# pyamg/pyamg

Measured on AMD Instinct MI355X. Metric: vcycle_iterations_per_sec, higher is better.
Workload: dtype f64; 1 GPU; 3D 7-pt Poisson 256^3 (16.7M dof) SA V-cycle, symmetric Gauss-Seidel, fp64; key=c3, n=16777216, nnz=117047296, levels=5, cycle=V(1,1), graph=True, parallelism=1 GPU, gs_order=fast, full=False

## Files before the change

include/pyamg_amd.h:

```cpp
#ifndef PYAMG_AMD_H
#define PYAMG_AMD_H

#include <stddef.h>
#include <stdint.h>

#ifdef __cplusplus
extern "C" {
#endif

#define PAMG_OK              0
#define PAMG_E_ARG          -1
#define PAMG_E_UNSUPPORTED  -2
#define PAMG_E_NODEVICE     -3
#define PAMG_E_STATE        -4
#define PAMG_E_ALLOC        -5
#define PAMG_E_TIMEOUT      -6

#define PAMG_F64 0
#define PAMG_F32 1

typedef void *pamg_stream_t;
typedef void *pamg_event_t;
typedef struct pamg_matrix_s *pamg_matrix_t;
typedef struct pamg_solver_s *pamg_solver_t;
// ... 159 lines not shown
                                int32_t row_step, int32_t blocksize);
int pamg_block_gauss_seidel_f32(const int32_t *Ap, int Ap_size, const int32_t *Aj,
                                int Aj_size, const float *Ax, int Ax_size, float *x,
                                int x_size, const float *b, int b_size, const float *Tx,
                                int Tx_size, int32_t row_start, int32_t row_stop,
                                int32_t row_step, int32_t blocksize);

int pamg_pinv_array_f64(double *AA, int AA_size, int32_t m, int32_t n, char TransA);
int pamg_pinv_array_f32(float *AA, int AA_size, int32_t m, int32_t n, char TransA);

int pamg_standard_aggregation(int32_t n_row, const int32_t *Ap, int Ap_size, const int32_t *Aj, int Aj_size,
                              int32_t *x, int x_size, int32_t *y, int y_size, int32_t *naggs);
int pamg_fit_candidates_f64(int32_t n_row, int32_t n_col, int32_t K1, int32_t K2, const int32_t *Ap, int Ap_size,
                            const int32_t *Ai, int Ai_size, double *Ax, int Ax_size, const double *B, int B_size,
                            double *R, int R_size, double tol);
int pamg_fit_candidates_f32(int32_t n_row, int32_t n_col, int32_t K1, int32_t K2, const int32_t *Ap, int Ap_size,
                            const int32_t *Ai, int Ai_size, float *Ax, int Ax_size, const float *B, int B_size,
                            float *R, int R_size, float tol);
int pamg_fit_tentative_f64(int32_t n_fine, int32_t n_coarse, int32_t K1, int32_t K2, const int32_t *Tp, const int32_t *Tj,
                           const double *B, double *Qx, double *R, double tol);
int pamg_fit_tentative_f32(int32_t n_fine, int32_t n_coarse, int32_t K1, int32_t K2, const int32_t *Tp, const int32_t *Tj,
                           const float *B, float *Qx, float *R, float tol);

int pamg_bsr_transpose_f64(int32_t n_brow, int32_t n_bcol, int32_t R, int32_t C, const int32_t *Ap, const int32_t *Aj,
                           const double *Ax, int32_t *Bp, int32_t *Bi, double *Bx);
int pamg_bsr_transpose_f32(int32_t n_brow, int32_t n_bcol, int32_t R, int32_t C, const int32_t *Ap, const int32_t *Aj,
                           const float *Ax, int32_t *Bp, int32_t *Bi, float *Bx);

#define PAMG_CSR 0
#define PAMG_BSR 1
int pamg_matrix_create(pamg_matrix_t *A, int dtype, int flavour, int n_brow, int n_bcol,
                       int R, int C, const int32_t *Ap, const int32_t *Aj, const void *Ax);
int pamg_matrix_destroy(pamg_matrix_t A);
int pamg_matrix_info(pamg_matrix_t A, int64_t info[8]);
int pamg_matrix_tune(pamg_matrix_t A, int key, int value);
int pamg_matrix_value_codes(pamg_matrix_t A, int *n_values);
int pamg_matrix_row_patterns(pamg_matrix_t A, int *n_patterns);
int pamg_matrix_row_masks(pamg_matrix_t A, long long info[8]);
int pamg_matrix_autotune(pamg_matrix_t A, int allow_cap);
int pamg_matrix_gs_profile(pamg_matrix_t A, int which, long long *out, int64_t capacity, int64_t *count);
int pamg_matrix_tile_info(pamg_matrix_t A, int which, int64_t info[8]);
int pamg_matrix_lane_info(pamg_matrix_t A, int which, int64_t info[8]);
int pamg_matrix_lanem_info(pamg_matrix_t A, int which, int64_t info[20], double *growth);
int pamg_matrix_point_twin(pamg_matrix_t A, int *state);
int pamg_matrix_lanem_levels(pamg_matrix_t A, int which, int64_t *out, int64_t capacity, int64_t *count);
int pamg_matrix_kz_info(pamg_matrix_t A, int which, int64_t info[8]);
int pamg_matrix_line_info(pamg_matrix_t A, int which, int64_t info[8]);
int pamg_matrix_lane_profile(pamg_matrix_t A, int which, long long *out, int64_t capacity, int64_t *count);
int pamg_matrix_subset_rows(pamg_matrix_t A, const int32_t *rows, int nrows, pamg_matrix_t *sub);
int pamg_matrix_kaczmarz(pamg_matrix_t L, int nr, void *v, const void *b, const void *Dinv, double omega,
                         int sweep, int iterations, void *xout, pamg_stream_t s);
int pamg_matrix_jacobi_indexed(pamg_matrix_t sub, void *x, const void *b, double omega, void *work,
                               pamg_stream_t s);
int pamg_matrix_flow_error(pamg_matrix_t A, int *error);

#define PAMG_SPMV_SET      0
#define PAMG_SPMV_ACC      1
#define PAMG_SPMV_RESID    2
#define PAMG_SPMV_AXPBY    3
#define PAMG_SPMV_ACC_AXPBY 4
int pamg_matrix_spmv(pamg_matrix_t A, int mode, const void *x, const void *b_or_v, double c,
                     void *y, pamg_stream_t s);
int pamg_matrix_split_ranges(pamg_matrix_t A, int64_t n_owned_cols);
int pamg_matrix_spmv_part(pamg_matrix_t A, int part, int mode, const void *x, const void *b_or_v, double c, void *y,
                          pamg_stream_t stream);
int pamg_matrix_resid_sumsq(pamg_matrix_t A, const void *x, const void *b, double *out_sumsq,
                            pamg_stream_t s);

#define PAMG_FORWARD   0
#define PAMG_BACKWARD  1
#define PAMG_SYMMETRIC 2
int pamg_matrix_jacobi(pamg_matrix_t A, void *x, const void *b, void *work, double omega,
                       int iterations, pamg_stream_t s);
int pamg_matrix_jacobi_step(pamg_matrix_t A, const void *x_in, const void *b, void *x_out,
                            double omega, pamg_stream_t s);
int pamg_matrix_block_jacobi_step(pamg_matrix_t A, const void *Dinv, const void *x_in, const void *b, void *x_out,
                                  double omega, pamg_stream_t s);
int pamg_matrix_block_jacobi_indexed(pamg_matrix_t A, const void *Dinv, void *x, const void *b, const int32_t *idx,
                                     int64_t nidx, double omega, void *work, pamg_stream_t s);
int pamg_matrix_gauss_seidel(pamg_matrix_t A, void *x, const void *b, int sweep, double omega,
                             int iterations, pamg_stream_t s);
int pamg_matrix_gauss_seidel_x0(pamg_matrix_t A, void *x, const void *b, int sweep, double omega,
                                int iterations, int x_is_zero, pamg_stream_t s);
int pamg_matrix_sym_info(pamg_matrix_t A, int64_t info[8]);
int pamg_matrix_polynomial(pamg_matrix_t A, void *x, const void *b, void *work,
                           const double *coeffs, int ncoeffs, int iterations, int x_is_zero,
                           pamg_stream_t s);
int pamg_matrix_block_jacobi(pamg_matrix_t A, void *x, const void *b, void *work,
                             const void *Dinv, double omega, int iterations, pamg_stream_t s);
int pamg_matrix_block_gauss_seidel(pamg_matrix_t A, void *x, const void *b, const void *Dinv,
                                   int sweep, int iterations, pamg_stream_t s);

int pamg_dev_pinv_array(int dtype, void *AA, int64_t m, int n, int transA, pamg_stream_t s);

int pamg_vec_sumsq(int dtype, int64_t n, const void *x, double *out_sumsq, pamg_stream_t s);
int pamg_vec_axpy(int dtype, int64_t n, double a, const void *x, void *y, pamg_stream_t s);
int pamg_vec_scale(int dtype, int64_t n, double a, const void *x, void *y, pamg_stream_t s);
int pamg_vec_mul(int dtype, int64_t n, const void *a, const void *b, void *y, pamg_stream_t s);
int pamg_vec_gather(int dtype, int64_t n, const int32_t *idx, const void *src, void *dst,
                    pamg_stream_t s);

int pamg_csr_renumber(int dtype, int64_t nrows, int64_t ncols, const int32_t *Ap, const int32_t *Aj, const void *Ax,
                      const int32_t *row_old_of_new, const int32_t *col_new_of_old, int32_t *Bp, int32_t *Bj, void *Bx);
int pamg_csr_row_argmax_abs(int dtype, int64_t nrows, const int32_t *Ap, const int32_t *Aj, const void *Ax, int32_t *out);
int pamg_csr_sort_rows(int dtype, int64_t nrows, const int32_t *Ap, int32_t *Aj, void *Ax, int block);
int pamg_host_cpus(int fresh);

#define PAMG_SMOOTH_NONE        0
#define PAMG_SMOOTH_JACOBI      1
#define PAMG_SMOOTH_GS          2
#define PAMG_SMOOTH_SOR         3
#define PAMG_SMOOTH_POLY        4
#define PAMG_SMOOTH_BLOCK_JACOBI 5
#define PAMG_SMOOTH_BLOCK_GS    6
#define PAMG_SMOOTH_CF_JACOBI   7
#define PAMG_SMOOTH_FC_JACOBI   8
#define PAMG_SMOOTH_GS_NE       9
#define PAMG_SMOOTH_GS_NR      10
#define PAMG_SMOOTH_JACOBI_NE  11
#define PAMG_SMOOTH_CF_BLOCK_JACOBI 12
#define PAMG_SMOOTH_FC_BLOCK_JACOBI 13
#define PAMG_SMOOTH_SCHWARZ    14
#define PAMG_SMOOTH_KRYLOV     15
#define PAMG_KRYLOV_CG    0
#define PAMG_KRYLOV_GMRES 1
#define PAMG_KRYLOV_CGNE  2
#define PAMG_KRYLOV_CGNR  3
#define PAMG_CYCLE_V 0
#define PAMG_CYCLE_W 1
#define PAMG_CYCLE_F 2
#define PAMG_CYCLE_AMLI 3
int pamg_solver_create(pamg_solver_t *S, int dtype);
int pamg_solver_destroy(pamg_solver_t S);
int pamg_solver_add_level(pamg_solver_t S, pamg_matrix_t A, pamg_matrix_t P, pamg_matrix_t R);
int pamg_solver_set_smoother(pamg_solver_t S, int level, int which, int kind, int iterations,
                             double omega, int sweep, const double *coeffs, int ncoeffs,
                             const void *Dinv, int blocksize);
int pamg_solver_set_cf_smoother(pamg_solver_t S, int level, int which, int kind, int iterations,
                                int f_iterations, int c_iterations, double omega, const int32_t *Fpts,
                                int nF, const int32_t *Cpts, int nC);
int pamg_solver_set_cf_block_smoother(pamg_solver_t S, int level, int which, int kind, int iterations,
                                      int f_iterations, int c_iterations, double omega, const void *Dinv,
                                      int blocksize, const int32_t *Fpts, int nF, const int32_t *Cpts, int nC);
typedef struct pamg_schwarz_s *pamg_schwarz_t;
int pamg_schwarz_create(pamg_schwarz_t *out, pamg_matrix_t A, int nsub, const int32_t *Sp, const int32_t *Sj,
                        const int32_t *Tp, const void *Tx);
int pamg_schwarz_destroy(pamg_schwarz_t h);
int pamg_schwarz_sweep(pamg_schwarz_t h, void *x, const void *b, int row_start, int row_stop, int row_step,
                       pamg_stream_t s);
int pamg_schwarz_info(pamg_schwarz_t h, int64_t info[4]);
int pamg_schwarz_set_mode(pamg_schwarz_t h, int mode);
int pamg_schwarz_error(pamg_schwarz_t h, int *error);
int pamg_solver_set_schwarz_smoother(pamg_solver_t S, int level, int which, int iterations, int sweep, pamg_matrix_t Ar,
                                     int nsub, const int32_t *Sp, const int32_t *Sj, const int32_t *Tp, const void *Tx);
int pamg_solver_set_ne_smoother(pamg_solver_t S, int level, int which, int kind, int iterations, double omega,
                                int sweep, const void *Dinv, pamg_matrix_t At, pamg_matrix_t Ar);
int pamg_solver_set_krylov_smoother(pamg_solver_t S, int level, int which, int method, double tol, int maxiter, int restart,
                                    pamg_matrix_t At);
int pamg_solver_set_coarse_dense(pamg_solver_t S, const void *M, int n_c);
int pamg_solver_set_coarse_relax(pamg_solver_t S);
typedef int (*pamg_coarse_host_fn)(void *user, const void *b_host, void *x_host, int64_t n_c);
int pamg_solver_set_coarse_host(pamg_solver_t S, pamg_coarse_host_fn fn, void *user, int n_c);
int pamg_solver_finalize(pamg_solver_t S);
int pamg_solver_cycle(pamg_solver_t S, void *x, const void *b, int cycle, int cycles_per_level,
                      pamg_stream_t s);
int pamg_solver_solve(pamg_solver_t S, void *x, const void *b, double tol, int maxiter,
                      int cycle, int cycles_per_level, int check_every, double *residuals,
// ... 86 lines not shown
```

pyamg_amd/_capi.py:

```python
from __future__ import annotations

import ctypes as C
import os
from pathlib import Path

import numpy as np

PKG = Path(__file__).resolve().parent
LIB_PATH = Path(os.environ.get("PAMG_LIB", PKG / "libpyamg_amd.so"))

OK = 0
E_ARG, E_UNSUPPORTED, E_NODEVICE, E_STATE, E_ALLOC = -1, -2, -3, -4, -5
E_TIMEOUT, E_COMM = -6, -7
F64, F32 = 0, 1
CSR, BSR = 0, 1
SPMV_SET, SPMV_ACC, SPMV_RESID, SPMV_AXPBY, SPMV_ACC_AXPBY = 0, 1, 2, 3, 4
FORWARD, BACKWARD, SYMMETRIC = 0, 1, 2
SMOOTH = {"schwarz": 14, "cf_block_jacobi": 12, "fc_block_jacobi": 13, "gauss_seidel_ne": 9, "gauss_seidel_nr": 10, "jacobi_ne": 11, "cf_jacobi": 7, "fc_jacobi": 8, "none": 0, "jacobi": 1, "gauss_seidel": 2, "sor": 3, "polynomial": 4,
          "block_jacobi": 5, "block_gauss_seidel": 6}
KRYLOV = {"cg": 0, "gmres": 1, "cgne": 2, "cgnr": 3}
ACCEL = {"bicgstab": 0, "cr": 1, "steepest_descent": 2, "minimal_residual": 3}
SWEEP = {"forward": FORWARD, "backward": BACKWARD, "symmetric": SYMMETRIC}
CYCLE = {"V": 0, "W": 1, "F": 2, "AMLI": 3}

# ... 44 lines not shown
    for n in ("h2d", "d2h", "d2d"):
        f(f"pamg_memcpy_{n}", _vp, _vp, _sz, _vp)
    f("pamg_memset", _vp, _i, _sz, _vp)
    f("pamg_stream_create", P(_vp))
    f("pamg_stream_destroy", _vp)
    f("pamg_stream_synchronize", _vp)
    f("pamg_device_synchronize")
    f("pamg_event_create", P(_vp))
    f("pamg_event_destroy", _vp)
    f("pamg_event_record", _vp, _vp)
    f("pamg_event_synchronize", _vp)
    f("pamg_event_elapsed_ms", _vp, _vp, P(C.c_float))
    for sfx, ct in (("f64", C.c_double), ("f32", C.c_float)):
        f(f"pamg_csr_matvec_{sfx}", _i, _i, _vp, _vp, _vp, _vp, _vp)
        f(f"pamg_bsr_matvec_{sfx}", _i, _i, _i, _i, _vp, _vp, _vp, _vp, _vp)
        csr5 = (_vp, _i, _vp, _i, _vp, _i, _vp, _i, _vp, _i)
        f(f"pamg_gauss_seidel_{sfx}", *csr5, _i, _i, _i)
        f(f"pamg_sor_gauss_seidel_{sfx}", *csr5, _i, _i, _i, ct)
        f(f"pamg_overlapping_schwarz_csr_{sfx}", *csr5, _vp, _i, _vp, _i, _vp, _i, _vp, _i, _i, _i, _i, _i, _i)
        f(f"pamg_gauss_seidel_indexed_{sfx}", *csr5, _vp, _i, _i, _i, _i)
        f(f"pamg_bsr_gauss_seidel_{sfx}", *csr5, _i, _i, _i, _i)
        f(f"pamg_jacobi_{sfx}", *csr5, _vp, _i, _i, _i, _i, _vp, _i)
        f(f"pamg_bsr_jacobi_{sfx}", *csr5, _vp, _i, _i, _i, _i, _i, _vp, _i)
        f(f"pamg_jacobi_indexed_{sfx}", *csr5, _vp, _i, _vp, _i)
        f(f"pamg_gauss_seidel_ne_{sfx}", *csr5, _i, _i, _i, _vp, _i, ct)
        f(f"pamg_gauss_seidel_nr_{sfx}", *csr5, _i, _i, _i, _vp, _i, ct)
        f(f"pamg_jacobi_ne_{sfx}", *csr5, _vp, _i, _vp, _i, _i, _i, _i, _vp, _i)
        f(f"pamg_block_jacobi_{sfx}", *csr5, _vp, _i, _vp, _i, _i, _i, _i, _vp, _i, _i)
        f(f"pamg_block_gauss_seidel_{sfx}", *csr5, _vp, _i, _i, _i, _i, _i)
        f(f"pamg_block_jacobi_indexed_{sfx}", *csr5, _vp, _i, _vp, _i, _vp, _i, _i)
    f("pamg_pinv_array_f64", _vp, _i, _i, _i, C.c_char)
    f("pamg_pinv_array_f32", _vp, _i, _i, _i, C.c_char)
    f("pamg_dev_pinv_array", _i, _vp, C.c_int64, _i, _i, _vp)
    f("pamg_bsr_transpose_f64", _i, _i, _i, _i, _vp, _vp, _vp, _vp, _vp, _vp)
    f("pamg_bsr_transpose_f32", _i, _i, _i, _i, _vp, _vp, _vp, _vp, _vp, _vp)
    f("pamg_standard_aggregation", _i, _vp, _i, _vp, _i, _vp, _i, _vp, _i, P(_i))
    f("pamg_csr_standard_aggregation", _vp, _vp, _vp, P(_i))
    f("pamg_fit_candidates_f64", _i, _i, _i, _i, _vp, _i, _vp, _i, _vp, _i, _vp, _i, _vp, _i, _d)
    f("pamg_fit_candidates_f32", _i, _i, _i, _i, _vp, _i, _vp, _i, _vp, _i, _vp, _i, _vp, _i, C.c_float)
    f("pamg_fit_tentative_f64", _i, _i, _i, _i, _vp, _vp, _vp, _vp, _vp, _d)
    f("pamg_fit_tentative_f32", _i, _i, _i, _i, _vp, _vp, _vp, _vp, _vp, C.c_float)
    f("pamg_matrix_create", P(_vp), _i, _i, _i, _i, _i, _i, _vp, _vp, _vp)
    f("pamg_matrix_destroy", _vp)
    f("pamg_matrix_info", _vp, P(C.c_int64))
    f("pamg_matrix_tune", _vp, _i, _i)
    f("pamg_matrix_value_codes", _vp, P(C.c_int))
    f("pamg_matrix_row_patterns", _vp, P(C.c_int))
    f("pamg_matrix_row_masks", _vp, P(C.c_longlong))
    f("pamg_matrix_flow_error", _vp, P(_i))
    f("pamg_matrix_subset_rows", _vp, _vp, _i, P(_vp))
    f("pamg_matrix_kaczmarz", _vp, _i, _vp, _vp, _vp, _d, _i, _i, _vp, _vp)
    f("pamg_vec_mul", _i, C.c_int64, _vp, _vp, _vp, _vp)
    f("pamg_matrix_jacobi_indexed", _vp, _vp, _vp, _d, _vp, _vp)
    f("pamg_matrix_gs_profile", _vp, _i, _vp, C.c_int64, P(C.c_int64))
    f("pamg_matrix_tile_info", _vp, _i, P(C.c_int64))
    f("pamg_matrix_lane_info", _vp, _i, P(C.c_int64))
    f("pamg_matrix_lanem_info", _vp, _i, P(C.c_int64), P(C.c_double))
    f("pamg_matrix_point_twin", _vp, P(_i))
    f("pamg_matrix_lanem_levels", _vp, _i, _vp, C.c_int64, P(C.c_int64))
    f("pamg_matrix_kz_info", _vp, _i, P(C.c_int64))
    f("pamg_matrix_line_info", _vp, _i, P(C.c_int64))
    f("pamg_matrix_lane_profile", _vp, _i, _vp, C.c_int64, P(C.c_int64))
    f("pamg_matrix_autotune", _vp, _i)
    f("pamg_matrix_spmv", _vp, _i, _vp, _vp, _d, _vp, _vp)
    f("pamg_matrix_split_ranges", _vp, C.c_int64)
    f("pamg_matrix_spmv_part", _vp, _i, _i, _vp, _vp, _d, _vp, _vp)
    f("pamg_matrix_resid_sumsq", _vp, _vp, _vp, _vp, _vp)
    f("pamg_matrix_jacobi", _vp, _vp, _vp, _vp, _d, _i, _vp)
    f("pamg_l1_cache_clear")
    f("pamg_l1_cache_size", P(C.c_int))
    f("pamg_matrix_jacobi_step", _vp, _vp, _vp, _vp, _d, _vp)
    f("pamg_matrix_block_jacobi_step", _vp, _vp, _vp, _vp, _vp, _d, _vp)
    f("pamg_matrix_block_jacobi_indexed", _vp, _vp, _vp, _vp, _vp, C.c_int64, _d, _vp, _vp)
    f("pamg_schwarz_create", P(_vp), _vp, _i, _vp, _vp, _vp, _vp)
    f("pamg_schwarz_destroy", _vp)
    f("pamg_schwarz_sweep", _vp, _vp, _vp, _i, _i, _i, _vp)
    f("pamg_schwarz_info", _vp, P(C.c_int64))
    f("pamg_schwarz_set_mode", _vp, _i)
    f("pamg_schwarz_error", _vp, P(_i))
    f("pamg_solver_set_schwarz_smoother", _vp, _i, _i, _i, _i, _vp, _i, _vp, _vp, _vp, _vp)
    f("pamg_solver_set_cf_block_smoother", _vp, _i, _i, _i, _i, _i, _i, _d, _vp, _i, _vp, _i, _vp, _i)
    f("pamg_matrix_gauss_seidel", _vp, _vp, _vp, _i, _d, _i, _vp)
    f("pamg_matrix_gauss_seidel_x0", _vp, _vp, _vp, _i, _d, _i, _i, _vp)
    f("pamg_matrix_sym_info", _vp, P(C.c_int64))
    f("pamg_matrix_polynomial", _vp, _vp, _vp, _vp, _vp, _i, _i, _i, _vp)
    f("pamg_matrix_block_jacobi", _vp, _vp, _vp, _vp, _vp, _d, _i, _vp)
    f("pamg_matrix_block_gauss_seidel", _vp, _vp, _vp, _vp, _i, _i, _vp)
    f("pamg_vec_sumsq", _i, C.c_int64, _vp, _vp, _vp)
    f("pamg_vec_axpy", _i, C.c_int64, _d, _vp, _vp, _vp)
    f("pamg_vec_scale", _i, C.c_int64, _d, _vp, _vp, _vp)
    f("pamg_vec_gather", _i, C.c_int64, _vp, _vp, _vp, _vp)
    f("pamg_csr_renumber", _i, C.c_int64, C.c_int64, _vp, _vp, _vp, _vp, _vp, _vp, _vp, _vp)
    f("pamg_csr_row_argmax_abs", _i, C.c_int64, _vp, _vp, _vp, _vp)
    f("pamg_csr_sort_rows", _i, C.c_int64, _vp, _vp, _vp, _i)
    f("pamg_host_cpus", _i)
    f("pamg_solver_create", P(_vp), _i)
    f("pamg_solver_destroy", _vp)
    f("pamg_solver_add_level", _vp, _vp, _vp, _vp)
    f("pamg_solver_set_smoother", _vp, _i, _i, _i, _i, _d, _i, _vp, _i, _vp, _i)
    f("pamg_solver_set_ne_smoother", _vp, _i, _i, _i, _i, _d, _i, _vp, _vp, _vp)
    f("pamg_solver_set_krylov_smoother", _vp, _i, _i, _i, _d, _i, _i, _vp)
    f("pamg_solver_set_cf_smoother", _vp, _i, _i, _i, _i, _i, _i, _d, _vp, _i, _vp, _i)
    f("pamg_solver_set_coarse_dense", _vp, _vp, _i)
    f("pamg_solver_set_coarse_relax", _vp)
    f("pamg_solver_set_coarse_host", _vp, _vp, _vp, _i)
    f("pamg_solver_finalize", _vp)
    f("pamg_solver_cycle", _vp, _vp, _vp, _i, _i, _vp)
    f("pamg_solver_solve", _vp, _vp, _vp, _d, _i, _i, _i, _i, _vp, P(_i), P(_i), _vp)
    f("pamg_solver_set_graph", _vp, _i)
    f("pamg_solver_pcg", _vp, _vp, _vp, _d, _i, _i, _i, _vp, P(_i), P(_i), _vp)
    f("pamg_solver_fgmres", _vp, _vp, _vp, _d, _i, _i, _i, _i, _vp, _i, P(_i), P(_i), P(_i), _vp)
    f("pamg_solver_gmres", _vp, _vp, _vp, _d, _i, _i, _i, _i, _vp, _i, P(_i), P(_i), P(_i), _vp)
    f("pamg_solver_krylov", _vp, _i, _vp, _vp, _d, _i, _i, _i, _vp, _i, P(_i), P(_i), P(_i), _vp)
    f("pamg_solver_load", _vp, _vp, _vp, _vp)
    f("pamg_solver_iterate", _vp, _i, _i, _i, _vp, _vp)
    f("pamg_solver_store", _vp, _vp, _vp)
    f("pamg_solver_stream", _vp, P(_vp))
    f("pamg_solver_stats", _vp, P(C.c_int64))
    f("pamg_dist_create", P(_vp), _i, _i, _i)
    f("pamg_dist_destroy", _vp)
    f("pamg_dist_add_level", _vp, _vp, _vp, _vp, C.c_int64, C.c_int64, _i, _vp, _vp, _vp, _i, _vp, _vp)
    f("pamg_dist_set_collapse", _vp, _vp, C.c_int64, C.c_int64, C.c_int64, C.c_int64, _vp)
    f("pamg_dist_set_smoother", _vp, _i, _i, _i, _i, _d, _vp, _i, _vp, _i)
    f("pamg_dist_set_callbacks", _vp, _vp, _vp, _vp)
    f("pamg_dist_rccl_unique_id", _vp)
    f("pamg_dist_set_rccl", _vp, _vp)
    f("pamg_dist_finalize", _vp)
    f("pamg_dist_set_options", _vp, _i, _i)
    f("pamg_dist_load", _vp, _vp, _vp)
    f("pamg_dist_store", _vp, _vp)
    f("pamg_dist_iterate", _vp, _i, _vp)
    f("pamg_dist_resid_norm", _vp, P(_d))
    f("pamg_dist_sync", _vp)
    f("pamg_dist_stream", _vp, P(_vp))
    f("pamg_dist_info", _vp, P(C.c_int64))
    f("pamg_dist_set_allgather", _vp, _i, C.c_int64, _vp)
    f("pamg_dist_set_exchange", _vp, _i)
    f("pamg_dist_set_model_transport", _vp)
    f("pamg_dist_level_info", _vp, _i, P(C.c_int64))
    f("pamg_rccl_selftest", C.c_int64, P(C.c_double))
    f("pamg_rccl_available")
    f("pamg_dist_exchange_test", _vp, _i, _vp, _vp)
    f("pamg_csr_create", P(_vp), C.c_int64, C.c_int64, _vp, _vp, _vp)
    f("pamg_csr_view", P(_vp), _vp)
    f("pamg_csr_destroy", _vp)
    f("pamg_csr_info", _vp, P(C.c_int64))
    f("pamg_csr_download", _vp, _vp, _vp, _vp)
    f("pamg_csr_matmat", _vp, _vp, _i, _i, P(_vp))
    f("pamg_csr_subtract", _vp, _vp, P(_vp))
    f("pamg_csr_subtract_bsr", _vp, _vp, _i, _i, P(_vp))
    f("pamg_csr_scale", _vp, _d)
    f("pamg_csr_strength_symmetric", _vp, _d, P(_vp))
    f("pamg_matrix_scale_rows", _vp, _vp)
    f("pamg_matrix_scale_values", _vp, _d)
    f("pamg_arnoldi_create", P(_vp), _vp, _i)
    f("pamg_arnoldi_destroy", _vp)
    f("pamg_arnoldi_run", _vp, _vp, _vp, _d, _vp, P(_i), P(_i))
    f("pamg_arnoldi_combine", _vp, _i, _vp, _vp)
    f("pamg_arnoldi_vector", _vp, _vp, _vp, P(_i))


def load(require_device: bool = False):
    global _lib
    if _lib is None:
        if not LIB_PATH.exists():
            raise DeviceUnavailable(
# ... 122 lines not shown
```

pyamg_amd/csrc/pamg_common.h:

```cpp
#pragma once
#include "pamg_host_threads.h"
#include <hip/hip_runtime.h>

#include <cstdint>
#include <cstdio>
#include <cstdlib>
#include <ctime>
#include <algorithm>
#include <atomic>
#include <cstring>
#include <thread>
#include <vector>

#include "../../include/pyamg_amd.h"

#define PAMG_STR2(x) #x
#define PAMG_STR(x) PAMG_STR2(x)
#define PAMG_HIP(expr)                                   \
    do {                                                 \
        hipError_t e__ = (expr);                         \
        if (e__ != hipSuccess) return (int)e__;          \
    } while (0)
#define PAMG_TRY(expr)                                   \
    do {                                                 \
// ... 121 lines not shown
}

struct pamg_matrix_s {
    int dtype = PAMG_F64;
    int flavour = PAMG_CSR;
    int n_brow = 0, n_bcol = 0, R = 1, C = 1;
    int64_t nrows = 0, ncols = 0, nnz = 0;
    int *d_Ap = nullptr, *d_Aj = nullptr;
    void *d_Ax = nullptr;
    void *d_diag = nullptr;
    int *d_rowid = nullptr;
    int *d_bAp = nullptr, *d_bAj = nullptr;
    int *d_bAjf = nullptr, *d_bdiag = nullptr;
    void *d_bAx = nullptr;
    int64_t nblocks_b = 0;
    int4 *d_bmeta = nullptr;
    int bnblk = 0;
    std::vector<int> h_Ap, h_Aj;
    std::vector<int> h_bAp, h_bAj;
    int cap = 1536, npl = 2, max_rows = 1024;
    int flow_cap = 32;
    unsigned short *d_Aj16 = nullptr;
    int4 *d_wbase = nullptr;
    int use_idx16 = 1;
    unsigned char *d_Ax8 = nullptr;
    void *d_vdict = nullptr;
    int nvdict = 0;
    int use_val8 = 1;
    int use_rowg = 0;
    unsigned char *d_pid = nullptr;
    void *d_ptab = nullptr;
    int npat = 0, pat_lmax = 0;
    unsigned char *d_pmask = nullptr;
    int rm_nu = 0, rm_off[8] = {0, 0, 0, 0, 0, 0, 0, 0};
    unsigned long long rm_val[8] = {0, 0, 0, 0, 0, 0, 0, 0};
    long long rm_walked = 0;
    int rowmask_kz = 8;
    int rowmask_flags = 3;
    int use_rowpat = 1;
    int cap_from_val8 = 0;
    int stream_flags = 0;
    int lds_pad = 0;
    int gran_xcd = 0;
    int gran_cap = 0;
    int gs_mode = 0;
    int tile_G = 0;
    int tile_W = 0;
    int tile_cap = 0;
    int tile_D = 0, tile_Q = -1;
    int tile_part = 1;
    bool tile_default = false;
    int max_row_len = 0;
    int borrowed = 0;
    int gs_prof = 0;
    int gs_order = 0;
    int lane_L = 0, lane_G = 0;
    int lane_flags = 1;
    int line_scan = 1;
    int lane_merge = 0;
    int lanem_rpw = 0;
    int lanem_cluster = 0;
    int lanem_ahead10 = 40;
    int lane_wide = 0;
    int gs_cap = 0;
    int nblk = 0;
    int *d_part[2] = {nullptr, nullptr};
    int npart[2] = {0, 0};
    int64_t part_cols = -1;
    int64_t part_row0[2] = {-1, -1}, part_row1[2] = {-1, -1};
    int4 *d_blkmeta = nullptr;
    double *d_partial = nullptr;
    pamg::GsSchedule *gs[4] = {nullptr, nullptr, nullptr, nullptr};
    pamg_matrix_s *point_twin = nullptr;
    size_t point_twin_bytes = 0;
    bool point_twin_unfit = false;
    pamg::LineSchedule *ls[4] = {nullptr, nullptr, nullptr, nullptr};
    int sym_fused = 1;
    void *d_sym_hf[2] = {nullptr, nullptr}, *d_sym_hb = nullptr;
    unsigned *d_sym_sync = nullptr;
    int sym_cap = 0;
    const void *sym_cap_kernel = nullptr;
    int zsym_cap = 0;
    const void *zsym_cap_kernel = nullptr;
    int sym_general_grid = 0;
    int sym_form = 0, sym_grid = 0;
    long long sym_launches = 0, sym_zero_launches = 0;
    int zero_plans = 0;
    int zero_merge = 0;
    struct pamg::LaneMSched *zplan[2] = {nullptr, nullptr};
    void *d_zw = nullptr;
    size_t zero_bytes = 0;
    long long zero_plan_launches = 0;
    size_t bytes = 0;
};

struct pamg_schwarz_s;
struct pamg_solver_s;
struct pamg_csr_s;

namespace pamg {
int schwarz_sweep(pamg_schwarz_s *h, void *x, const void *b, int start, int stop, int step, hipStream_t s);
int schwarz_prepare(pamg_schwarz_s *h, int sweep);
int schwarz_error(pamg_schwarz_s *h, bool *error);
void schwarz_level_launches(pamg_schwarz_s *h);
int stream_launch(pamg_matrix_s *A, int epi, const void *x, const void *b, void *y, double c,
                  double omega, double *partial, hipStream_t s);
int stream_launch_part(pamg_matrix_s *A, int part, int epi, const void *x, const void *b, void *y, double c,
                       double omega, double *partial, hipStream_t s);
int matrix_split_ranges(pamg_matrix_s *A, int64_t n_owned_cols);
void matrix_drop_value_codes(pamg_matrix_s *A);
void matrix_drop_point_twin(pamg_matrix_s *A);
void matrix_drop_schedules(pamg_matrix_s *A);
int gs_sweep(pamg_matrix_s *A, int epi, void *x, const void *b, double omega, int row_start,
             int row_stop, int row_step, hipStream_t s);
int gs_sweep_symmetric(pamg_matrix_s *A, void *x, const void *b, bool x_zero, hipStream_t s, bool *ran);
int ensure_sym_parts(pamg_matrix_s *A);
int sym_reset(pamg_matrix_s *A);
int reduce_partials(const double *partial, int n, double *out, hipStream_t s);
int vec_sumsq(int dtype, int64_t n, const void *x, double *scratch, double *out, hipStream_t s);
int vec_axpy(int dtype, int64_t n, double a, const void *x, void *y, hipStream_t s);
int vec_scale(int dtype, int64_t n, double a, const void *x, void *y, hipStream_t s);
int vec_dot(int dtype, int64_t n, const void *x, const void *y, double *scratch, double *out, hipStream_t s);
int vec_mul(int dtype, int64_t n, const void *a, const void *b, void *y, hipStream_t s);
int kaczmarz_sweep(pamg_matrix_s *L, bool nr, void *v, const void *b, const void *Dinv, double omega, int start, int stop,
                   int step, void *xout, hipStream_t s);
int ensure_line_schedule(pamg_matrix_s *L, int start, int stop, int step);
void free_line_schedule(LineSchedule *g);
int vec_scatter(int dtype, int64_t n, const int *idx, const void *src, void *dst, hipStream_t s);
int vec_copy_indexed(int dtype, int64_t n, const int *idx, const void *src, void *dst, hipStream_t s);
int matrix_row_subset(pamg_matrix_s *A, const int32_t *rows, int nrows, pamg_matrix_s **out);
int jacobi_indexed(pamg_matrix_s *sub, void *x, const void *b, double omega, void *work, hipStream_t s);
int vec_maxratio(int dtype, int64_t n, const void *u, const void *x, double *scratch, double *out, hipStream_t s);
int vec_xpby(int dtype, int64_t n, double beta, const void *z, void *p, hipStream_t s);
int vec_axpy_ratio(int dtype, int64_t n, const double *num, const double *den, double sign, const void *x, void *y, hipStream_t s);
int vec_fill(int dtype, int64_t n, double v, void *y, hipStream_t s);
int dense_gemv(int dtype, int n, const void *M, const void *b, void *x, hipStream_t s);
int block_gs_sweep(pamg_matrix_s *A, void *x, const void *b, const void *Dinv, int row_start,
                   int row_stop, int row_step, hipStream_t s);
int block_jacobi_step(pamg_matrix_s *A, int kind, const void *Dinv, const void *xsrc, void *xdst,
                      const void *b, double omega, hipStream_t s);
int ensure_schedule(pamg_matrix_s *A, int row_start, int row_stop, int row_step, bool block_gs = false);
struct CsrArrays { int64_t m, n, nnz; const int *p, *j; const double *x; };
int csr_device_arrays(struct ::pamg_csr_s *A, CsrArrays *out);
constexpr int KR_PARTIALS = 3 * 2048;
int kr_reduce(int64_t n, const double *part, int k, double *o0, double *o1, double *o2, hipStream_t s);
int kr_dots(int dtype, int64_t n, int k, const void *a0, const void *b0, const void *a1, const void *b1, const void *a2, const void *b2,
            double *part, hipStream_t s);
int bicg_alpha(int dtype, int64_t n, const double *rr, const double *d, double *alpha, void *x, void *xc, const void *r, const void *AMp,
               void *bc, hipStream_t s);
int bicg_omega(int dtype, int64_t n, const double *num, const double *den, double *omega, void *x, const void *xc, const void *bc,
               const void *AMs, void *r, const void *rstar, double *part, hipStream_t s);
int bicg_dir(int dtype, int64_t n, const double *rr_new, const double *rr_old, const double *alpha, const double *omega, const void *r,
             void *p, const void *AMp, void *bc, void *xc, hipStream_t s);
int cr_update(int dtype, int64_t n, const double *rAz, const double *ApAp, void *x, const void *p, void *r, const void *Ap, bool update_r,
              void *xc, hipStream_t s);
int cr_dir(int dtype, int64_t n, const double *rAz_new, const double *rAz_old, void *p, const void *z, void *Ap, const void *Az,
           double *part, hipStream_t s);
int sd_update(int dtype, int64_t n, const double *rz, const double *zAz, void *x, void *xc, void *r, const void *q, bool update_r,
              hipStream_t s);
int mr_update(int dtype, int64_t n, const double *pz, const double *pp, void *x, void *z, void *xc, bool update_z, double *part,
              hipStream_t s);
int kr_take(int dtype, int64_t n, void *xc, void *dst, double *part, hipStream_t s);
int solver_cycle_inline(pamg_solver_s *S, void *x, const void *b, int cycle, int cpl, hipStream_t s, bool allow_graph);
bool solver_needs_host_sync(const pamg_solver_s *S);
bool line_eligible(const pamg_matrix_s *A, const GsSchedule *g);
int build_line_part(pamg_matrix_s *A, GsSchedule *g);
void free_line_part(LineSched *t);
size_t line_part_bytes(const GsSchedule *g);
int line_launch(pamg_matrix_s *A, GsSchedule *g, int epi, void *x, const void *b, double omega, hipStream_t s);
int line_info(const GsSchedule *g, int64_t *info);
int line_sym_launch(pamg_matrix_s *A, GsSchedule *gf, GsSchedule *gb, void *x, const void *b, hipStream_t s);
int build_kz_lane_part(pamg_matrix_s *Lm, LineSchedule *g);
void free_kz_lane_part(KzLaneSched *t);
int kz_lane_launch(pamg_matrix_s *Lm, LineSchedule *g, bool nr, void *v, const void *b, const void *Dinv, double omega, void *xout, hipStream_t s);
int kz_lane_info(const LineSchedule *g, int64_t *info);
bool kz_lane_error(LineSchedule *g);
bool want_blanes(const pamg_matrix_s *A, const GsSchedule *g);
int block_point_sweep(pamg_matrix_s *A, GsSchedule *g, void *x, const void *b, int dirn, hipStream_t s);
int get_schedule(pamg_matrix_s *A, int row_start, int row_stop, int row_step, GsSchedule **out);
int ensure_parts(pamg_matrix_s *A, GsSchedule *g, bool block_gs = false);
int device_cus();
bool blane_eligible(const pamg_matrix_s *A, const GsSchedule *g);
int build_blane_part(pamg_matrix_s *A, GsSchedule *g);
void free_blane_part(BlaneSched *t);
size_t blane_part_bytes(const GsSchedule *g);
int blane_launch(pamg_matrix_s *A, GsSchedule *g, const void *Dinv, void *x, const void *b, hipStream_t s);
int blane_info(const GsSchedule *g, int64_t *info);
int blane_profile(const GsSchedule *g, long long *out, int64_t cap, int64_t *n);
int device_cus_lane();
bool lane_eligible(const pamg_matrix_s *A, const GsSchedule *g);
int build_lane_part(pamg_matrix_s *A, GsSchedule *g);
void free_lane_part(LaneSched *t);
size_t lane_part_bytes(const GsSchedule *g);
int lane_launch(pamg_matrix_s *A, GsSchedule *g, int epi, void *x, const void *b, double omega, hipStream_t s);
int lane_info(const GsSchedule *g, int64_t *info);
int lane_profile(const GsSchedule *g, long long *out, int64_t cap, int64_t *n);
int lanem_smax(const pamg_matrix_s *A, const GsSchedule *g);
int build_lanem_part(pamg_matrix_s *A, GsSchedule *g);
void free_lanem_part(struct LaneMSched *t);
size_t lanem_part_bytes(const GsSchedule *g);
int lanem_info(const GsSchedule *g, int64_t *info, double *growth);
int lanem_levels(const GsSchedule *g, int64_t *out, int64_t cap, int64_t *n);
int lanem_sym_launch(pamg_matrix_s *A, GsSchedule *gf, GsSchedule *gb, void *x, const void *b, bool x_zero, hipStream_t s);
int lanem_plan_info(const struct LaneMSched *t, int64_t *info, double *growth);
int build_zero_plan(pamg_matrix_s *A, int dir);
void free_zero_plans(pamg_matrix_s *A);
size_t zero_plan_bytes(const pamg_matrix_s *A);
bool zero_plans_ready(const pamg_matrix_s *A, const GsSchedule *gf, const GsSchedule *gb);
int lanem_zero_pair_launch(pamg_matrix_s *A, GsSchedule *gf, GsSchedule *gb, void *x, const void *b, hipStream_t s);
int ensure_zero_parts(pamg_matrix_s *A, bool build);
void matrix_drop_zero_plans(pamg_matrix_s *A);
int gs_sweep_zero_pair(pamg_matrix_s *A, void *x, const void *b, hipStream_t s, bool *ran);
int sym_fill_sentinels(void *p, int64_t n);
int sweep_error(pamg_matrix_s *A, bool *error);
inline size_t tsize(int dtype) { return dtype == PAMG_F64 ? 8 : 4; }

template <typename F>
inline void host_parallel(int64_t n, F fn, int64_t grain = 1 << 20)
{
    const unsigned hw = std::max(1u, std::min(32u, pamg::host_cpus()));
    const int nt = n < 2 * grain ? 1 : (int)std::min<int64_t>(hw, n / grain);
    if (nt <= 1) { fn((int64_t)0, n); return; }
    std::vector<std::thread> th;
    for (int t = 0; t < nt; ++t) {
        const int64_t lo = n * t / nt, hi = n * (t + 1) / nt;
        th.emplace_back([=] { fn(lo, hi); });
    }
    for (auto &x : th) x.join();
}

struct PhaseTimer {
    const char *name;
    int64_t items;
    timespec t0;
    static bool on() { static const int v = [] { const char *e = getenv("PAMG_TIMING"); return (e && *e && *e != '0') ? 1 : 0; }(); return v != 0; }
    explicit PhaseTimer(const char *n, int64_t k = 0) : name(n), items(k) { if (on()) clock_gettime(CLOCK_MONOTONIC, &t0); }
    ~PhaseTimer()
    {
        if (!on()) return;
        timespec t1;
        clock_gettime(CLOCK_MONOTONIC, &t1);
        fprintf(stderr, "[pamg timing] %-28s %8.3f s  (%lld)\n", name, (double)(t1.tv_sec - t0.tv_sec) + 1e-9 * (double)(t1.tv_nsec - t0.tv_nsec), (long long)items);
    }
};
}
```

pyamg_amd/csrc/pamg_lane.hip:

```cpp
#include "pamg_common.h"
#include "pamg_lane_plan.h"
#include "pamg_lanem_plan.h"
#include "pamg_tile_plan.h"

namespace pamg {

template <typename T> struct Sentinel;
template <> struct Sentinel<double> {
    using bits_t = unsigned long long;
    static constexpr bits_t value = 0x7FF8DEADBEEF5A5Aull;
    static __device__ __forceinline__ bits_t bits(double v) { return (bits_t)__double_as_longlong(v); }
};
template <> struct Sentinel<float> {
    using bits_t = unsigned int;
    static constexpr bits_t value = 0x7FC5BEEFu;
    static __device__ __forceinline__ bits_t bits(float v) { return __float_as_uint(v); }
};

template <typename T>
__global__ __launch_bounds__(BLK) void lane_fill_sentinel_kernel(T *xs, int64_t n)
{
    using B = typename Sentinel<T>::bits_t;
    B *p = reinterpret_cast<B *>(xs);
    for (int64_t i = (int64_t)blockIdx.x * BLK + threadIdx.x; i < n; i += (int64_t)gridDim.x * BLK) p[i] = Sentinel<T>::value;
// ... 290 lines not shown
    LaneMRec *d_rec = nullptr;
    long long *d_prof = nullptr;
    int cluster = 0;
    int4 *d_crec = nullptr;
    unsigned short *d_sidx = nullptr;
    int *d_crid = nullptr;
    double *d_crd = nullptr;
    int64_t n_uunits = 0, n_uearly = 0, n_uold = 0, n_ub = 0, n_early_lines = 0;
    std::vector<int64_t> super_grp;
    int last_grid = 0;
    int cap = 0;
    const void *cap_kernel = nullptr;
    size_t bytes = 0;
};

struct LaneMArgs {
    const int *cols;
    const double *vals;
    const LaneMRec *rec;
    const double *xold;
    double *y;
    double *xs;
    const double *b;
    unsigned *err;
    unsigned *ticket;
    int ngroups, nidle, use_gate;
    long long *prof;
    const unsigned short *sidx;
    const int *crid;
    const double *crd;
    int crows;
    double *w;
};

__global__ __launch_bounds__(BLK) void lanem_prepare_kernel(const double *__restrict__ x, double *__restrict__ xold, double *__restrict__ xs, int64_t n)
{
    unsigned long long *p = reinterpret_cast<unsigned long long *>(xs);
    for (int64_t i = (int64_t)blockIdx.x * BLK + threadIdx.x; i < n; i += (int64_t)gridDim.x * BLK) {
        xold[i] = x[i];
        p[i] = Sentinel<double>::value;
    }
}

template <int NREG>
struct MCtx {
    int c[NREG];
    double v[NREG], xv[NREG];
    double bv, xo, rd;
    double num;
    int rid;
    int gate, unit, K, g;
};

__device__ __forceinline__ void m_rec(const int4 *rp, int g, int gend, int4 &q0, int4 &q1)
{
    const size_t gg = (size_t)(g < gend ? g : gend - 1);
    q0 = rp[2 * gg];
    q1 = rp[2 * gg + 1];
}

template <int RPW, int NREG>
__device__ __forceinline__ void m_slots(const LaneMArgs &a, MCtx<NREG> &C, const int4 &q0, const int4 &q1, int g, int lane)
{
    C.g = g;
    const int rid_a = __builtin_amdgcn_readfirstlane(q0.x), rid_b = __builtin_amdgcn_readfirstlane(q0.y);
    C.gate = a.use_gate ? __builtin_amdgcn_readfirstlane(q0.z) : -1;
    const int uk = __builtin_amdgcn_readfirstlane(q0.w);
    C.unit = uk >> 4;
    C.K = uk & 15;
    const double rd_a = __hiloint2double(__builtin_amdgcn_readfirstlane(q1.y), __builtin_amdgcn_readfirstlane(q1.x));
    const double rd_b = __hiloint2double(__builtin_amdgcn_readfirstlane(q1.w), __builtin_amdgcn_readfirstlane(q1.z));
    const bool second = RPW == 2 && lane >= 32;
    C.rid = second ? rid_b : rid_a;
    C.rd = second ? rd_b : rd_a;
    const size_t e0 = (size_t)C.unit * 64 + (size_t)lane;
#pragma unroll
    for (int k = 0; k < NREG; ++k) {
        const size_t e = e0 + (size_t)64 * (size_t)(k < C.K ? k : C.K - 1);
        C.c[k] = a.cols[e];
        C.v[k] = a.vals[e];
    }
}

template <int NREG, bool BCOH = false>
__device__ __forceinline__ void m_gather(const LaneMArgs &a, MCtx<NREG> &C, int idle, const bool xz = false, const bool coh = false)
{
#pragma unroll
    for (int k = 1; k < NREG; ++k)
        if (k >= C.K) C.c[k] = LANE_NONE;
    if (xz) {
#pragma unroll
        for (int k = 0; k < NREG; ++k)
            if (!(C.c[k] & (LANE_EARLY | LANEM_BSRC))) C.c[k] |= LANE_NONE;
    }
    const int row = C.rid < 0 ? 0 : (C.rid & LANE_MASK);
    if constexpr (BCOH) C.bv = __hip_atomic_load(a.b + row, __ATOMIC_RELAXED, __HIP_MEMORY_SCOPE_AGENT);
    else C.bv = a.b[row];
    C.xo = coh ? __hip_atomic_load(a.xold + row, __ATOMIC_RELAXED, __HIP_MEMORY_SCOPE_AGENT) : a.xold[row];
#pragma unroll
    for (int k = 0; k < NREG; ++k) {
        const int col = C.c[k] & LANEM_MASK;
        const double *p = (C.c[k] & LANE_NONE) ? a.xold + idle : ((C.c[k] & LANE_EARLY) ? a.xs + col : ((C.c[k] & LANEM_BSRC) ? a.b + col : a.xold + col));
        C.xv[k] = __hip_atomic_load(p, __ATOMIC_RELAXED, __HIP_MEMORY_SCOPE_AGENT);
    }
}

template <int RPW, int NREG>
__device__ __forceinline__ double m_finish(const LaneMArgs &a, MCtx<NREG> &C, int idle, long long *t_ready = nullptr, unsigned *n_spins = nullptr, const bool xz = false)
{
    using T = double;
    const int lane = threadIdx.x & 63;
    unsigned pend = 0;
#pragma unroll
    for (int k = 0; k < NREG; ++k)
        if ((C.c[k] & LANE_EARLY) && !(C.c[k] & LANE_NONE) && Sentinel<T>::bits(C.xv[k]) == Sentinel<T>::value) pend |= 1u << k;
    unsigned spins = 0;
    if (C.gate >= 0 && __builtin_amdgcn_ballot_w64(pend != 0)) {
        const T *gp = a.xs + C.gate;
        while (true) {
            const T gv = __hip_atomic_load(gp, __ATOMIC_RELAXED, __HIP_MEMORY_SCOPE_AGENT);
            if (Sentinel<T>::bits(gv) != Sentinel<T>::value) break;
            __builtin_amdgcn_s_sleep(2);
            if ((++spins & 1023u) == 0 && (spins > (1u << 21) || __hip_atomic_load(a.err, __ATOMIC_RELAXED, __HIP_MEMORY_SCOPE_AGENT))) break;
        }
    }
    while (pend) {
        if (spins) __builtin_amdgcn_s_sleep(1);
        T t[NREG];
#pragma unroll
        for (int k = 0; k < NREG; ++k)
            t[k] = __hip_atomic_load(((pend >> k) & 1u) ? a.xs + (C.c[k] & LANEM_MASK) : a.xs + idle, __ATOMIC_RELAXED, __HIP_MEMORY_SCOPE_AGENT);
#pragma unroll
        for (int k = 0; k < NREG; ++k)
            if ((pend >> k) & 1u) {
                C.xv[k] = t[k];
                if (Sentinel<T>::bits(t[k]) != Sentinel<T>::value) pend &= ~(1u << k);
            }
        if ((++spins & 1023u) == 0) {
            if (spins > (1u << 21) || __hip_atomic_load(a.err, __ATOMIC_RELAXED, __HIP_MEMORY_SCOPE_AGENT)) {
                __hip_atomic_store(a.err, 1u, __ATOMIC_RELAXED, __HIP_MEMORY_SCOPE_AGENT);
                break;
            }
        }
    }
    if (t_ready) { *t_ready = wall_clock64(); *n_spins = spins; }
    T s = T(0);
#pragma unroll
    for (int k = 0; k < NREG; ++k) {
        const T pr = C.v[k] * C.xv[k];
        s = s + ((C.c[k] & LANE_NONE) ? T(0) : pr);
    }
    if (C.K > NREG) {
        for (int k = NREG; k < C.K; ++k) {
            const size_t e = (size_t)(C.unit + k) * 64 + (size_t)lane;
            int c = a.cols[e];
            if (xz && !(c & (LANE_EARLY | LANEM_BSRC))) c |= LANE_NONE;
            const T v = a.vals[e];
            const int col = c & LANEM_MASK;
            const bool early = (c & LANE_EARLY) && !(c & LANE_NONE);
            const T *p = (c & LANE_NONE) ? a.xold + idle : ((c & LANE_EARLY) ? a.xs + col : ((c & LANEM_BSRC) ? a.b + col : a.xold + col));
            T x = __hip_atomic_load(p, __ATOMIC_RELAXED, __HIP_MEMORY_SCOPE_AGENT);
            unsigned sp2 = 0;
            while (__builtin_amdgcn_ballot_w64(early && Sentinel<T>::bits(x) == Sentinel<T>::value)) {
                __builtin_amdgcn_s_sleep(1);
                const T t = __hip_atomic_load(p, __ATOMIC_RELAXED, __HIP_MEMORY_SCOPE_AGENT);
                if (early && Sentinel<T>::bits(x) == Sentinel<T>::value) x = t;
                if ((++sp2 & 1023u) == 0 && (sp2 > (1u << 21) || __hip_atomic_load(a.err, __ATOMIC_RELAXED, __HIP_MEMORY_SCOPE_AGENT))) {
                    __hip_atomic_store(a.err, 1u, __ATOMIC_RELAXED, __HIP_MEMORY_SCOPE_AGENT);
                    break;
                }
            }
            const T pr = v * x;
            s = s + ((c & LANE_NONE) ? T(0) : pr);
        }
    }
    s = seg_allreduce<64 / RPW, T>(s);
    const bool upd = C.rid >= 0 && !(C.rid & LANE_NODIAG);
    C.num = C.bv - s;
    T val = C.num * C.rd;
    if (!upd) val = C.xo;
    return val;
}

template <int RPW, int MODE, int NREG, int PH = 0, bool WST = false>
__device__ __forceinline__ void m_publish(const LaneMArgs &a, const MCtx<NREG> &C, double val)
{
    if (((threadIdx.x & 63) & (64 / RPW - 1)) == 0 && C.rid >= 0) {
        const int row = C.rid & LANE_MASK;
        if constexpr (MODE == 1) __hip_atomic_store(a.xs + row, val, __ATOMIC_RELAXED, __HIP_MEMORY_SCOPE_WORKGROUP);
        else __hip_atomic_store(a.xs + row, val, __ATOMIC_RELAXED, __HIP_MEMORY_SCOPE_AGENT);
        if constexpr (PH != 1) {
            if (!(C.rid & LANE_NODIAG)) a.y[row] = val;
        }
        if constexpr (WST) {
            if (!(C.rid & LANE_NODIAG)) __hip_atomic_store(a.w + row, C.num, __ATOMIC_RELAXED, __HIP_MEMORY_SCOPE_AGENT);
        }
    }
}

constexpr int LANEC_K = 8;

__device__ __forceinline__ int4 c_rec(const int4 *rp, int g, int gend) { return rp[(size_t)(g < gend ? g : gend - 1)]; }

template <int PH, bool WST = false, bool BCOH = false>
__device__ __forceinline__ void c_group(const LaneMArgs &a, double *lds, const int4 &q, int g, int lane, int idle, const bool xz, const bool coh)
{
    using T = double;
    const int gate = a.use_gate ? __builtin_amdgcn_readfirstlane(q.x) : -1;
    const int uunit = __builtin_amdgcn_readfirstlane(q.y), sunit = __builtin_amdgcn_readfirstlane(q.z), kk = __builtin_amdgcn_readfirstlane(q.w);
    const int KU = kk & 15, KS = (kk >> 8) & 15;
    int c[LANEC_K];
    unsigned si[LANEC_K];
    T sv[LANEC_K], xv[LANEC_K];
    const size_t u0 = (size_t)uunit * 64 + (size_t)lane, s0 = (size_t)sunit * 64 + (size_t)lane;
#pragma unroll
    for (int k = 0; k < LANEC_K; ++k) {
        c[k] = LANE_NONE;
        if (k < KU) c[k] = a.cols[u0 + (size_t)64 * k];
    }
#pragma unroll
    for (int k = 0; k < LANEC_K; ++k) {
        si[k] = LANEC_PAD | LANEC_UNUSED; sv[k] = T(0);
        if (k < KS) { si[k] = a.sidx[s0 + (size_t)64 * k]; sv[k] = a.vals[s0 + (size_t)64 * k]; }
    }
    if (xz) {
#pragma unroll
        for (int k = 0; k < LANEC_K; ++k)
            if (!(c[k] & (LANE_EARLY | LANEM_BSRC))) c[k] |= LANE_NONE;
    }
#pragma unroll
    for (int k = 0; k < LANEC_K; ++k) {
        xv[k] = T(0);
        if (k < KU) {
            const int col = c[k] & LANEM_MASK;
            const T *p = (c[k] & LANE_NONE) ? a.xold + idle : ((c[k] & LANE_EARLY) ? a.xs + col : ((c[k] & LANEM_BSRC) ? a.b + col : a.xold + col));
            xv[k] = __hip_atomic_load(p, __ATOMIC_RELAXED, __HIP_MEMORY_SCOPE_AGENT);
        }
    }
    const bool unused = (si[0] & LANEC_UNUSED) != 0;
    const int tag = (int)((si[0] >> LANEC_ROWSHIFT) & 7u);
    const size_t ri = (size_t)g * (size_t)a.crows + (size_t)(tag < a.crows ? tag : 0);
    const int rid = unused ? -1 : a.crid[ri];
    const T rd = a.crd[ri];
    const int row = rid < 0 ? 0 : (rid & LANE_MASK);
    T bv;
    if constexpr (BCOH) bv = __hip_atomic_load(a.b + row, __ATOMIC_RELAXED, __HIP_MEMORY_SCOPE_AGENT);
    else bv = a.b[row];
    const T xo = coh ? __hip_atomic_load(a.xold + row, __ATOMIC_RELAXED, __HIP_MEMORY_SCOPE_AGENT) : a.xold[row];
    unsigned pend = 0;
#pragma unroll
    for (int k = 0; k < LANEC_K; ++k)
        if ((c[k] & LANE_EARLY) && !(c[k] & LANE_NONE) && Sentinel<T>::bits(xv[k]) == Sentinel<T>::value) pend |= 1u << k;
    unsigned spins = 0;
    if (gate >= 0 && __builtin_amdgcn_ballot_w64(pend != 0)) {
        const T *gp = a.xs + gate;
        while (true) {
            const T gv = __hip_atomic_load(gp, __ATOMIC_RELAXED, __HIP_MEMORY_SCOPE_AGENT);
            if (Sentinel<T>::bits(gv) != Sentinel<T>::value) break;
            __builtin_amdgcn_s_sleep(2);
            if ((++spins & 1023u) == 0 && (spins > (1u << 21) || __hip_atomic_load(a.err, __ATOMIC_RELAXED, __HIP_MEMORY_SCOPE_AGENT))) break;
        }
    }
    while (pend) {
        if (spins) __builtin_amdgcn_s_sleep(1);
        T t[LANEC_K];
#pragma unroll
        for (int k = 0; k < LANEC_K; ++k) {
            t[k] = T(0);
            if (k < KU) t[k] = __hip_atomic_load(((pend >> k) & 1u) ? a.xs + (c[k] & LANEM_MASK) : a.xs + idle, __ATOMIC_RELAXED, __HIP_MEMORY_SCOPE_AGENT);
        }
#pragma unroll
        for (int k = 0; k < LANEC_K; ++k)
            if ((pend >> k) & 1u) {
                xv[k] = t[k];
                if (Sentinel<T>::bits(t[k]) != Sentinel<T>::value) pend &= ~(1u << k);
            }
        if ((++spins & 1023u) == 0) {
            if (spins > (1u << 21) || __hip_atomic_load(a.err, __ATOMIC_RELAXED, __HIP_MEMORY_SCOPE_AGENT)) {
                __hip_atomic_store(a.err, 1u, __ATOMIC_RELAXED, __HIP_MEMORY_SCOPE_AGENT);
                break;
            }
        }
    }
#pragma unroll
    for (int k = 0; k < LANEC_K; ++k)
        if (k < KU) lds[k * 64 + lane] = (c[k] & LANE_NONE) ? T(0) : xv[k];
    __builtin_amdgcn_fence(__ATOMIC_RELEASE, "wavefront");
    __builtin_amdgcn_wave_barrier();
    __builtin_amdgcn_fence(__ATOMIC_ACQUIRE, "wavefront");
    T s = T(0);
#pragma unroll
    for (int k = 0; k < LANEC_K; ++k) {
        const T pr = sv[k] * lds[si[k] & LANEC_IDX];
        s = s + ((si[k] & LANEC_PAD) ? T(0) : pr);
    }
    const unsigned key = si[0] & ((7u << LANEC_ROWSHIFT) | LANEC_UNUSED);
    const unsigned left = (unsigned)__shfl_up((int)key, 1);
    const unsigned long long heads = __builtin_amdgcn_ballot_w64(lane == 0 || left != key);
    const int seglo = 63 - __builtin_clzll(heads & (~0ull >> (63 - lane)));
#pragma unroll
    for (int d = 1; d < 64; d *= 2) {
        const T o = __shfl_up(s, d);
        s = s + ((lane - d >= seglo) ? o : T(0));
    }
    const bool tail = ((((heads >> 1) | (1ull << 63)) >> lane) & 1ull) != 0;
    __builtin_amdgcn_fence(__ATOMIC_RELEASE, "wavefront");
    __builtin_amdgcn_wave_barrier();
    const bool upd = rid >= 0 && !(rid & LANE_NODIAG);
    const T num = bv - s;
    T val = num * rd;
    if (!upd) val = xo;
    if (tail && rid >= 0) {
        __hip_atomic_store(a.xs + row, val, __ATOMIC_RELAXED, __HIP_MEMORY_SCOPE_AGENT);
        if constexpr (PH != 1) {
            if (upd) a.y[row] = val;
        }
        if constexpr (WST) {
            if (upd) __hip_atomic_store(a.w + row, num, __ATOMIC_RELAXED, __HIP_MEMORY_SCOPE_AGENT);
        }
    }
}

template <int MODE, int RPW, int NREG, int Z = 0>
__global__ __launch_bounds__(BLK) void gs_lanem_kernel(const LaneMArgs a)
{
    const int lane = threadIdx.x & 63;
    const int wib = threadIdx.x >> 6;
    const int idle = (int)((((unsigned)blockIdx.x * LANE_WPB + (unsigned)wib) * 16u) % (unsigned)a.nidle);
    const int4 *rp = reinterpret_cast<const int4 *>(a.rec);
    const int gend = a.ngroups;
    __shared__ double c_lds[RPW == 0 ? LANE_WPB * LANEC_UMAX : 1];
    if constexpr (RPW == 0) {
        static_assert(RPW != 0 || MODE != 1, "the cluster layout has no ticket form");
        const int W = (int)gridDim.x * LANE_WPB;
        int g = __builtin_amdgcn_readfirstlane((int)blockIdx.x * LANE_WPB + wib);
        if (g >= gend) return;
        int4 q = c_rec(rp, g, gend);
        for (; g < gend; g += W) {
            const int4 nq = c_rec(rp, g + W, gend);
            c_group<0, Z != 0>(a, c_lds + wib * LANEC_UMAX, q, g, lane, idle, false, false);
            q = nq;
        }
    } else {
    MCtx<NREG> X;
    if constexpr (MODE != 1) {
        const int W = (int)gridDim.x * LANE_WPB;
        int g = __builtin_amdgcn_readfirstlane((int)blockIdx.x * LANE_WPB + wib);
        if (g >= gend) return;
        int4 q0, q1;
        m_rec(rp, g, gend, q0, q1);
        for (; g < gend; g += W) {
            int4 n0, n1;
            m_rec(rp, g + W, gend, n0, n1);
            if (a.prof) {
                const long long t0 = wall_clock64();
                m_slots<RPW, NREG>(a, X, q0, q1, g, lane);
                asm volatile("s_waitcnt vmcnt(0)" ::: "memory");
                const long long t1 = wall_clock64();
                m_gather<NREG>(a, X, idle);
                long long t2 = 0;
                unsigned sp = 0;
                const double val = m_finish<RPW, NREG>(a, X, idle, &t2, &sp);
                m_publish<RPW, MODE, NREG, 0, Z != 0>(a, X, val);
                if (lane == 0) {
                    long long *o = a.prof + (size_t)g * 4;
                    o[0] = t0 | ((long long)(sp > 4095u ? 4095u : sp) << 52);
                    o[1] = t1; o[2] = t2; o[3] = wall_clock64();
                }
            } else {
                m_slots<RPW, NREG>(a, X, q0, q1, g, lane);
                m_gather<NREG>(a, X, idle);
                const double val = m_finish<RPW, NREG>(a, X, idle);
                m_publish<RPW, MODE, NREG, 0, Z != 0>(a, X, val);
            }
            q0 = n0; q1 = n1;
        }
    } else {
        __shared__ int sh_home;
        if (threadIdx.x == 0) {
            const unsigned me = (__builtin_amdgcn_s_getreg((3 << 11) | 20) & 0xF) + 1u;
            unsigned home = 0u;
            __hip_atomic_compare_exchange_strong(a.ticket + 1, &home, me, __ATOMIC_RELAXED, __ATOMIC_RELAXED, __HIP_MEMORY_SCOPE_AGENT);
            sh_home = (home == 0u || home == me) ? 1 : 0;
        }
        __syncthreads();
        if (!sh_home) return;
        unsigned tk = 0;
        if (lane == 0) tk = __hip_atomic_fetch_add(a.ticket, 1u, __ATOMIC_RELAXED, __HIP_MEMORY_SCOPE_AGENT);
        int g = (int)__builtin_amdgcn_readfirstlane(tk);
        if (g >= gend) return;
        if (lane == 0) tk = __hip_atomic_fetch_add(a.ticket, 1u, __ATOMIC_RELAXED, __HIP_MEMORY_SCOPE_AGENT);
        int g2 = (int)__builtin_amdgcn_readfirstlane(tk);
        int4 q0, q1;
        m_rec(rp, g, gend, q0, q1);
        while (true) {
            int4 n0, n1;
            m_rec(rp, g2, gend, n0, n1);
            unsigned tk3 = 0;
            if (g2 < gend && lane == 0) tk3 = __hip_atomic_fetch_add(a.ticket, 1u, __ATOMIC_RELAXED, __HIP_MEMORY_SCOPE_AGENT);
            m_slots<RPW, NREG>(a, X, q0, q1, g, lane);
            m_gather<NREG>(a, X, idle);
            const double val = m_finish<RPW, NREG>(a, X, idle);
            m_publish<RPW, MODE, NREG, 0, Z != 0>(a, X, val);
            if (g2 >= gend) break;
            g = g2; q0 = n0; q1 = n1;
            g2 = (int)__builtin_amdgcn_readfirstlane(tk3);
        }
    }
    }
}

struct LaneMSymArgs {
    LaneMArgs ph[2];
    double *hf[2];
    unsigned *sync;
    int wq[2], wr[2], wblk[2];
    int xzero;
};

template <int MODE>
__device__ __forceinline__ void m_wipe(double *w, int g, int G, int q, int r, int blk, int lane)
{
    if (g & (blk - 1)) return;
    const int g1 = g + blk < G ? g + blk : G;
    const int lo = g * q + (g < r ? g : r), hi = g1 * q + (g1 < r ? g1 : r);
    unsigned long long *p = reinterpret_cast<unsigned long long *>(w);
    for (int i = lo + lane; i < hi; i += 64) {
        if constexpr (MODE == 1) __hip_atomic_store(p + i, Sentinel<double>::value, __ATOMIC_RELAXED, __HIP_MEMORY_SCOPE_WORKGROUP);
        else __hip_atomic_store(p + i, Sentinel<double>::value, __ATOMIC_RELAXED, __HIP_MEMORY_SCOPE_AGENT);
    }
}

template <int MODE, int RPW, int NREG, int PH, int Z = 0>
__device__ __forceinline__ unsigned m_phase(const LaneMArgs &a, double *wipe, int wq, int wr, int wblk, unsigned *ticket, const bool xz, int lane, int wib, int idle, double *c_lds)
{
    const int4 *rp = reinterpret_cast<const int4 *>(a.rec);
    const int gend = a.ngroups;
    unsigned done = 0;
    if constexpr (RPW == 0) {
        static_assert(RPW != 0 || MODE != 1, "the cluster layout has no ticket form");
        const int W = (int)gridDim.x * LANE_WPB;
        int g = __builtin_amdgcn_readfirstlane((int)blockIdx.x * LANE_WPB + wib);
        if (g >= gend) return 0;
        int4 q = c_rec(rp, g, gend);
        for (; g < gend; g += W) {
            const int4 nq = c_rec(rp, g + W, gend);
            c_group<PH, Z && PH == 1, Z && PH == 2>(a, c_lds + wib * LANEC_UMAX, q, g, lane, idle, xz, PH == 2);
            m_wipe<MODE>(wipe, g, gend, wq, wr, wblk, lane);
            ++done;
            q = nq;
        }
    } else {
    MCtx<NREG> X;
    if constexpr (MODE != 1) {
        const int W = (int)gridDim.x * LANE_WPB;
        int g = __builtin_amdgcn_readfirstlane((int)blockIdx.x * LANE_WPB + wib);
        if (g >= gend) return 0;
        int4 q0, q1;
        m_rec(rp, g, gend, q0, q1);
        for (; g < gend; g += W) {
            int4 n0, n1;
            m_rec(rp, g + W, gend, n0, n1);
            m_slots<RPW, NREG>(a, X, q0, q1, g, lane);
            m_gather<NREG, Z && PH == 2>(a, X, idle, xz, PH == 2);
            const double val = m_finish<RPW, NREG>(a, X, idle, nullptr, nullptr, xz);
            m_publish<RPW, MODE, NREG, PH, Z && PH == 1>(a, X, val);
            m_wipe<MODE>(wipe, g, gend, wq, wr, wblk, lane);
            ++done;
            q0 = n0; q1 = n1;
        }
    } else {
        unsigned tk = 0;
        if (lane == 0) tk = __hip_atomic_fetch_add(ticket, 1u, __ATOMIC_RELAXED, __HIP_MEMORY_SCOPE_AGENT);
        int g = (int)__builtin_amdgcn_readfirstlane(tk);
        if (g >= gend) return 0;
        if (lane == 0) tk = __hip_atomic_fetch_add(ticket, 1u, __ATOMIC_RELAXED, __HIP_MEMORY_SCOPE_AGENT);
        int g2 = (int)__builtin_amdgcn_readfirstlane(tk);
        int4 q0, q1;
        m_rec(rp, g, gend, q0, q1);
        while (true) {
            int4 n0, n1;
            m_rec(rp, g2, gend, n0, n1);
            unsigned tk3 = 0;
            if (g2 < gend && lane == 0) tk3 = __hip_atomic_fetch_add(ticket, 1u, __ATOMIC_RELAXED, __HIP_MEMORY_SCOPE_AGENT);
            m_slots<RPW, NREG>(a, X, q0, q1, g, lane);
            m_gather<NREG, Z && PH == 2>(a, X, idle, xz, PH == 2);
            const double val = m_finish<RPW, NREG>(a, X, idle, nullptr, nullptr, xz);
            m_publish<RPW, MODE, NREG, PH, Z && PH == 1>(a, X, val);
            m_wipe<MODE>(wipe, g, gend, wq, wr, wblk, lane);
            ++done;
            if (g2 >= gend) break;
            g = g2; q0 = n0; q1 = n1;
            g2 = (int)__builtin_amdgcn_readfirstlane(tk3);
        }
    }
    }
    return done;
}

__device__ __forceinline__ void sym_phase_barrier(unsigned *counter, unsigned *err, unsigned *sh_done, unsigned done, unsigned total)
{
    asm volatile("s_waitcnt vmcnt(0)" ::: "memory");
    if ((threadIdx.x & 63) == 0 && done) atomicAdd(sh_done, done);
    __syncthreads();
    if (threadIdx.x == 0) {
        const unsigned mine = *sh_done;
        if (mine) __hip_atomic_fetch_add(counter, mine, __ATOMIC_RELAXED, __HIP_MEMORY_SCOPE_AGENT);
        unsigned spins = 0;
        while (__hip_atomic_load(counter, __ATOMIC_RELAXED, __HIP_MEMORY_SCOPE_AGENT) < total) {
            __builtin_amdgcn_s_sleep(2);
            if ((++spins & 1023u) == 0 && (spins > (1u << 21) || __hip_atomic_load(err, __ATOMIC_RELAXED, __HIP_MEMORY_SCOPE_AGENT))) {
                __hip_atomic_store(err, 1u, __ATOMIC_RELAXED, __HIP_MEMORY_SCOPE_AGENT);
                break;
            }
        }
    }
    __syncthreads();
}

__device__ __forceinline__ void sym_leave(unsigned *sync, unsigned parity)
{
    __syncthreads();
    if (threadIdx.x == 0) {
        const unsigned left = __hip_atomic_fetch_add(sync + 1, 1u, __ATOMIC_RELAXED, __HIP_MEMORY_SCOPE_AGENT);
        if (left == gridDim.x - 1) {
            for (int k = 0; k < 5; ++k) __hip_atomic_store(sync + k, 0u, __ATOMIC_RELAXED, __HIP_MEMORY_SCOPE_AGENT);
            __hip_atomic_store(sync + 5, parity ^ 1u, __ATOMIC_RELAXED, __HIP_MEMORY_SCOPE_AGENT);
        }
    }
}

template <int MODE, int RPW, int NREG, int Z = 0>
__global__ __launch_bounds__(BLK) void gs_lanem_sym_kernel(const LaneMSymArgs a)
{
    __shared__ unsigned sh_done;
    __shared__ int sh_home;
    __shared__ double c_lds[RPW == 0 ? LANE_WPB * LANEC_UMAX : 1];
    const int lane = threadIdx.x & 63;
    const int wib = threadIdx.x >> 6;
    const int idle = (int)((((unsigned)blockIdx.x * LANE_WPB + (unsigned)wib) * 16u) % (unsigned)a.ph[0].nidle);
    const unsigned parity = __builtin_amdgcn_readfirstlane(__hip_atomic_load(a.sync + 5, __ATOMIC_RELAXED, __HIP_MEMORY_SCOPE_AGENT)) & 1u;
    if (threadIdx.x == 0) {
        sh_done = 0u;
        sh_home = 1;
        if constexpr (MODE == 1) {
            const unsigned me = (__builtin_amdgcn_s_getreg((3 << 11) | 20) & 0xF) + 1u;
            unsigned home = 0u;
            __hip_atomic_compare_exchange_strong(a.sync + 4, &home, me, __ATOMIC_RELAXED, __ATOMIC_RELAXED, __HIP_MEMORY_SCOPE_AGENT);
            sh_home = (home == 0u || home == me) ? 1 : 0;
        }
    }
    __syncthreads();
    if (sh_home) {
        double *hf = a.hf[parity], *hf_next = a.hf[parity ^ 1u];
        LaneMArgs p1 = a.ph[0], p2 = a.ph[1];
        p1.xs = hf; p1.y = nullptr;
        p2.xold = hf;
        const unsigned done = m_phase<MODE, RPW, NREG, 1, Z>(p1, p2.xs, a.wq[0], a.wr[0], a.wblk[0], a.sync + 2, a.xzero != 0, lane, wib, idle, c_lds);
        sym_phase_barrier(a.sync, p1.err, &sh_done, done, (unsigned)p1.ngroups);
        (void)m_phase<MODE, RPW, NREG, 2, Z>(p2, hf_next, a.wq[1], a.wr[1], a.wblk[1], a.sync + 3, false, lane, wib, idle, c_lds);
    }
    sym_leave(a.sync, parity);
}

namespace {

template <typename U>
int lane_upload(U **dst, const void *src, size_t bytes, size_t *total)
{
    *dst = nullptr;
    const size_t alloc = std::max<size_t>(bytes, 256) + 256;
// ... 286 lines not shown

int lanem_zero_smax(const pamg_matrix_s *A)
{
    if (A->zero_merge >= 2) return A->zero_merge;
    static const int env = [] { const char *e = getenv("PAMG_ZERO_MERGE"); return e ? atoi(e) : 0; }();
    if (env >= 2) return env;
    return A->nrows > 131072 ? 6 : 16;
}

int build_zero_plan(pamg_matrix_s *A, int dir)
{
    if (dir < 0 || dir > 1 || A->zplan[dir]) return PAMG_OK;
    if (A->dtype != PAMG_F64 || A->R != 1 || A->nrows < 2 || A->nrows != A->ncols || !A->d_Ax) return PAMG_E_ARG;
    PhaseTimer pt_(dir ? "build_zero_plan (backward, triu)" : "build_zero_plan (forward, tril)", A->nnz);
    const int n = (int)A->nrows;
    PlanVec<double> hAx;
    hAx.resize((size_t)A->nnz + 1);
    if (A->nnz) PAMG_HIP(hipMemcpy(hAx.data(), A->d_Ax, (size_t)A->nnz * sizeof(double), hipMemcpyDeviceToHost));
    const int *Ap = A->h_Ap.data(), *Aj = A->h_Aj.data();
    std::vector<int> Tp((size_t)n + 1, 0);
    lane_parallel(n, [&](int64_t i0, int64_t i1) {
        for (int64_t i = i0; i < i1; ++i) {
            int c = 0;
            for (int p = Ap[i]; p < Ap[i + 1]; ++p) c += dir ? (Aj[p] >= (int)i) : (Aj[p] <= (int)i);
            Tp[(size_t)i + 1] = c;
        }
    });
    for (int i = 0; i < n; ++i) Tp[(size_t)i + 1] += Tp[(size_t)i];
    PlanVec<int> Tj;
    PlanVec<double> Tx;
    Tj.resize((size_t)Tp[(size_t)n] + 1);
    Tx.resize((size_t)Tp[(size_t)n] + 1);
    lane_parallel(n, [&](int64_t i0, int64_t i1) {
        for (int64_t i = i0; i < i1; ++i) {
            int q = Tp[(size_t)i];
            for (int p = Ap[i]; p < Ap[i + 1]; ++p)
                if (dir ? (Aj[p] >= (int)i) : (Aj[p] <= (int)i)) { Tj[(size_t)q] = Aj[p]; Tx[(size_t)q] = hAx[(size_t)p]; ++q; }
        }
    });
    hAx = PlanVec<double>();
    std::vector<int> vis, lvl;
    int m = 0, nl = 0;
    if (sweep_levels(n, Tp.data(), Tj.data(), dir ? n - 1 : 0, dir ? -1 : n, dir ? -1 : 1, vis, lvl, m, nl) || m != n || nl < 8) return PAMG_E_ARG;
    const int s_max = lanem_zero_smax(A);
    const int rpw = A->lanem_rpw ? A->lanem_rpw : (A->nrows > 131072 ? 2 : 1);
    LaneMPlan P;
    if (build_lanem_plan(n, Tp.data(), Tj.data(), Tx.data(), dir ? n - 1 : 0, dir ? -1 : 1, m, nl, vis, lvl, s_max, 1e3, P, LANEM_KMAX * 64, rpw, lanem_cluster_rows(A)))
        return PAMG_E_ARG;
    LaneMSched *t = nullptr;
    PAMG_TRY(lanem_to_device(P, s_max, &t));
    A->zplan[dir] = t;
    return PAMG_OK;
}

void free_zero_plans(pamg_matrix_s *A)
{
    for (int d = 0; d < 2; ++d) { free_lanem_part(A->zplan[d]); A->zplan[d] = nullptr; }
    hipFree(A->d_zw);
    A->d_zw = nullptr;
}

size_t zero_plan_bytes(const pamg_matrix_s *A)
{
    size_t b = A->d_zw ? ((size_t)A->nrows + 8) * sizeof(double) : 0;
    for (int d = 0; d < 2; ++d) if (A->zplan[d]) b += A->zplan[d]->bytes;
    return b;
}

bool zero_plans_ready(const pamg_matrix_s *A, const GsSchedule *gf, const GsSchedule *gb)
{
    const LaneMSched *zf = A->zplan[0], *zb = A->zplan[1];
    if (A->zero_plans == 1 || !zf || !zb || !A->d_zw || !gf || !gb || !gf->lanem || !gb->lanem) return false;
    return zf->rpw == zb->rpw && zf->cluster == zb->cluster && zf->rpw == gf->lanem->rpw && zf->cluster == gf->lanem->cluster &&
           zb->rpw == gb->lanem->rpw && zb->cluster == gb->lanem->cluster && zf->ngroups >= 1 && zb->ngroups >= 1;
}

static void lanem_layout_args(const LaneMSched *t, LaneMArgs &a)
{
    a.cols = t->d_cols; a.vals = t->d_vals;
    a.rec = t->cluster ? reinterpret_cast<const LaneMRec *>(t->d_crec) : t->d_rec;
    a.sidx = t->d_sidx; a.crid = t->d_crid; a.crd = t->d_crd; a.crows = t->cluster;
}

static int lanem_launch_plan(pamg_matrix_s *A, GsSchedule *g, LaneMSched *t, void *x, const void *b, double *w, hipStream_t s)
{
    if (!t || !g->d_xold) return PAMG_E_STATE;
    const int64_t n = A->nrows;
    LaneMArgs a;
    lanem_layout_args(t, a);
    a.use_gate = (A->lane_flags & 1) ? 1 : 0;
    a.xold = (const double *)g->d_xold; a.y = (double *)x; a.xs = (double *)g->d_xs; a.b = (const double *)b;
    a.w = w;
    a.err = g->d_sync + 1; a.ticket = g->d_sync + 20;
    a.ngroups = (int)t->ngroups;
    a.nidle = (int)std::max<int64_t>(1, std::min<int64_t>(n, 1 << 20));
    if (A->gs_prof && !t->d_prof && !t->cluster) {
        PAMG_HIP(hipMalloc((void **)&t->d_prof, (size_t)t->ngroups * 4 * sizeof(long long)));
        PAMG_HIP(hipMemset(t->d_prof, 0, (size_t)t->ngroups * 4 * sizeof(long long)));
    }
    a.prof = (A->gs_prof && !t->cluster) ? t->d_prof : nullptr;
    const int fgrid = (int)std::min<int64_t>(4096, (n + BLK - 1) / BLK);
    hipLaunchKernelGGL(lanem_prepare_kernel, dim3(fgrid), dim3(BLK), 0, s, (const double *)x, (double *)g->d_xold, (double *)g->d_xs, n);
    PAMG_HIP(hipGetLastError());
    const bool xcd = !t->cluster && (A->gran_xcd == 1 || (A->gran_xcd == 0 && lane_one_xcd(A, g) && A->nrows <= 8192));
    static const int nreg_env = [] { const char *e = getenv("PAMG_LANEM_NREG"); return e ? atoi(e) : 0; }();
    const bool all_regs = t->rpw == 1 && (nreg_env ? nreg_env == 8 : A->nrows <= 131072);
    const void *k = t->cluster  ? (const void *)gs_lanem_kernel<0, 0, 8>
                  : t->rpw == 2 ? (xcd ? (const void *)gs_lanem_kernel<1, 2, 4> : (const void *)gs_lanem_kernel<0, 2, 4>)
                  : all_regs    ? (xcd ? (const void *)gs_lanem_kernel<1, 1, 8> : (const void *)gs_lanem_kernel<0, 1, 8>)
                                : (xcd ? (const void *)gs_lanem_kernel<1, 1, 2> : (const void *)gs_lanem_kernel<0, 1, 2>);
    if (w)
        k = t->cluster  ? (const void *)gs_lanem_kernel<0, 0, 8, 1>
          : t->rpw == 2 ? (xcd ? (const void *)gs_lanem_kernel<1, 2, 4, 1> : (const void *)gs_lanem_kernel<0, 2, 4, 1>)
          : all_regs    ? (xcd ? (const void *)gs_lanem_kernel<1, 1, 8, 1> : (const void *)gs_lanem_kernel<0, 1, 8, 1>)
                        : (xcd ? (const void *)gs_lanem_kernel<1, 1, 2, 1> : (const void *)gs_lanem_kernel<0, 1, 2, 1>);
    static thread_local int cus = 0;
    if (!cus) cus = device_cus_lane();
    if (!(t->cap > 0 && t->cap_kernel == k)) {
        int nb = 0;
        if (hipOccupancyMaxActiveBlocksPerMultiprocessor(&nb, k, BLK, 0) != hipSuccess) nb = 2;
        t->cap = std::max(1, std::min(nb - 1, 8));
        t->cap_kernel = k;
    }
    const int cap = t->cap;
    const int per_level = (int)((t->ngroups + t->nsuper - 1) / std::max(1, t->nsuper));
    const int64_t want_waves = std::max<int64_t>(128, ((int64_t)A->lanem_ahead10 * per_level + 9) / 10);
    const int cwpb = LANE_WPB;
    int G = (int)std::min<int64_t>((want_waves + cwpb - 1) / cwpb, (int64_t)std::min(cap, (t->rpw == 2 || t->cluster) ? 2 : 3) * cus);
    if (A->lane_G > 0) G = std::min(A->lane_G, cap * cus);
    G = (int)std::max<int64_t>(1, std::min<int64_t>(G, (t->ngroups + cwpb - 1) / cwpb));
    void *args[] = {(void *)&a};
    if (xcd) {
        PAMG_HIP(hipMemsetAsync(g->d_sync + 20, 0, 2 * sizeof(unsigned), s));
        const int Gx = std::max(1, std::min(G, (cus / 8) * cap));
        t->last_grid = 8 * Gx;
        PAMG_HIP(hipLaunchKernel(k, dim3(8 * Gx), dim3(BLK), args, 0, s));
        return PAMG_OK;
    }
    t->last_grid = G;
    PAMG_HIP(hipLaunchKernel(k, dim3(G), dim3(BLK), args, 0, s));
    return PAMG_OK;
}

int lanem_launch(pamg_matrix_s *A, GsSchedule *g, void *x, const void *b, hipStream_t s) { return lanem_launch_plan(A, g, g->lanem, x, b, nullptr, s); }

int lanem_zero_pair_launch(pamg_matrix_s *A, GsSchedule *gf, GsSchedule *gb, void *x, const void *b, hipStream_t s)
{
    if (!zero_plans_ready(A, gf, gb)) return PAMG_E_UNSUPPORTED;
    PAMG_TRY(lanem_launch_plan(A, gf, A->zplan[0], x, b, (double *)A->d_zw, s));
    PAMG_TRY(lanem_launch_plan(A, gb, A->zplan[1], x, A->d_zw, nullptr, s));
    A->zero_plan_launches++;
    return PAMG_OK;
}

int sym_fill_sentinels(void *p, int64_t n)
{
    if (n <= 0) return PAMG_OK;
    const int fgrid = (int)std::min<int64_t>(4096, (n + BLK - 1) / BLK);
    hipLaunchKernelGGL((lane_fill_sentinel_kernel<double>), dim3(fgrid), dim3(BLK), 0, 0, (double *)p, n);
    PAMG_HIP(hipGetLastError());
    PAMG_HIP(hipDeviceSynchronize());
    return PAMG_OK;
}

int lanem_sym_launch(pamg_matrix_s *A, GsSchedule *gf, GsSchedule *gb, void *x, const void *b, bool x_zero, hipStream_t s)
{
    LaneMSched *tf = gf->lanem, *tb = gb->lanem;
    if (!tf || !tb || !A->d_sym_hf[0] || !A->d_sym_hf[1] || !A->d_sym_hb || !A->d_sym_sync) return PAMG_E_STATE;
    const bool zero = x_zero && zero_plans_ready(A, gf, gb);
    if (zero) { tf = A->zplan[0]; tb = A->zplan[1]; }
    const int64_t n = A->nrows;
    auto one_xcd = [&](const GsSchedule *g) { return !g->lanem->cluster && (A->gran_xcd == 1 || (A->gran_xcd == 0 && lane_one_xcd(A, g) && A->nrows <= 8192)); };
    const bool xcd = one_xcd(gf);
    if (xcd != one_xcd(gb) || tf->rpw != tb->rpw || tf->cluster != tb->cluster || tf->ngroups < 1 || tb->ngroups < 1) return PAMG_E_UNSUPPORTED;
    LaneMSymArgs a;
    LaneMSched *ts2[2] = {tf, tb};
    for (int p = 0; p < 2; ++p) {
        LaneMSched *t = ts2[p];
        LaneMArgs &q = a.ph[p];
        lanem_layout_args(t, q);
        q.use_gate = (A->lane_flags & 1) ? 1 : 0;
        q.b = (const double *)b;
        q.w = nullptr;
        q.err = gf->d_sync + 1; q.ticket = nullptr;
        q.ngroups = (int)t->ngroups;
        q.nidle = (int)std::max<int64_t>(1, std::min<int64_t>(n, 1 << 20));
        q.prof = nullptr;
        a.wq[p] = (int)(n / t->ngroups); a.wr[p] = (int)(n % t->ngroups);
        a.wblk[p] = 1;
        while ((int64_t)a.wblk[p] * n < 64 * t->ngroups && a.wblk[p] < (1 << 20)) a.wblk[p] *= 2;
    }
    a.ph[0].xold = (const double *)x; a.ph[0].y = nullptr;     a.ph[0].xs = nullptr;
    a.ph[1].xold = nullptr;           a.ph[1].y = (double *)x; a.ph[1].xs = (double *)A->d_sym_hb;
    if (zero) { a.ph[0].w = (double *)A->d_zw; a.ph[1].b = (const double *)A->d_zw; }
    a.hf[0] = (double *)A->d_sym_hf[0]; a.hf[1] = (double *)A->d_sym_hf[1];
    a.sync = A->d_sym_sync;
    a.xzero = x_zero ? 1 : 0;
    static const int nreg_env = [] { const char *e = getenv("PAMG_LANEM_NREG"); return e ? atoi(e) : 0; }();
    const bool all_regs = tf->rpw == 1 && (nreg_env ? nreg_env == 8 : A->nrows <= 131072);
    const void *k = tf->cluster  ? (const void *)gs_lanem_sym_kernel<0, 0, 8>
                  : tf->rpw == 2 ? (xcd ? (const void *)gs_lanem_sym_kernel<1, 2, 4> : (const void *)gs_lanem_sym_kernel<0, 2, 4>)
                  : all_regs     ? (xcd ? (const void *)gs_lanem_sym_kernel<1, 1, 8> : (const void *)gs_lanem_sym_kernel<0, 1, 8>)
                                 : (xcd ? (const void *)gs_lanem_sym_kernel<1, 1, 2> : (const void *)gs_lanem_sym_kernel<0, 1, 2>);
    if (zero)
        k = tf->cluster  ? (const void *)gs_lanem_sym_kernel<0, 0, 8, 1>
          : tf->rpw == 2 ? (xcd ? (const void *)gs_lanem_sym_kernel<1, 2, 4, 1> : (const void *)gs_lanem_sym_kernel<0, 2, 4, 1>)
          : all_regs     ? (xcd ? (const void *)gs_lanem_sym_kernel<1, 1, 8, 1> : (const void *)gs_lanem_sym_kernel<0, 1, 8, 1>)
                         : (xcd ? (const void *)gs_lanem_sym_kernel<1, 1, 2, 1> : (const void *)gs_lanem_sym_kernel<0, 1, 2, 1>);
    static thread_local int cus = 0;
    if (!cus) cus = device_cus_lane();
    int &kcap = zero ? A->zsym_cap : A->sym_cap;
    const void *&kcap_kernel = zero ? A->zsym_cap_kernel : A->sym_cap_kernel;
    if (!(kcap > 0 && kcap_kernel == k)) {
        int nb = 0;
        if (hipOccupancyMaxActiveBlocksPerMultiprocessor(&nb, k, BLK, 0) != hipSuccess) nb = 2;
        kcap = std::max(1, std::min(nb - 1, 8));
        kcap_kernel = k;
    }
    const int cap = kcap;
    int G = 1;
    for (int p = 0; p < 2; ++p) {
        const LaneMSched *t = ts2[p];
        const int per_level = (int)((t->ngroups + t->nsuper - 1) / std::max(1, t->nsuper));
        const int64_t want_waves = std::max<int64_t>(128, ((int64_t)A->lanem_ahead10 * per_level + 9) / 10);
        int Gp = (int)std::min<int64_t>((want_waves + LANE_WPB - 1) / LANE_WPB, (int64_t)std::min(cap, (t->rpw == 2 || t->cluster) ? 2 : 3) * cus);
        if (A->lane_G > 0) Gp = std::min(A->lane_G, cap * cus);
        Gp = (int)std::max<int64_t>(1, std::min<int64_t>(Gp, (t->ngroups + LANE_WPB - 1) / LANE_WPB));
        G = std::max(G, Gp);
    }
    if (xcd) G = 8 * std::max(1, std::min(G, (cus / 8) * cap));
    void *args[] = {(void *)&a};
    PAMG_HIP(hipLaunchKernel(k, dim3(G), dim3(BLK), args, 0, s));
    A->sym_form = xcd ? 3 : 1; A->sym_grid = G;
    if (zero) tf->last_grid = tb->last_grid = G;
    else A->sym_general_grid = G;
    A->sym_launches++;
    if (x_zero) A->sym_zero_launches++;
    if (zero) A->zero_plan_launches++;
    return PAMG_OK;
}

int lanem_info(const GsSchedule *g, int64_t *info, double *growth) { return lanem_plan_info(g ? g->lanem : nullptr, info, growth); }

int lanem_plan_info(const LaneMSched *t, int64_t *info, double *growth)
{
    for (int i = 0; i < 20; ++i) info[i] = 0;
    if (growth) *growth = 0.0;
    if (!t) return PAMG_OK;
    info[0] = t->nsuper; info[1] = t->nlevels; info[2] = t->nrows; info[3] = t->n_units; info[4] = t->n_early; info[5] = t->n_old; info[6] = t->n_b;
    info[7] = t->max_len; info[8] = t->s_max; info[9] = t->closed_by_length; info[10] = t->closed_by_growth; info[11] = t->last_grid;
    info[12] = t->cluster; info[13] = t->ngroups; info[14] = t->n_units * 64; info[15] = t->n_uunits;
    info[16] = t->cluster ? t->n_uearly : t->n_early; info[17] = t->cluster ? t->n_uold : t->n_old; info[18] = t->cluster ? t->n_ub : t->n_b; info[19] = t->n_early_lines;
    if (growth) *growth = t->max_growth;
    return PAMG_OK;
}


static int lane_grid_cap(LaneSched *t, const void *k)
{
    if (t->cap > 0 && t->cap_kernel == k) return t->cap;
    int nb = 0;
    if (hipOccupancyMaxActiveBlocksPerMultiprocessor(&nb, k, BLK, 0) != hipSuccess) nb = 2;
    nb = std::max(1, std::min(nb - 1, 8));
    t->cap = nb; t->cap_kernel = k;
    return nb;
}

int device_cus_lane()
{
    int dev = 0;
    hipDeviceProp_t p;
    if (hipGetDevice(&dev) != hipSuccess || hipGetDeviceProperties(&p, dev) != hipSuccess) return 64;
    return p.multiProcessorCount;
}

template <typename T>
static int lane_launch_t(pamg_matrix_s *A, GsSchedule *g, int epi, void *x, const void *b, double omega, hipStream_t s)
{
    LaneSched *t = g->lane;
    const size_t ts = tsize(A->dtype);
    const int64_t n = A->nrows;
    LaneArgs<T> a;
    a.cols = t->d_cols; a.vals = (const T *)t->d_vals; a.rec = t->d_rec;
    a.use_gate = (A->lane_flags & 1) ? 1 : 0;
    a.x = (const T *)x; a.y = (T *)x; a.xs = (T *)g->d_xs; a.b = (const T *)b;
    a.err = g->d_sync + 1; a.ticket = g->d_sync + 20;
    a.ngroups = (int)t->ngroups;
    a.nidle = (int)std::max<int64_t>(1, std::min<int64_t>(n, 1 << 20));
    a.omega = (T)omega;
    if (!g->symmetric) {
        if (!g->d_xold) return PAMG_E_STATE;
        PAMG_HIP(hipMemcpyAsync(g->d_xold, x, (size_t)n * ts, hipMemcpyDeviceToDevice, s));
        a.x = (const T *)g->d_xold;
    }
    if (A->gs_prof && !t->d_prof) {
// ... 74 lines not shown
```

pyamg_amd/csrc/pamg_matrix.hip:

```cpp
#include "pamg_host_threads.h"
#include <algorithm>
#include <atomic>
#include <mutex>
#include <climits>
#include <new>
#include <thread>

#include "pamg_kernels.h"
#include "pamg_tile_kernels.h"
#include "pamg_tile_plan.h"
#include "pamg_stream_plan.h"

using namespace pamg;

namespace {

constexpr int PAD = 8;

std::mutex g_sched_mu;

template <typename U>
int upload(U **dptr, const U *h, size_t n, size_t *bytes)
{
    const size_t sz = (n + PAD) * sizeof(U);
// ... 1298 lines not shown
        PAMG_TRY(ensure_sym_parts(A));
        if (!A->d_sym_hf[0]) return PAMG_OK;
    }
    if (form == 1 && x_zero && A->zero_plans == 2 && !A->zplan[0] && !A->zplan[1]) {
        hipStreamCaptureStatus cs = hipStreamCaptureStatusNone;
        PAMG_HIP(hipStreamIsCapturing(s, &cs));
        if (cs == hipStreamCaptureStatusNone) {
            PAMG_TRY(ensure_zero_parts(A, true));
            if (!zero_plans_ready(A, gf, gb)) A->zero_plans = 1;
        }
    }
    const int st = form == 2 ? line_sym_launch(A, gf, gb, x, b, s) : lanem_sym_launch(A, gf, gb, x, b, x_zero, s);
    if (st == PAMG_E_UNSUPPORTED) return PAMG_OK;
    if (st == PAMG_OK) *ran = true;
    return st;
}

void matrix_drop_zero_plans(pamg_matrix_s *A)
{
    if (!A || (!A->zplan[0] && !A->zplan[1] && !A->d_zw)) return;
    free_zero_plans(A);
    std::lock_guard<std::mutex> lk(g_sched_mu);
    A->bytes -= std::min(A->bytes, A->zero_bytes);
    A->zero_bytes = 0;
}

static bool zero_form_of(pamg_matrix_s *A, GsSchedule **pf, GsSchedule **pb)
{
    if (A->zero_plans == 1 || A->R != 1 || A->dtype != PAMG_F64 || A->gs_order != 1 || A->gs_mode != 0 || A->gs_prof || A->nrows < 2) return false;
    const int n = (int)A->nrows;
    GsSchedule *gf = nullptr, *gb = nullptr;
    if (get_schedule(A, 0, n, 1, &gf) != PAMG_OK || get_schedule(A, n - 1, -1, -1, &gb) != PAMG_OK) return false;
    if (ensure_parts(A, gf) != PAMG_OK || ensure_parts(A, gb) != PAMG_OK) return false;
    if (gf->nrows != A->nrows || gb->nrows != A->nrows) return false;
    if (want_lines(A, gf) || want_lines(A, gb)) return false;
    if (!(want_lanes(A, gf) && want_lanes(A, gb) && gf->lanem && gb->lanem)) return false;
    *pf = gf; *pb = gb;
    return true;
}

int ensure_zero_parts(pamg_matrix_s *A, bool build)
{
    if (!A) return PAMG_OK;
    GsSchedule *gf = nullptr, *gb = nullptr;
    if (!zero_form_of(A, &gf, &gb)) { matrix_drop_zero_plans(A); return PAMG_OK; }
    if (A->d_zw && A->zplan[0] && A->zplan[1]) return PAMG_OK;
    if (build && (!A->zplan[0] || !A->zplan[1])) {
        int st[2] = {PAMG_OK, PAMG_OK};
        int dev = 0;
        PAMG_HIP(hipGetDevice(&dev));
        std::thread other([&] { st[1] = (int)hipSetDevice(dev); if (!st[1]) st[1] = build_zero_plan(A, 1); });
        st[0] = build_zero_plan(A, 0);
        other.join();
        for (int d = 0; d < 2; ++d) if (st[d] != PAMG_OK && st[d] != PAMG_E_ARG) { matrix_drop_zero_plans(A); return st[d]; }
    }
    if (!A->zplan[0] || !A->zplan[1]) { matrix_drop_zero_plans(A); return PAMG_OK; }
    if (!A->d_zw) {
        const size_t vb = ((size_t)A->nrows + 8) * sizeof(double);
        PAMG_HIP(hipMalloc(&A->d_zw, vb));
        PAMG_HIP(hipMemset(A->d_zw, 0, vb));
    }
    if (!zero_plans_ready(A, gf, gb)) { matrix_drop_zero_plans(A); return PAMG_OK; }
    std::lock_guard<std::mutex> lk(g_sched_mu);
    A->bytes -= std::min(A->bytes, A->zero_bytes);
    A->zero_bytes = zero_plan_bytes(A);
    A->bytes += A->zero_bytes;
    return PAMG_OK;
}

int gs_sweep_zero_pair(pamg_matrix_s *A, void *x, const void *b, hipStream_t s, bool *ran)
{
    *ran = false;
    if (A->zero_plans == 1 || (A->zero_plans == 0 && !A->zplan[0])) return PAMG_OK;
    GsSchedule *gf = nullptr, *gb = nullptr;
    if (!zero_form_of(A, &gf, &gb)) return PAMG_OK;
    if (!zero_plans_ready(A, gf, gb)) {
        if (A->zero_plans != 2 || A->zplan[0] || A->zplan[1]) return PAMG_OK;
        hipStreamCaptureStatus cs = hipStreamCaptureStatusNone;
        PAMG_HIP(hipStreamIsCapturing(s, &cs));
        if (cs != hipStreamCaptureStatusNone) return PAMG_OK;
        PAMG_TRY(ensure_zero_parts(A, true));
        if (!zero_plans_ready(A, gf, gb)) { A->zero_plans = 1; return PAMG_OK; }
    }
    const int st = lanem_zero_pair_launch(A, gf, gb, x, b, s);
    if (st == PAMG_E_UNSUPPORTED) return PAMG_OK;
    if (st == PAMG_OK) *ran = true;
    return st;
}

int ensure_schedule(pamg_matrix_s *A, int row_start, int row_stop, int row_step, bool block_gs)
{
    GsSchedule *g = nullptr;
    PAMG_TRY(get_schedule(A, row_start, row_stop, row_step, &g));
    return ensure_parts(A, g, block_gs);
}

int reduce_partials(const double *partial, int n, double *out, hipStream_t s)
{
    if (n > 8192) {
        double *mid = const_cast<double *>(partial) + n;
        hipLaunchKernelGGL(reduce_mid_kernel, dim3(256), dim3(BLK), 0, s, partial, n, mid);
        hipLaunchKernelGGL(reduce_final_kernel, dim3(1), dim3(BLK), 0, s, (const double *)mid, 256, out);
    } else {
        hipLaunchKernelGGL(reduce_final_kernel, dim3(1), dim3(BLK), 0, s, partial, n, out);
    }
    return (int)hipGetLastError();
}

int vec_sumsq(int dtype, int64_t n, const void *x, double *scratch, double *out, hipStream_t s)
{
    const int grid = (int)std::min<int64_t>(1024, std::max<int64_t>(1, (n + BLK - 1) / BLK));
    if (dtype == PAMG_F64)
        hipLaunchKernelGGL((vec_sumsq_kernel<double>), dim3(grid), dim3(BLK), 0, s, (const double *)x, n, scratch);
    else
        hipLaunchKernelGGL((vec_sumsq_kernel<float>), dim3(grid), dim3(BLK), 0, s, (const float *)x, n, scratch);
    PAMG_HIP(hipGetLastError());
    return reduce_partials(scratch, grid, out, s);
}

int vec_dot(int dtype, int64_t n, const void *x, const void *y, double *scratch, double *out, hipStream_t s)
{
    const int grid = (int)std::min<int64_t>(1024, std::max<int64_t>(1, (n + BLK - 1) / BLK));
    if (dtype == PAMG_F64)
        hipLaunchKernelGGL((vec_dot_kernel<double>), dim3(grid), dim3(BLK), 0, s, (const double *)x, (const double *)y, n, scratch);
    else
        hipLaunchKernelGGL((vec_dot_kernel<float>), dim3(grid), dim3(BLK), 0, s, (const float *)x, (const float *)y, n, scratch);
    PAMG_HIP(hipGetLastError());
    hipLaunchKernelGGL(reduce_final_kernel, dim3(1), dim3(BLK), 0, s, (const double *)scratch, grid, out);
    return (int)hipGetLastError();
}

static int vgrid(int64_t n) { return (int)std::min<int64_t>(1 << 21, std::max<int64_t>(1, (n + BLK - 1) / BLK)); }

int vec_mul(int dtype, int64_t n, const void *a, const void *b, void *y, hipStream_t s)
{
    if (n <= 0) return PAMG_OK;
    const int grid = vgrid(n);
    if (dtype == PAMG_F64)
        hipLaunchKernelGGL((vec_mul_kernel<double>), dim3(grid), dim3(BLK), 0, s, n, (const double *)a, (const double *)b, (double *)y);
    else
        hipLaunchKernelGGL((vec_mul_kernel<float>), dim3(grid), dim3(BLK), 0, s, n, (const float *)a, (const float *)b, (float *)y);
    return (int)hipGetLastError();
}

void free_line_schedule(LineSchedule *g)
{
    if (!g) return;
    hipFree(g->d_lines); hipFree(g->d_level_ptr); hipFree(g->d_len); hipFree(g->d_lo); hipFree(g->d_ej); hipFree(g->d_ea);
    free_kz_lane_part(g->kzl);
    delete g;
}

static int get_line_schedule(pamg_matrix_s *L, int start, int stop, int step, LineSchedule **out)
{
    for (int k = 0; k < 4; ++k) {
        LineSchedule *g = L->ls[k];
        if (g && g->start == start && g->stop == stop && g->step == step) {
            *out = g;
            if (L->gs_order == 1) PAMG_TRY(build_kz_lane_part(L, g));
            return PAMG_OK;
        }
    }
    if (step == 0) return PAMG_E_ARG;
    const long span = (long)stop - start;
    if (span % step != 0 || span / step < 0) return PAMG_E_ARG;
    const int m = (int)(span / step), n = (int)L->nrows;
    if (m > 0 && (start < 0 || start >= n || start + (long)(m - 1) * step < 0 || start + (long)(m - 1) * step >= n)) return PAMG_E_ARG;
    std::vector<int> seen((size_t)L->ncols, -1), lvl((size_t)std::max(m, 1));
    int nl = 0;
    for (int t = 0; t < m; ++t) {
// ... 401 lines not shown
    if (!A || !info) return PAMG_E_ARG;
    info[0] = A->nrows; info[1] = A->ncols; info[2] = A->nnz; info[3] = A->nblk;
    info[4] = A->cap; info[5] = (int64_t)A->bytes;
    info[6] = info[7] = 0;
    const int n = A->R > 1 ? A->n_brow : (int)A->nrows;
    for (int k = 0; k < 4; ++k) {
        GsSchedule *g = A->gs[k];
        if (!g) continue;
        if (g->row_start == 0 && g->row_stop == n && g->row_step == 1) info[6] = g->nlevels;
        if (g->row_start == n - 1 && g->row_stop == -1 && g->row_step == -1) info[7] = g->nlevels;
    }
    return PAMG_OK;
}

int pamg_matrix_value_codes(pamg_matrix_t A, int *n_values)
{
    if (!A || !n_values) return PAMG_E_ARG;
    *n_values = (A->d_Ax8 && A->use_val8 && A->use_idx16 && A->d_Aj16 && A->npl == 2) ? A->nvdict : 0;
    return PAMG_OK;
}

int pamg_matrix_row_patterns(pamg_matrix_t A, int *n_patterns)
{
    if (!A || !n_patterns) return PAMG_E_ARG;
    *n_patterns = (A->d_pid && A->use_rowpat && A->d_Ax8 && A->use_val8 && A->use_idx16 && A->d_Aj16 && A->npl == 2) ? A->npat : 0;
    return PAMG_OK;
}

int pamg_matrix_row_masks(pamg_matrix_t A, long long info[8])
{
    if (!A || !info) return PAMG_E_ARG;
    for (int k = 0; k < 8; ++k) info[k] = 0;
    int npat = 0;
    pamg_matrix_row_patterns(A, &npat);
    if (!npat || !A->d_pmask || (A->use_rowpat != 1 && A->use_rowpat != 4)) return PAMG_OK;
    info[0] = A->rm_nu; info[1] = A->rm_walked; info[5] = A->rowmask_kz; info[6] = A->rowmask_flags;
    info[7] = (A->nrows + BLK - 1) / BLK;
    RowMaskLattice g;
    int grid3 = 0;
    if (A->use_rowpat == 1 && rowmask_lattice_plan(A->rm_nu, A->rm_off, A->nrows, A->rowmask_kz, (A->rowmask_flags & 2) != 0, false, g, grid3)) {
        info[2] = 1; info[3] = g.L; info[4] = g.P; info[7] = grid3;
    }
    return PAMG_OK;
}

int pamg_matrix_tune(pamg_matrix_t A, int key, int value)
{
    if (!A) return PAMG_E_ARG;
    if (key == 21) { A->use_val8 = value != 0; return PAMG_OK; }
    if (key == 22) { A->use_rowg = value != 0; return PAMG_OK; }
    if (key == 23) { if (value < 0 || value > 4 || value == 2) return PAMG_E_ARG; A->use_rowpat = value; return PAMG_OK; }
    if (A->borrowed > 0) return PAMG_E_STATE;
    switch (key) {
        case 0: if (value < 64 || value > 12288) return PAMG_E_ARG; A->cap = value & ~3; A->cap_from_val8 = 0; break;
        case 1: if (value != 2) return PAMG_E_ARG; A->npl = 2; return PAMG_OK;
        case 2: if (value < 1) return PAMG_E_ARG; A->max_rows = value; break;
        case 3: if (value < 0 || value > 256) return PAMG_E_ARG; A->flow_cap = value; return PAMG_OK;
        case 5: if (value < 0 || value > 5) return PAMG_E_ARG; A->gs_mode = value; return PAMG_OK;
        case 6: if (value < 0) return PAMG_E_ARG; A->gran_cap = value; return PAMG_OK;
        case 7: if (value < 0 || value > 2) return PAMG_E_ARG; A->gran_xcd = value; matrix_drop_point_twin(A); return PAMG_OK;
        case 8: if (value < 0 || value > 63) return PAMG_E_ARG; A->stream_flags = value; return PAMG_OK;
        case 11: A->gs_prof = value != 0; return PAMG_OK;
        case 12: if (value < 0) return PAMG_E_ARG; A->tile_G = value; break;
        case 13: if (value != 0 && (value < 64 || value > 8192 || (value & (value - 1)))) return PAMG_E_ARG; A->tile_W = value; break;
        case 14: if (value < 0 || value > TILE_MAX_ENTRIES) return PAMG_E_ARG; A->tile_cap = value; break;
        case 15: A->tile_default = value != 0; return PAMG_OK;
        case 16: if (value < 0 || value > 32) return PAMG_E_ARG; A->tile_D = value; break;
        case 17: if (value < -1 || value > 4) return PAMG_E_ARG; A->tile_Q = value; break;
        case 18: if (value < 0 || value > 1) return PAMG_E_ARG; A->tile_part = value; break;
        case 19: A->use_idx16 = value != 0; return PAMG_OK;
        case 20: if (value != 0 && (value < 64 || value > 2048)) return PAMG_E_ARG; A->gs_cap = value & ~3; break;
        case 24: if (value < 0 || value > 1) return PAMG_E_ARG; A->gs_order = value; return PAMG_OK;
        case 25: if (value != 0 && value != 4 && value != 8 && value != 16 && value != 32 && value != 64) return PAMG_E_ARG; A->lane_L = value; break;
        case 26: if (value < 0) return PAMG_E_ARG; A->lane_G = value; matrix_drop_point_twin(A); return PAMG_OK;
        case 27: if (value < 0 || value > 1) return PAMG_E_ARG; A->lane_wide = value; matrix_drop_point_twin(A); return PAMG_OK;
        case 33: if (value < 0 || value > 8) return PAMG_E_ARG; A->lane_merge = value; break;
        case 35: if (value < 0 || value > 2) return PAMG_E_ARG; A->lanem_rpw = value; break;
        case 38: if (value != 0 && value != 1 && value != 4 && value != 8) return PAMG_E_ARG; A->lanem_cluster = value; break;
        case 36: if (value < 0 || value > 98304) return PAMG_E_ARG; A->lds_pad = value & ~15; return PAMG_OK;
        case 34: if (value < 1 || value > 400) return PAMG_E_ARG; A->lanem_ahead10 = value; matrix_drop_point_twin(A); return PAMG_OK;
        case 37: if (value < 0 || value > 1) return PAMG_E_ARG; A->sym_fused = value; return PAMG_OK;
        case 39: if (value < 0 || value > 2) return PAMG_E_ARG; A->zero_plans = value; if (value == 1) matrix_drop_zero_plans(A); return PAMG_OK;
        case 40: if (value != 0 && (value < 2 || value > 16)) return PAMG_E_ARG; A->zero_merge = value; matrix_drop_zero_plans(A); return PAMG_OK;
        case 30:
            if (value < 0 || value > 2) return PAMG_E_ARG;
            A->line_scan = value;
            matrix_drop_point_twin(A);
            for (int k = 0; k < 4; ++k) if (A->gs[k]) A->gs[k]->line_unfit = false;
            return PAMG_OK;
        case 31: if (value != 2 && value != 4 && value != 8) return PAMG_E_ARG; A->rowmask_kz = value; return PAMG_OK;
        case 32: if (value < 0 || value > 7) return PAMG_E_ARG; A->rowmask_flags = value; return PAMG_OK;
        case 28: if (value < 0 || value > 15 || (value & 6)) return PAMG_E_ARG; A->lane_flags = value; matrix_drop_point_twin(A); return PAMG_OK;
        default: return PAMG_E_ARG;
    }
    if (key == 25 || key == 33 || key == 35 || key == 38) {
        matrix_drop_point_twin(A);
        matrix_drop_zero_plans(A);
        for (int k = 0; k < 4; ++k) {
            GsSchedule *g = A->gs[k];
            if (g) g->lane_unfit = false;
            if (g && g->lane) { const size_t lb = lane_part_bytes(g); A->bytes -= lb; g->bytes -= lb; free_lane_part(g->lane); g->lane = nullptr; }
            if (g) g->lanem_unfit = false;
            if (g && g->lanem) { const size_t lb = lanem_part_bytes(g); A->bytes -= lb; g->bytes -= lb; free_lanem_part(g->lanem); g->lanem = nullptr; }
            if (g) g->blane_unfit = false;
            if (g && g->blane) { const size_t lb = blane_part_bytes(g); A->bytes -= lb; g->bytes -= lb; free_blane_part(g->blane); g->blane = nullptr; }
            if (g) g->line_unfit = false;
        }
        return PAMG_OK;
    }
    if (key >= 12) {
        for (int k = 0; k < 4; ++k) {
            GsSchedule *g = A->gs[k];
            if (g) g->tile_unfit = false;
            if (g && g->tile) { A->bytes -= g->tile->bytes; g->bytes -= g->tile->bytes; free_tile_part(g->tile); g->tile = nullptr; }
        }
        return PAMG_OK;
    }
    for (int k = 0; k < 4; ++k) { if (A->gs[k]) A->bytes -= A->gs[k]->bytes; free_schedule(A->gs[k]); A->gs[k] = nullptr; }
    matrix_drop_zero_plans(A);
    matrix_drop_point_twin(A);
    return replan(A);
}

int pamg_matrix_autotune(pamg_matrix_t A, int allow_cap)
{
    if (!A) return PAMG_E_ARG;
    if (A->borrowed > 0) return PAMG_E_STATE;
    if (A->nnz < 4000000 || A->npl != 2) return PAMG_OK;
    const size_t ts = tsize(A->dtype);
    void *x = nullptr, *y = nullptr;
    PAMG_HIP(hipMalloc(&x, (size_t)(A->ncols + 8) * ts));
    if (hipMalloc(&y, (size_t)(A->nrows + 8) * ts) != hipSuccess) { hipFree(x); return (int)hipErrorOutOfMemory; }
    hipMemset(x, 0, (size_t)(A->ncols + 8) * ts);
    hipEvent_t e0, e1;
    hipEventCreate(&e0); hipEventCreate(&e1);
    const int cap0 = A->cap, fl0 = A->stream_flags;
    const int caps[2] = {cap0, 512};
    int best_cap = cap0, best_fl = fl0, st = PAMG_OK;
    float best_ms = 1e30f;
    long long rm0[8];
    const bool masked = pamg_matrix_row_masks(A, rm0) == PAMG_OK && rm0[0] > 0;
    const int idx0 = A->use_idx16;
    const int nidx = (A->d_Aj16 && !A->d_Ax8 && idx0) ? 2 : 1;
    const bool square = A->nrows == A->ncols;
    const int probe = square ? EPI_RESID : EPI_SET;
    void *pb = nullptr;
    if (square) {
        if (hipMalloc(&pb, (size_t)(A->nrows + 8) * ts) != hipSuccess) { hipFree(x); hipFree(y); hipEventDestroy(e0); hipEventDestroy(e1); return (int)hipErrorOutOfMemory; }
        hipMemset(pb, 0, (size_t)(A->nrows + 8) * ts);
    }
    float cand_ms[2][2][2][2];
    for (int q = 0; q < 16; ++q) (&cand_ms[0][0][0][0])[q] = 1e30f;
    const int nvc = A->d_Ax8 ? 1 : 2;
    for (int ci = 0; ci < (allow_cap ? 2 : 1) && st == PAMG_OK && !masked; ++ci) {
        if (caps[ci] != A->cap) { A->cap = caps[ci]; st = replan(A); if (st) break; }
        for (int round = 0; round < 2 && st == PAMG_OK; ++round) {
            for (int ix = 0; ix < nidx && st == PAMG_OK; ++ix) {
                A->use_idx16 = ix == 0 ? idx0 : 0;
                for (int fl = 0; fl < 2 && st == PAMG_OK; ++fl)
                    for (int vc = 0; vc < nvc && st == PAMG_OK; ++vc) {
                        A->stream_flags = (fl0 & ~(1 | 32)) | fl | (vc ? 32 : 0);
                        for (int w = 0; w < 2 && st == PAMG_OK; ++w) st = stream_launch(A, probe, x, pb, y, 0.0, 0.0, nullptr, nullptr);
                        hipEventRecord(e0, nullptr);
                        for (int r = 0; r < 6 && st == PAMG_OK; ++r) st = stream_launch(A, probe, x, pb, y, 0.0, 0.0, nullptr, nullptr);
                        hipEventRecord(e1, nullptr);
                        hipEventSynchronize(e1);
// ... 28 lines not shown
        void *bvec = nullptr;
        if (hipMalloc(&bvec, (size_t)(A->nrows + 8) * ts) == hipSuccess) hipMemset(bvec, 0, (size_t)(A->nrows + 8) * ts);
        const int epi_t = bvec ? EPI_RESID : EPI_SET;
        float tmin[9];
        for (int k = 0; k < 9; ++k) tmin[k] = 1e30f;
        for (int round = 0; round < 2 && st == PAMG_OK; ++round)
            for (int kz = 8; kz >= 2 && st == PAMG_OK; kz >>= 1) {
                A->rowmask_kz = kz;
                if (pamg_matrix_row_masks(A, rm) != PAMG_OK || !rm[2]) continue;
                for (int w = 0; w < 2 && st == PAMG_OK; ++w) st = stream_launch(A, epi_t, x, bvec, y, 0.0, 0.0, nullptr, nullptr);
                hipEventRecord(e0, nullptr);
                for (int r = 0; r < 8 && st == PAMG_OK; ++r) st = stream_launch(A, epi_t, x, bvec, y, 0.0, 0.0, nullptr, nullptr);
                hipEventRecord(e1, nullptr);
                hipEventSynchronize(e1);
                float ms = 0.f;
                hipEventElapsedTime(&ms, e0, e1);
                if (st == PAMG_OK) tmin[kz] = std::min(tmin[kz], ms);
            }
        for (int kz = 8; kz >= 2; kz >>= 1)
            if (tmin[kz] < best * 0.98f) { best = tmin[kz]; best_kz = kz; }
        A->rowmask_kz = best_kz;
        if (bvec) hipFree(bvec);
    }
    hipEventDestroy(e0); hipEventDestroy(e1);
    hipFree(x); hipFree(y);
    return st;
}

int pamg_matrix_gs_profile(pamg_matrix_t A, int which, long long *out, int64_t capacity, int64_t *count)
{
    if (!A || which < 0 || which > 3 || !count) return PAMG_E_ARG;
    *count = 0;
    GsSchedule *g = A->gs[which];
    if (g && g->tile && g->tile->d_prof) {
        PAMG_HIP(hipDeviceSynchronize());
        TileSched *t = g->tile;
        *count = t->nsteps;
        if (!out) return PAMG_OK;
        if (capacity < t->nsteps) return PAMG_E_ARG;
        PAMG_HIP(hipMemcpy(out, t->d_prof, (size_t)t->nsteps * 8 * sizeof(long long), hipMemcpyDeviceToHost));
        std::vector<int> ts((size_t)t->G + 1);
        PAMG_HIP(hipMemcpy(ts.data(), t->d_tile_step, ts.size() * sizeof(int), hipMemcpyDeviceToHost));
        for (int k = 0; k < t->G; ++k)
            for (int q = ts[k]; q < ts[k + 1]; ++q) { out[(size_t)q * 8 + 2] = k; out[(size_t)q * 8 + 3] = q - ts[k]; }
        return PAMG_OK;
    }
    if (!g || !g->d_prof) return PAMG_OK;
    PAMG_HIP(hipDeviceSynchronize());
    *count = g->nblk_total;
    if (!out) return PAMG_OK;
    if (capacity < g->nblk_total) return PAMG_E_ARG;
    PAMG_HIP(hipMemcpy(out, g->d_prof, (size_t)g->nblk_total * 8 * sizeof(long long), hipMemcpyDeviceToHost));
    for (int l = 0; l < g->nlevels; ++l)
        for (int q = g->level_blk[l]; q < g->level_blk[l + 1]; ++q) out[(size_t)q * 8 + 7] = l;
    return PAMG_OK;
}

int pamg_matrix_line_info(pamg_matrix_t A, int which, int64_t info[8])
{
    if (!A || which < 0 || which > 3 || !info) return PAMG_E_ARG;
    return pamg::line_info(A->gs[which], info);
}

int pamg_matrix_lane_info(pamg_matrix_t A, int which, int64_t info[8])
{
    if (!A || which < 0 || which > 3 || !info) return PAMG_E_ARG;
    if (A->R > 1) return pamg::blane_info(A->gs[which], info);
    return pamg::lane_info(A->gs[which], info);
}

int pamg_matrix_kz_info(pamg_matrix_t A, int which, int64_t info[8])
{
    if (!A || !info || which < 0 || which > 3) return PAMG_E_ARG;
    return pamg::kz_lane_info(A->ls[which], info);
}

int pamg_matrix_lanem_info(pamg_matrix_t A, int which, int64_t info[20], double *growth)
{
    if (!A || !info || which < 0 || which > 5) return PAMG_E_ARG;
    if (which >= 4) return pamg::lanem_plan_info(A->zplan[which - 4], info, growth);
    return pamg::lanem_info(A->gs[which], info, growth);
}

int pamg_matrix_sym_info(pamg_matrix_t A, int64_t info[8])
{
    if (!A || !info) return PAMG_E_ARG;
    for (int k = 0; k < 8; ++k) info[k] = 0;
    info[0] = A->sym_launches; info[1] = A->sym_zero_launches; info[2] = A->sym_form; info[3] = A->sym_general_grid ? A->sym_general_grid : A->sym_grid; info[4] = A->sym_fused;
    info[5] = -1; info[6] = -1;
    info[7] = A->zero_plan_launches;
    if (!A->d_sym_hf[0]) return PAMG_OK;
    PAMG_HIP(hipDeviceSynchronize());
    unsigned w[8] = {0, 0, 0, 0, 0, 0, 0, 0};
    PAMG_HIP(hipMemcpy(w, A->d_sym_sync, sizeof(w), hipMemcpyDeviceToHost));
    std::vector<unsigned long long> h((size_t)A->nrows);
    if (A->nrows) PAMG_HIP(hipMemcpy(h.data(), A->d_sym_hf[w[5] & 1u], (size_t)A->nrows * 8, hipMemcpyDeviceToHost));
    int64_t bad = 0;
    for (unsigned long long v : h) bad += (v != 0x7FF8DEADBEEF5A5Aull);
    info[5] = bad;
    info[6] = 0;
    for (int k = 0; k < 5; ++k) info[6] += w[k] != 0u;
    return PAMG_OK;
}

int pamg_matrix_lanem_levels(pamg_matrix_t A, int which, int64_t *out, int64_t capacity, int64_t *count)
{
    if (!A || !count || which < 0 || which > 3) return PAMG_E_ARG;
    return pamg::lanem_levels(A->gs[which], out, capacity, count);
}

int pamg_matrix_lane_profile(pamg_matrix_t A, int which, long long *out, int64_t capacity, int64_t *count)
{
    if (!A || which < 0 || which > 3 || !count) return PAMG_E_ARG;
    PAMG_HIP(hipDeviceSynchronize());
    if (A->R > 1) return pamg::blane_profile(A->gs[which], out, capacity, count);
    return pamg::lane_profile(A->gs[which], out, capacity, count);
}

int pamg_matrix_tile_info(pamg_matrix_t A, int which, int64_t info[8])
{
    if (!A || which < 0 || which > 3 || !info) return PAMG_E_ARG;
    for (int k = 0; k < 8; ++k) info[k] = 0;
    const GsSchedule *g = A->gs[which];
    if (!g || !g->tile) return PAMG_OK;
    const TileSched *t = g->tile;
    info[0] = t->G; info[1] = t->W; info[2] = (t->NCH + t->NV + 1) | (t->D << 8) | (TILE_VAR[t->wide][2] << 16) | (t->Q << 24); info[3] = t->nsteps;
    info[4] = t->n_local; info[5] = t->n_global; info[6] = t->n_publish; info[7] = t->lds;
    return PAMG_OK;
}

int pamg_matrix_kaczmarz(pamg_matrix_t L, int nr, void *v, const void *b, const void *Dinv, double omega, int sweep,
                         int iterations, void *xout, pamg_stream_t s)
{
    if (!L || iterations < 0 || sweep < PAMG_FORWARD || sweep > PAMG_SYMMETRIC) return PAMG_E_ARG;
    const int n = (int)L->nrows;
    if (n == 0) return PAMG_OK;
    for (int it = 0; it < iterations; ++it) {
        if (sweep != PAMG_BACKWARD) PAMG_TRY(pamg::kaczmarz_sweep(L, nr != 0, v, b, Dinv, omega, 0, n, 1, xout, (hipStream_t)s));
        if (sweep != PAMG_FORWARD) PAMG_TRY(pamg::kaczmarz_sweep(L, nr != 0, v, b, Dinv, omega, n - 1, -1, -1, xout, (hipStream_t)s));
    }
    return PAMG_OK;
}

int pamg_vec_mul(int dtype, int64_t n, const void *a, const void *b, void *y, pamg_stream_t s)
{
    if (dtype != PAMG_F64 && dtype != PAMG_F32) return PAMG_E_ARG;
    return pamg::vec_mul(dtype, n, a, b, y, (hipStream_t)s);
}

int pamg_matrix_subset_rows(pamg_matrix_t A, const int32_t *rows, int nrows, pamg_matrix_t *sub)
{
    return pamg::matrix_row_subset(A, rows, nrows, sub);
}

int pamg_matrix_jacobi_indexed(pamg_matrix_t sub, void *x, const void *b, double omega, void *work, pamg_stream_t s)
{
    return pamg::jacobi_indexed(sub, x, b, omega, work, (hipStream_t)s);
}

int pamg_matrix_flow_error(pamg_matrix_t A, int *error)
{
    if (!A || !error) return PAMG_E_ARG;
    *error = 0;
    PAMG_HIP(hipDeviceSynchronize());
    bool e = false;
    PAMG_TRY(pamg::sweep_error(A, &e));
    *error = e ? 1 : 0;
    return PAMG_OK;
}

int pamg_matrix_spmv(pamg_matrix_t A, int mode, const void *x, const void *b_or_v, double c, void *y,
                     pamg_stream_t s)
{
// ... 82 lines not shown
```

pyamg_amd/csrc/pamg_solver.hip:

```cpp
#include <algorithm>
#include <cmath>
#include <functional>
#include <map>
#include <new>
#include <thread>

#include "pamg_common.h"

using namespace pamg;

namespace {

struct Smoother {
    int kind = PAMG_SMOOTH_NONE;
    int iterations = 1;
    double omega = 1.0;
    int sweep = PAMG_FORWARD;
    std::vector<double> coeffs;
    void *d_Dinv = nullptr;
    int blocksize = 1;
    pamg_matrix_s *AF = nullptr, *AC = nullptr;
    void *wF = nullptr, *wC = nullptr;
    int f_iterations = 1, c_iterations = 1;
    int *iF = nullptr, *iC = nullptr;
    int64_t nF = 0, nC = 0;
    pamg_schwarz_s *sw = nullptr;
    pamg_matrix_s *At = nullptr, *Ar = nullptr;
    int kmethod = 0, kmaxiter = 1, krestart = 0;
    double ktol = 1e-12;
    void *kw = nullptr;
};

struct Level {
    pamg_matrix_s *A = nullptr, *P = nullptr, *R = nullptr;
    Smoother pre, post;
    int64_t n = 0;
    void *x = nullptr, *xalt = nullptr;
    void *x_home = nullptr;
    void *b = nullptr, *r = nullptr, *work = nullptr;
    void *amli = nullptr;
};

int sweep_bounds(const pamg_matrix_s *A, int dir, int &r0, int &r1, int &rs)
{
    const int n = A->R > 1 ? A->n_brow : (int)A->nrows;
    if (dir == PAMG_FORWARD) { r0 = 0; r1 = n; rs = 1; }
    else if (dir == PAMG_BACKWARD) { r0 = n - 1; r1 = -1; rs = -1; }
    else return PAMG_E_ARG;
    return PAMG_OK;
}

bool square_ok(const pamg_matrix_s *A) { return A && A->nrows == A->ncols && A->R == A->C; }

int jacobi_pp(pamg_matrix_s *A, void **px, void **palt, const void *b, double omega, int its, hipStream_t s)
{
    if (!square_ok(A)) return PAMG_E_ARG;
    if (A->nrows == 0) return PAMG_OK;
    for (int it = 0; it < its; ++it) {
        if (A->R > 1)
            PAMG_TRY(block_jacobi_step(A, PNT_JACOBI, nullptr, *px, *palt, b, omega, s));
        else
            PAMG_TRY(stream_launch(A, A->flavour == PAMG_BSR ? EPI_JACOBI_B : EPI_JACOBI, *px, b, *palt,
                                   0.0, omega, nullptr, s));
        std::swap(*px, *palt);
    }
    return PAMG_OK;
}

int block_jacobi_pp(pamg_matrix_s *A, void **px, void **palt, const void *b, const void *Dinv,
                    double omega, int its, hipStream_t s)
{
    if (!square_ok(A) || A->R < 2 || !Dinv) return PAMG_E_ARG;
    for (int it = 0; it < its; ++it) {
        PAMG_TRY(block_jacobi_step(A, BLK_JACOBI, Dinv, *px, *palt, b, omega, s));
        std::swap(*px, *palt);
    }
    return PAMG_OK;
}

int gs_apply(pamg_matrix_s *A, void *x, const void *b, int sweep, double omega, int its, hipStream_t s, bool x_zero = false)
{
    if (!square_ok(A)) return PAMG_E_ARG;
    if (A->nrows == 0) return PAMG_OK;
    auto one = [&](int dir, double om) -> int {
        int r0, r1, rs;
        PAMG_TRY(sweep_bounds(A, dir, r0, r1, rs));
        int epi;
        if (A->R > 1 || A->flavour == PAMG_BSR) epi = EPI_GS_B;
        else epi = (om != 1.0) ? EPI_SOR : EPI_GS;
        return gs_sweep(A, epi, x, b, om, r0, r1, rs, s);
    };
    if (sweep == PAMG_SYMMETRIC) {
        for (int it = 0; it < its; ++it) {
            bool ran = false;
            PAMG_TRY(gs_sweep_symmetric(A, x, b, x_zero && it == 0, s, &ran));
            if (ran) continue;
            if (x_zero && it == 0) PAMG_TRY(gs_sweep_zero_pair(A, x, b, s, &ran));
            if (ran) continue;
            PAMG_TRY(one(PAMG_FORWARD, 1.0));
            PAMG_TRY(one(PAMG_BACKWARD, 1.0));
        }
        return PAMG_OK;
    }
    for (int it = 0; it < its; ++it) PAMG_TRY(one(sweep, omega));
    return PAMG_OK;
}

int block_gs_apply(pamg_matrix_s *A, void *x, const void *b, const void *Dinv, int sweep, int its,
                   hipStream_t s)
{
    if (!square_ok(A) || A->R < 2 || !Dinv) return PAMG_E_ARG;
    auto one = [&](int dir) -> int {
        int r0, r1, rs;
        PAMG_TRY(sweep_bounds(A, dir, r0, r1, rs));
        return block_gs_sweep(A, x, b, Dinv, r0, r1, rs, s);
    };
    for (int it = 0; it < its; ++it) {
        if (sweep == PAMG_SYMMETRIC) { PAMG_TRY(one(PAMG_FORWARD)); PAMG_TRY(one(PAMG_BACKWARD)); }
        else PAMG_TRY(one(sweep));
    }
    return PAMG_OK;
}

int poly_apply(pamg_matrix_s *A, void *x, const void *b, void *work, const double *coeffs, int nc,
               int its, int x_is_zero, hipStream_t s)
{
    if (!A || A->nrows != A->ncols || nc < 1 || !coeffs) return PAMG_E_ARG;
    const int64_t n = A->nrows;
    if (n == 0) return PAMG_OK;
    const size_t ts = tsize(A->dtype);
    void *res_buf = work, *h0 = (char *)work + n * ts, *h1 = (char *)work + 2 * n * ts;
    for (int it = 0; it < its; ++it) {
        const void *res = b;
        bool have_h = false;
        if (!(x_is_zero && it == 0)) {
            PAMG_TRY(stream_launch(A, EPI_RESID, x, b, res_buf, nc > 1 ? coeffs[0] : 0.0, 0.0, nc > 1 ? (double *)h0 : nullptr, s));
            res = res_buf;
            have_h = nc > 1;
        }
        if (nc == 1) {
            PAMG_TRY(vec_axpy(A->dtype, n, coeffs[0], res, x, s));
            continue;
        }
        if (!have_h) PAMG_TRY(vec_scale(A->dtype, n, coeffs[0], res, h0, s));
        void *hc = h0, *hn = h1;
        for (int k = 1; k < nc - 1; ++k) {
            PAMG_TRY(stream_launch(A, EPI_AXPBY, hc, res, hn, coeffs[k], 0.0, nullptr, s));
            std::swap(hc, hn);
        }
        PAMG_TRY(stream_launch(A, EPI_ACC_AXPBY, hc, res, x, coeffs[nc - 1], 0.0, nullptr, s));
    }
    return PAMG_OK;
}

}

struct pamg_solver_s {
    int dtype = PAMG_F64;
    std::vector<Level> levels;
    void *d_coarse = nullptr;
    int n_c = 0;
    bool coarse_set = false, coarse_zero = false, coarse_relax = false;
    pamg_coarse_host_fn coarse_host = nullptr;
    void *coarse_host_user = nullptr;
    std::vector<unsigned char> coarse_hb, coarse_hx;
    bool finalized = false;
    bool use_graph = true;
    hipStream_t own_stream = nullptr;
    double *d_norms = nullptr;
    int norms_cap = 0;
    double *d_slot = nullptr;
    double *d_scratch = nullptr;
    void *cg_r = nullptr, *cg_z = nullptr, *cg_p = nullptr, *cg_q = nullptr;
    void *kr_v[5] = {nullptr, nullptr, nullptr, nullptr, nullptr};
    double *kr_red = nullptr;
    std::map<int, hipGraphExec_t> graphs;
    bool host_sync = false;
    int fallbacks = 0;
    size_t bytes = 0;
};

namespace {

int krylov_smooth(pamg_solver_s *S, Level &L, const Smoother &sm, hipStream_t s);

int apply_smoother(pamg_solver_s *S, Level &L, const Smoother &sm, bool x_zero, hipStream_t s)
{
    switch (sm.kind) {
        case PAMG_SMOOTH_NONE: return PAMG_OK;
        case PAMG_SMOOTH_JACOBI: return jacobi_pp(L.A, &L.x, &L.xalt, L.b, sm.omega, sm.iterations, s);
        case PAMG_SMOOTH_GS: return gs_apply(L.A, L.x, L.b, sm.sweep, 1.0, sm.iterations, s, x_zero);
        case PAMG_SMOOTH_SOR: return gs_apply(L.A, L.x, L.b, sm.sweep, sm.omega, sm.iterations, s, x_zero);
        case PAMG_SMOOTH_POLY:
            return poly_apply(L.A, L.x, L.b, L.work, sm.coeffs.data(), (int)sm.coeffs.size(),
                              sm.iterations, x_zero ? 1 : 0, s);
        case PAMG_SMOOTH_BLOCK_JACOBI:
            return block_jacobi_pp(L.A, &L.x, &L.xalt, L.b, sm.d_Dinv, sm.omega, sm.iterations, s);
        case PAMG_SMOOTH_BLOCK_GS:
            return block_gs_apply(L.A, L.x, L.b, sm.d_Dinv, sm.sweep, sm.iterations, s);
        case PAMG_SMOOTH_GS_NE: {
            const int n = (int)L.A->nrows;
            for (int it = 0; it < sm.iterations; ++it) {
                pamg_matrix_s *Ak = sm.Ar ? sm.Ar : L.A;
                if (sm.sweep != PAMG_BACKWARD) PAMG_TRY(kaczmarz_sweep(Ak, false, L.x, L.b, sm.d_Dinv, sm.omega, 0, n, 1, nullptr, s));
                if (sm.sweep != PAMG_FORWARD) PAMG_TRY(kaczmarz_sweep(Ak, false, L.x, L.b, sm.d_Dinv, sm.omega, n - 1, -1, -1, nullptr, s));
            }
            return PAMG_OK;
        }
        case PAMG_SMOOTH_GS_NR: {
            const int n = (int)L.A->nrows;
            auto call = [&](bool fwd, int its) -> int {
                PAMG_TRY(stream_launch(sm.Ar ? sm.Ar : L.A, EPI_RESID, L.x, L.b, L.r, 0.0, 0.0, nullptr, s));
                for (int k = 0; k < its; ++k)
                    PAMG_TRY(kaczmarz_sweep(sm.At, true, L.r, nullptr, sm.d_Dinv, sm.omega, fwd ? 0 : n - 1, fwd ? n : -1, fwd ? 1 : -1, L.x, s));
                return PAMG_OK;
            };
            if (sm.sweep == PAMG_SYMMETRIC) {
                for (int it = 0; it < sm.iterations; ++it) { PAMG_TRY(call(true, 1)); PAMG_TRY(call(false, 1)); }
                return PAMG_OK;
            }
            return call(sm.sweep == PAMG_FORWARD, sm.iterations);
        }
        case PAMG_SMOOTH_JACOBI_NE:
            for (int it = 0; it < sm.iterations; ++it) {
                PAMG_TRY(stream_launch(sm.Ar ? sm.Ar : L.A, EPI_RESID, L.x, L.b, L.r, 0.0, 0.0, nullptr, s));
                PAMG_TRY(vec_mul(S->dtype, L.n, L.r, sm.d_Dinv, L.r, s));
                PAMG_TRY(stream_launch(sm.At, EPI_ACC, L.r, nullptr, L.x, 0.0, 0.0, nullptr, s));
            }
            return PAMG_OK;
        case PAMG_SMOOTH_CF_JACOBI:
        case PAMG_SMOOTH_FC_JACOBI:
            for (int it = 0; it < sm.iterations; ++it) {
                const bool f_first = sm.kind == PAMG_SMOOTH_FC_JACOBI;
                for (int half = 0; half < 2; ++half) {
                    const bool f = (half == 0) == f_first;
                    pamg_matrix_s *sub = f ? sm.AF : sm.AC;
                    void *w = f ? sm.wF : sm.wC;
                    const int reps = f ? sm.f_iterations : sm.c_iterations;
                    for (int k = 0; k < reps; ++k) PAMG_TRY(jacobi_indexed(sub, L.x, L.b, sm.omega, w, s));
                }
            }
            return PAMG_OK;
        case PAMG_SMOOTH_KRYLOV: return krylov_smooth(S, L, sm, s);
        case PAMG_SMOOTH_SCHWARZ: {
            int nsub = 0;
            { int64_t info[4]; PAMG_TRY(pamg_schwarz_info(sm.sw, info)); nsub = (int)info[0]; }
            for (int it = 0; it < sm.iterations; ++it) {
                if (sm.sweep != PAMG_BACKWARD) PAMG_TRY(schwarz_sweep(sm.sw, L.x, L.b, 0, nsub, 1, s));
                if (sm.sweep != PAMG_FORWARD) PAMG_TRY(schwarz_sweep(sm.sw, L.x, L.b, nsub - 1, -1, -1, s));
            }
            return PAMG_OK;
        }
        case PAMG_SMOOTH_CF_BLOCK_JACOBI:
        case PAMG_SMOOTH_FC_BLOCK_JACOBI:
            for (int it = 0; it < sm.iterations; ++it) {
                const bool f_first = sm.kind == PAMG_SMOOTH_FC_BLOCK_JACOBI;
                for (int half = 0; half < 2; ++half) {
                    const bool f = (half == 0) == f_first;
                    const int reps = f ? sm.f_iterations : sm.c_iterations;
                    for (int k = 0; k < reps; ++k) {
                        PAMG_TRY(block_jacobi_step(L.A, BLK_JACOBI, sm.d_Dinv, L.x, L.xalt, L.b, sm.omega, s));
                        PAMG_TRY(vec_copy_indexed(S->dtype, f ? sm.nF : sm.nC, f ? sm.iF : sm.iC, L.xalt, L.x, s));
                    }
                }
            }
            return PAMG_OK;
    }
    (void)S;
    return PAMG_E_ARG;
}

void drop_graphs(pamg_solver_s *S);
int prebuild_schedules(Level &L, const Smoother &sm, bool zero = false);

int check_sweeps(pamg_solver_s *S)
// ... 815 lines not shown
{
    const int64_t n = L.n;
    if (n == 0) return PAMG_OK;
    const size_t ts = tsize(S->dtype);
    unsigned char *kw = (unsigned char *)sm.kw;
    void *w0 = kw, *w1 = kw + (size_t)n * ts, *w2 = kw + 2 * (size_t)n * ts, *w3 = kw + 3 * (size_t)n * ts;
    int it = 0, inf = 0;
    switch (sm.kmethod) {
        case PAMG_KRYLOV_CG:
            return cg_core(S, L.A, n, nullptr, w0, w0, w1, w2, L.x, L.b, sm.ktol, sm.kmaxiter, nullptr, &it, &inf, s);
        case PAMG_KRYLOV_CGNE:
            return cgn_core(S, false, L.A, sm.At, n, w0, w3, w1, w2, L.x, L.b, sm.ktol, sm.kmaxiter, &it, &inf, s);
        case PAMG_KRYLOV_CGNR:
            return cgn_core(S, true, L.A, sm.At, n, w0, w3, w1, w2, L.x, L.b, sm.ktol, sm.kmaxiter, &it, &inf, s);
        case PAMG_KRYLOV_GMRES: {
            int nres = 0;
            return krylov_householder(S, L.A, n, false, L.x, L.b, sm.ktol, sm.kmaxiter, sm.krestart, -1, 1, nullptr, 0, &nres, &it, &inf, s);
        }
    }
    return PAMG_E_ARG;
}

}

extern "C" {

int pamg_matrix_jacobi(pamg_matrix_t A, void *x, const void *b, void *work, double omega, int iterations,
                       pamg_stream_t s)
{
    if (!A || !x || !b || !work || iterations < 0) return PAMG_E_ARG;
    void *cur = x, *alt = work;
    PAMG_TRY(jacobi_pp(A, &cur, &alt, b, omega, iterations, (hipStream_t)s));
    if (cur != x)
        PAMG_HIP(hipMemcpyAsync(x, cur, (size_t)A->nrows * tsize(A->dtype), hipMemcpyDeviceToDevice, (hipStream_t)s));
    return PAMG_OK;
}

int pamg_matrix_jacobi_step(pamg_matrix_t A, const void *x_in, const void *b, void *x_out, double omega,
                            pamg_stream_t s)
{
    if (!A || !x_in || !b || !x_out) return PAMG_E_ARG;
    if (A->R != A->C || A->ncols < A->nrows) return PAMG_E_UNSUPPORTED;
    if (A->nrows == 0) return PAMG_OK;
    if (A->R > 1) return block_jacobi_step(A, PNT_JACOBI, nullptr, x_in, x_out, b, omega, (hipStream_t)s);
    return stream_launch(A, A->flavour == PAMG_BSR ? EPI_JACOBI_B : EPI_JACOBI, x_in, b, x_out, 0.0, omega,
                         nullptr, (hipStream_t)s);
}

int pamg_matrix_block_jacobi_step(pamg_matrix_t A, const void *Dinv, const void *x_in, const void *b, void *x_out,
                                  double omega, pamg_stream_t s)
{
    if (!A || !Dinv || !x_in || !b || !x_out) return PAMG_E_ARG;
    if (A->R != A->C || A->R < 2 || A->ncols < A->nrows) return PAMG_E_UNSUPPORTED;
    if (A->nrows == 0) return PAMG_OK;
    return block_jacobi_step(A, BLK_JACOBI, Dinv, x_in, x_out, b, omega, (hipStream_t)s);
}

int pamg_matrix_block_jacobi_indexed(pamg_matrix_t A, const void *Dinv, void *x, const void *b, const int32_t *idx,
                                     int64_t nidx, double omega, void *work, pamg_stream_t s)
{
    if (!A || !Dinv || !x || !b || !work || nidx < 0 || (nidx > 0 && !idx)) return PAMG_E_ARG;
    if (A->R != A->C || A->R < 2 || A->ncols != A->nrows) return PAMG_E_UNSUPPORTED;
    if (A->nrows == 0 || nidx == 0) return PAMG_OK;
    PAMG_TRY(block_jacobi_step(A, BLK_JACOBI, Dinv, x, work, b, omega, (hipStream_t)s));
    return vec_copy_indexed(A->dtype, nidx, idx, work, x, (hipStream_t)s);
}

int pamg_matrix_gauss_seidel(pamg_matrix_t A, void *x, const void *b, int sweep, double omega,
                             int iterations, pamg_stream_t s)
{
    if (!A || !x || !b || iterations < 0) return PAMG_E_ARG;
    if (sweep < PAMG_FORWARD || sweep > PAMG_SYMMETRIC) return PAMG_E_ARG;
    return gs_apply(A, x, b, sweep, omega, iterations, (hipStream_t)s);
}

int pamg_matrix_gauss_seidel_x0(pamg_matrix_t A, void *x, const void *b, int sweep, double omega,
                                int iterations, int x_is_zero, pamg_stream_t s)
{
    if (!A || !x || !b || iterations < 0) return PAMG_E_ARG;
    if (sweep < PAMG_FORWARD || sweep > PAMG_SYMMETRIC) return PAMG_E_ARG;
    return gs_apply(A, x, b, sweep, omega, iterations, (hipStream_t)s, x_is_zero != 0);
}

int pamg_matrix_polynomial(pamg_matrix_t A, void *x, const void *b, void *work, const double *coeffs,
                           int ncoeffs, int iterations, int x_is_zero, pamg_stream_t s)
{
    if (!A || !x || !b || !work || iterations < 0) return PAMG_E_ARG;
    return poly_apply(A, x, b, work, coeffs, ncoeffs, iterations, x_is_zero, (hipStream_t)s);
}

int pamg_matrix_block_jacobi(pamg_matrix_t A, void *x, const void *b, void *work, const void *Dinv,
                             double omega, int iterations, pamg_stream_t s)
{
    if (!A || !x || !b || !work || iterations < 0) return PAMG_E_ARG;
    void *cur = x, *alt = work;
    PAMG_TRY(block_jacobi_pp(A, &cur, &alt, b, Dinv, omega, iterations, (hipStream_t)s));
    if (cur != x)
        PAMG_HIP(hipMemcpyAsync(x, cur, (size_t)A->nrows * tsize(A->dtype), hipMemcpyDeviceToDevice, (hipStream_t)s));
    return PAMG_OK;
}

int pamg_matrix_block_gauss_seidel(pamg_matrix_t A, void *x, const void *b, const void *Dinv, int sweep,
                                   int iterations, pamg_stream_t s)
{
    if (!A || !x || !b || iterations < 0) return PAMG_E_ARG;
    if (sweep < PAMG_FORWARD || sweep > PAMG_SYMMETRIC) return PAMG_E_ARG;
    return block_gs_apply(A, x, b, Dinv, sweep, iterations, (hipStream_t)s);
}

int pamg_solver_create(pamg_solver_t *S, int dtype)
{
    if (!S) return PAMG_E_ARG;
    if (dtype != PAMG_F64 && dtype != PAMG_F32) return PAMG_E_UNSUPPORTED;
    pamg_solver_s *p = new (std::nothrow) pamg_solver_s();
    if (!p) return PAMG_E_ALLOC;
    p->dtype = dtype;
    *S = p;
    return PAMG_OK;
}

int pamg_solver_destroy(pamg_solver_t S)
{
    if (!S) return PAMG_OK;
    drop_graphs(S);
    for (Level &L : S->levels) {
        if (L.A) L.A->borrowed--;
        if (L.P) L.P->borrowed--;
        if (L.R) L.R->borrowed--;
        hipFree(L.x); hipFree(L.xalt);
        hipFree(L.b); hipFree(L.r); hipFree(L.work); hipFree(L.amli);
        hipFree(L.pre.d_Dinv); hipFree(L.post.d_Dinv);
        for (Smoother *sm : {&L.pre, &L.post}) {
            if (sm->AF) pamg_matrix_destroy(sm->AF);
            if (sm->AC) pamg_matrix_destroy(sm->AC);
            hipFree(sm->wF); hipFree(sm->wC); hipFree(sm->iF); hipFree(sm->iC); hipFree(sm->kw);
            if (sm->sw) pamg_schwarz_destroy(sm->sw);
        }
    }
    hipFree(S->d_coarse); hipFree(S->d_norms); hipFree(S->d_slot); hipFree(S->d_scratch);
    hipFree(S->cg_r); hipFree(S->cg_z); hipFree(S->cg_p); hipFree(S->cg_q);
    for (void *v : S->kr_v) hipFree(v);
    hipFree(S->kr_red);
    if (S->own_stream) hipStreamDestroy(S->own_stream);
    delete S;
    return PAMG_OK;
}

int pamg_solver_add_level(pamg_solver_t S, pamg_matrix_t A, pamg_matrix_t P, pamg_matrix_t R)
{
    if (!S || !A) return PAMG_E_ARG;
    if (S->finalized) return PAMG_E_STATE;
    if (A->dtype != S->dtype || A->nrows != A->ncols) return PAMG_E_ARG;
    if ((P == nullptr) != (R == nullptr)) return PAMG_E_ARG;
    if (!S->levels.empty()) {
        const Level &prev = S->levels.back();
        if (!prev.P) return PAMG_E_STATE;
        if (prev.P->ncols != A->nrows || prev.R->nrows != A->nrows) return PAMG_E_ARG;
    }
    if (P && (P->dtype != S->dtype || R->dtype != S->dtype || P->nrows != A->nrows || R->ncols != A->nrows ||
              P->ncols != R->nrows))
        return PAMG_E_ARG;
    Level L;
    L.A = A; L.P = P; L.R = R; L.n = A->nrows;
    S->levels.push_back(L);
    A->borrowed++;
    if (P) P->borrowed++;
// ... 559 lines not shown
```

pyamg_amd/multilevel.py:

```python
from __future__ import annotations

import ctypes as C
from typing import List, Optional

import numpy as np

from . import _capi as capi
from .hierarchy import HierarchySpec, SmootherSpec, SparseOp, extract

__all__ = ["DeviceMatrix", "DeviceMultilevelSolver"]


class DeviceMatrix:

    def __init__(self, op: SparseOp):
        lib = capi.lib()
        self.op = op
        self.dtype = np.dtype(op.dtype)
        R, Cc = op.blocksize
        h = C.c_void_p()
        capi.check(lib.pamg_matrix_create(
            C.byref(h), capi.dtype_code(op.dtype), capi.BSR if op.fmt == "bsr" else capi.CSR,
            op.shape[0] // R, op.shape[1] // Cc, R, Cc,
            capi.ptr(op.indptr), capi.ptr(op.indices), capi.ptr(op.data)), "pamg_matrix_create")
# ... 20 lines not shown
        return sub

    def kaczmarz(self, v, Dinv, omega, sweep="forward", iterations=1, b=None, xout=None, stream=None):
        nr = xout is not None
        capi.check(capi.lib().pamg_matrix_kaczmarz(self.handle, int(nr), v.ptr, b.ptr if b is not None else None, Dinv.ptr,
                                                   float(omega), capi.SWEEP[sweep], int(iterations),
                                                   xout.ptr if nr else None, stream), "pamg_matrix_kaczmarz")

    def jacobi_indexed(self, x, b, omega, work, stream=None):
        capi.check(capi.lib().pamg_matrix_jacobi_indexed(self.handle, x.ptr, b.ptr, float(omega), work.ptr, stream),
                   "pamg_matrix_jacobi_indexed")

    def flow_error(self) -> bool:
        e = C.c_int(0)
        capi.check(capi.lib().pamg_matrix_flow_error(self.handle, C.byref(e)), "pamg_matrix_flow_error")
        return bool(e.value)

    def gs_profile(self, which=0):
        import numpy as np
        n = C.c_int64(0)
        lib = capi.lib()
        capi.check(lib.pamg_matrix_gs_profile(self.handle, which, None, 0, C.byref(n)), "pamg_matrix_gs_profile")
        out = np.zeros((n.value, 8), dtype=np.int64)
        if n.value:
            capi.check(lib.pamg_matrix_gs_profile(self.handle, which, C.c_void_p(out.ctypes.data), n.value, C.byref(n)),
                       "pamg_matrix_gs_profile")
        return out

    def value_codes(self) -> int:
        n = C.c_int(0)
        capi.check(capi.lib().pamg_matrix_value_codes(self.handle, C.byref(n)), "pamg_matrix_value_codes")
        return int(n.value)

    def row_patterns(self) -> int:
        n = C.c_int(0)
        capi.check(capi.lib().pamg_matrix_row_patterns(self.handle, C.byref(n)), "pamg_matrix_row_patterns")
        return int(n.value)

    def row_masks(self) -> dict:
        out = (C.c_longlong * 8)()
        capi.check(capi.lib().pamg_matrix_row_masks(self.handle, out), "pamg_matrix_row_masks")
        keys = ("entries", "walked_rows", "lattice", "line", "plane", "planes_per_lane", "flags", "launch_grid")
        return dict(zip(keys, (int(v) for v in out)))

    def tile_info(self, which=0):
        a = (C.c_int64 * 8)()
        capi.check(capi.lib().pamg_matrix_tile_info(self.handle, which, a), "pamg_matrix_tile_info")
        d = dict(zip(("tiles", "ring", "geom", "steps", "early_local", "early_global", "publishing_rows", "lds_bytes"), list(a)))
        geom = d.pop("geom")
        d.update(code_chunks=geom & 0xFF, lds_slots=(geom >> 8) & 0xFF, gather_depth=(geom >> 16) & 0xFF, loader_in_flight=(geom >> 24) & 0xFF)
        return d

    def lane_info(self, which=0):
        a = (C.c_int64 * 8)()
        capi.check(capi.lib().pamg_matrix_lane_info(self.handle, which, a), "pamg_matrix_lane_info")
        return dict(zip(("lanes_per_row", "slots_per_lane", "groups", "entry_slots", "early_entries", "launch_grid", "widest_level_groups", "bytes"), list(a)))

    def lanem_info(self, which=0):
        a = (C.c_int64 * 20)()
        gr = C.c_double(0.0)
        capi.check(capi.lib().pamg_matrix_lanem_info(self.handle, which, a, C.byref(gr)), "pamg_matrix_lanem_info")
        d = dict(zip(("super_levels", "dependency_levels", "rows", "units", "early_operands", "old_operands", "b_operands", "longest_row", "s_max",
                      "closed_by_length", "closed_by_growth", "launch_grid", "cluster_rows", "groups", "padded_slots", "unique_units",
                      "unique_early", "unique_old", "unique_b", "early_lines"), list(a)))
        d["max_growth"] = gr.value
        d["padding"] = d["padded_slots"] / max(1, d["early_operands"] + d["old_operands"] + d["b_operands"])
        return d

    def point_twin(self) -> int:
        st = C.c_int(0)
        capi.check(capi.lib().pamg_matrix_point_twin(self.handle, C.byref(st)), "pamg_matrix_point_twin")
        return int(st.value)

    def lanem_levels(self, which=0):
        n = C.c_int64(0)
        lib = capi.lib()
        capi.check(lib.pamg_matrix_lanem_levels(self.handle, which, None, 0, C.byref(n)), "pamg_matrix_lanem_levels")
        out = np.zeros(n.value, dtype=np.int64)
        if n.value:
            capi.check(lib.pamg_matrix_lanem_levels(self.handle, which, C.c_void_p(out.ctypes.data), n.value, C.byref(n)), "pamg_matrix_lanem_levels")
        return out

    def sym_info(self):
        a = (C.c_int64 * 8)()
        capi.check(capi.lib().pamg_matrix_sym_info(self.handle, a), "pamg_matrix_sym_info")
        d = dict(zip(("launches", "zero_launches", "form", "launch_grid", "enabled", "handoff_not_sentinel", "counters_not_zero", "zero_plan_launches"), list(a)))
        d["form"] = {0: "none", 1: "merged", 2: "line", 3: "merged_one_xcd"}[d["form"]]
        return d

    def line_info(self, which=0):
        a = (C.c_int64 * 8)()
        capi.check(capi.lib().pamg_matrix_line_info(self.handle, which, a), "pamg_matrix_line_info")
        return dict(zip(("slots_per_row", "chunks", "lines", "line_levels", "early_entries", "launch_grid", "widest_level_lines", "bytes"), list(a)))

    def kz_info(self, which=0):
        a = (C.c_int64 * 8)()
        capi.check(capi.lib().pamg_matrix_kz_info(self.handle, which, a), "pamg_matrix_kz_info")
        return dict(zip(("lanes_per_line", "slots_per_lane", "groups", "dependency_levels", "widest_level_groups", "launch_grid", "bytes"), list(a)[:7]))

    def lane_profile(self, which=0):
        n = C.c_int64(0)
        lib = capi.lib()
        capi.check(lib.pamg_matrix_lane_profile(self.handle, which, None, 0, C.byref(n)), "pamg_matrix_lane_profile")
        out = np.zeros((n.value, 4), dtype=np.int64)
        if n.value:
            capi.check(lib.pamg_matrix_lane_profile(self.handle, which, C.c_void_p(out.ctypes.data), n.value, C.byref(n)), "pamg_matrix_lane_profile")
        return out

    def tune(self, lds_entries=None, nnz_per_lane=None, max_rows=None, flow_cap=None, gs_mode=None, gran_cap=None, gran_xcd=None, stream_flags=None, gs_prof=None,
             tile_G=None, tile_W=None, tile_cap=None, tile_default=None, tile_D=None, tile_Q=None, tile_part=None, idx16=None, gs_cap=None, val8=None, rowgather=None, rowpat=None,
             gs_order=None, lane_L=None, lane_G=None, lane_wide=None, lane_flags=None, line_scan=None, rowmask_kz=None, rowmask_flags=None, lane_merge=None, lanem_ahead=None, lanem_rpw=None, lds_pad=None, sym_fused=None, lanem_cluster=None, zero_plans=None, zero_merge=None):
        lib = capi.lib()
        for key, v in ((0, lds_entries), (1, nnz_per_lane), (2, max_rows), (3, flow_cap), (5, gs_mode), (6, gran_cap), (7, gran_xcd), (8, stream_flags), (11, gs_prof),
                       (12, tile_G), (13, tile_W), (14, tile_cap), (15, tile_default), (16, tile_D), (17, tile_Q), (18, tile_part), (19, idx16), (20, gs_cap), (21, val8), (22, rowgather), (23, rowpat),
                       (24, gs_order), (25, lane_L), (26, lane_G), (27, lane_wide), (28, lane_flags), (30, line_scan), (31, rowmask_kz), (32, rowmask_flags), (33, lane_merge), (34, lanem_ahead), (35, lanem_rpw), (36, lds_pad), (37, sym_fused), (38, lanem_cluster), (39, zero_plans), (40, zero_merge)):
            if v is not None:
                capi.check(lib.pamg_matrix_tune(self.handle, key, int(v)), "pamg_matrix_tune")

    def spmv(self, mode, x, y, b=None, c=0.0, stream=None, part=None):
        if part is not None:
            capi.check(capi.lib().pamg_matrix_spmv_part(self.handle, int(part), mode, x.ptr, b.ptr if b is not None else None,
                                                        float(c), y.ptr, stream), "pamg_matrix_spmv_part")
            return
        capi.check(capi.lib().pamg_matrix_spmv(self.handle, mode, x.ptr, b.ptr if b is not None else None,
                                               float(c), y.ptr, stream), "pamg_matrix_spmv")

    def split_ranges(self, n_owned_cols: int):
        capi.check(capi.lib().pamg_matrix_split_ranges(self.handle, int(n_owned_cols)), "pamg_matrix_split_ranges")

    def resid_sumsq(self, x, b, out, stream=None):
        capi.check(capi.lib().pamg_matrix_resid_sumsq(self.handle, x.ptr, b.ptr, out.ptr, stream),
                   "pamg_matrix_resid_sumsq")

    def jacobi(self, x, b, work, omega, iterations=1, stream=None):
        capi.check(capi.lib().pamg_matrix_jacobi(self.handle, x.ptr, b.ptr, work.ptr, float(omega),
                                                 int(iterations), stream), "pamg_matrix_jacobi")

    def gauss_seidel(self, x, b, sweep="forward", omega=1.0, iterations=1, stream=None):
        capi.check(capi.lib().pamg_matrix_gauss_seidel(self.handle, x.ptr, b.ptr, capi.SWEEP[sweep],
                                                       float(omega), int(iterations), stream),
                   "pamg_matrix_gauss_seidel")

    def gauss_seidel_x0(self, x, b, sweep="symmetric", omega=1.0, iterations=1, x_is_zero=False, stream=None):
        capi.check(capi.lib().pamg_matrix_gauss_seidel_x0(self.handle, x.ptr, b.ptr, capi.SWEEP[sweep], float(omega), int(iterations),
                                                          int(bool(x_is_zero)), stream), "pamg_matrix_gauss_seidel_x0")

    def polynomial(self, x, b, work, coefficients, iterations=1, x_is_zero=False, stream=None):
        co = np.ascontiguousarray(coefficients, dtype=np.float64)
        capi.check(capi.lib().pamg_matrix_polynomial(self.handle, x.ptr, b.ptr, work.ptr, capi.ptr(co),
                                                     co.size, int(iterations), int(bool(x_is_zero)), stream),
                   "pamg_matrix_polynomial")

    def block_jacobi(self, x, b, work, Dinv, omega, iterations=1, stream=None):
        capi.check(capi.lib().pamg_matrix_block_jacobi(self.handle, x.ptr, b.ptr, work.ptr, Dinv.ptr,
                                                       float(omega), int(iterations), stream),
                   "pamg_matrix_block_jacobi")

    def block_gauss_seidel(self, x, b, Dinv, sweep="forward", iterations=1, stream=None):
        capi.check(capi.lib().pamg_matrix_block_gauss_seidel(self.handle, x.ptr, b.ptr, Dinv.ptr,
                                                             capi.SWEEP[sweep], int(iterations), stream),
                   "pamg_matrix_block_gauss_seidel")

    def free(self):
        if getattr(self, "handle", None):
            try:
                capi._lib.pamg_matrix_destroy(self.handle)
            except Exception:
                pass
            self.handle = None

    def __del__(self):
        self.free()


def _set_smoother(lib, S, level, which, s: Optional[SmootherSpec], dtype, aux, fast=False):
    if s is None or s.kind == "none":
        capi.check(lib.pamg_solver_set_smoother(S, level, which, 0, 0, 1.0, 0, None, 0, None, 1), "set_smoother")
        return
    if s.kind in ("gauss_seidel_ne", "gauss_seidel_nr", "jacobi_ne"):
        Dinv = np.ascontiguousarray(s.Dinv, dtype=dtype)
        At = None
        if s.At is not None:
            At = DeviceMatrix(s.At)
            aux.append(At)
        Ar = None
        if getattr(s, "Ar", None) is not None:
            Ar = DeviceMatrix(s.Ar)
            aux.append(Ar)
        if fast:
            for m_ in (At, Ar):
                if m_ is not None:
                    m_.tune(gs_order=1)
        capi.check(lib.pamg_solver_set_ne_smoother(S, level, which, capi.SMOOTH[s.kind], int(s.iterations), float(s.omega),
                                                   capi.SWEEP.get(s.sweep, 0), capi.ptr(Dinv), At.handle if At else None,
                                                   Ar.handle if Ar else None),
                   f"pamg_solver_set_ne_smoother({s.kind})")
        return
    if s.kind in capi.KRYLOV:
        At = None
        if s.At is not None:
            At = DeviceMatrix(s.At)
            aux.append(At)
        capi.check(lib.pamg_solver_set_krylov_smoother(S, level, which, capi.KRYLOV[s.kind], float(s.tol), int(s.iterations),
                                                       int(s.restart), At.handle if At else None),
                   f"pamg_solver_set_krylov_smoother({s.kind})")
        return
    if s.kind in ("cf_jacobi", "fc_jacobi"):
        F = np.ascontiguousarray(s.Fpts, dtype=np.int32)
        Cp = np.ascontiguousarray(s.Cpts, dtype=np.int32)
        capi.check(lib.pamg_solver_set_cf_smoother(S, level, which, capi.SMOOTH[s.kind], int(s.iterations),
                                                   int(s.f_iterations), int(s.c_iterations), float(s.omega),
                                                   capi.ptr(F), F.size, capi.ptr(Cp), Cp.size),
                   f"pamg_solver_set_cf_smoother({s.kind})")
        return
    if s.kind == "schwarz":
        Ar = None
        if getattr(s, "Ar", None) is not None:
            Ar = DeviceMatrix(s.Ar)
            aux.append(Ar)
        Sp, Sj = np.ascontiguousarray(s.subdomain_ptr, dtype=np.int32), np.ascontiguousarray(s.subdomain, dtype=np.int32)
        Tp, Tx = np.ascontiguousarray(s.inv_subblock_ptr, dtype=np.int32), np.ascontiguousarray(s.inv_subblock, dtype=dtype)
        capi.check(lib.pamg_solver_set_schwarz_smoother(S, level, which, int(s.iterations), capi.SWEEP.get(s.sweep, 0),
                                                        Ar.handle if Ar else None, Sp.size - 1, capi.ptr(Sp), capi.ptr(Sj),
                                                        capi.ptr(Tp), capi.ptr(Tx)),
# ... 450 lines not shown
```

Measured before the change: 91.00 cycles/s.

## Run nonzero-guess symmetric Gauss-Seidel as residual correction using zero-guess plans

Adds a correction form of symmetric Gauss-Seidel for sweeps with a nonzero initial guess. It computes r = b - Ax, runs the specialised zero-initial-guess lane plans (fused or as a pair) on r, and accumulates the result into x via a new ACC template path. The aim is to reuse the cheaper zero-guess schedules, which skip reading x_old, for post-smoothing and later iterations. The cost is an extra residual SpMV, a memset and a read-modify-write of x. The path is on by default for levels with at least 16384 rows.

```diff
diff --git a/include/pyamg_amd.h b/include/pyamg_amd.h
--- a/include/pyamg_amd.h
+++ b/include/pyamg_amd.h
@@ -265,7 +265,8 @@
                              int iterations, pamg_stream_t s);
 int pamg_matrix_gauss_seidel_x0(pamg_matrix_t A, void *x, const void *b, int sweep, double omega,
                                 int iterations, int x_is_zero, pamg_stream_t s);
-int pamg_matrix_sym_info(pamg_matrix_t A, int64_t info[8]);
+int pamg_matrix_sym_info(pamg_matrix_t A, int64_t info[9]);
+int pamg_matrix_gauss_seidel_correction(pamg_matrix_t A, void *x, const void *b, void *r, int iterations, pamg_stream_t s);
 int pamg_matrix_polynomial(pamg_matrix_t A, void *x, const void *b, void *work,
                            const double *coeffs, int ncoeffs, int iterations, int x_is_zero,
                            pamg_stream_t s);
diff --git a/pyamg_amd/_capi.py b/pyamg_amd/_capi.py
--- a/pyamg_amd/_capi.py
+++ b/pyamg_amd/_capi.py
@@ -150,6 +150,7 @@
     f("pamg_solver_set_cf_block_smoother", _vp, _i, _i, _i, _i, _i, _i, _d, _vp, _i, _vp, _i, _vp, _i)
     f("pamg_matrix_gauss_seidel", _vp, _vp, _vp, _i, _d, _i, _vp)
     f("pamg_matrix_gauss_seidel_x0", _vp, _vp, _vp, _i, _d, _i, _i, _vp)
+    f("pamg_matrix_gauss_seidel_correction", _vp, _vp, _vp, _vp, _i, _vp)
     f("pamg_matrix_sym_info", _vp, P(C.c_int64))
     f("pamg_matrix_polynomial", _vp, _vp, _vp, _vp, _vp, _i, _i, _i, _vp)
     f("pamg_matrix_block_jacobi", _vp, _vp, _vp, _vp, _vp, _d, _i, _vp)
diff --git a/pyamg_amd/csrc/pamg_common.h b/pyamg_amd/csrc/pamg_common.h
--- a/pyamg_amd/csrc/pamg_common.h
+++ b/pyamg_amd/csrc/pamg_common.h
@@ -227,6 +227,8 @@
     const void *sym_cap_kernel = nullptr;
     int zsym_cap = 0;
     const void *zsym_cap_kernel = nullptr;
+    int csym_cap = 0;
+    const void *csym_cap_kernel = nullptr;
     int sym_general_grid = 0;
     int sym_form = 0, sym_grid = 0;
     long long sym_launches = 0, sym_zero_launches = 0;
@@ -236,6 +238,8 @@
     void *d_zw = nullptr;
     size_t zero_bytes = 0;
     long long zero_plan_launches = 0;
+    int gs_correction = 0;
+    long long correction_launches = 0;
     size_t bytes = 0;
 };
 
@@ -346,16 +350,18 @@
 size_t lanem_part_bytes(const GsSchedule *g);
 int lanem_info(const GsSchedule *g, int64_t *info, double *growth);
 int lanem_levels(const GsSchedule *g, int64_t *out, int64_t cap, int64_t *n);
-int lanem_sym_launch(pamg_matrix_s *A, GsSchedule *gf, GsSchedule *gb, void *x, const void *b, bool x_zero, hipStream_t s);
+int lanem_sym_launch(pamg_matrix_s *A, GsSchedule *gf, GsSchedule *gb, void *x, const void *b, bool x_zero, hipStream_t s, bool acc = false);
 int lanem_plan_info(const struct LaneMSched *t, int64_t *info, double *growth);
 int build_zero_plan(pamg_matrix_s *A, int dir);
 void free_zero_plans(pamg_matrix_s *A);
 size_t zero_plan_bytes(const pamg_matrix_s *A);
 bool zero_plans_ready(const pamg_matrix_s *A, const GsSchedule *gf, const GsSchedule *gb);
-int lanem_zero_pair_launch(pamg_matrix_s *A, GsSchedule *gf, GsSchedule *gb, void *x, const void *b, hipStream_t s);
+int lanem_zero_pair_launch(pamg_matrix_s *A, GsSchedule *gf, GsSchedule *gb, void *x, const void *b, bool acc, hipStream_t s);
 int ensure_zero_parts(pamg_matrix_s *A, bool build);
 void matrix_drop_zero_plans(pamg_matrix_s *A);
 int gs_sweep_zero_pair(pamg_matrix_s *A, void *x, const void *b, hipStream_t s, bool *ran);
+int gs_sweep_correction(pamg_matrix_s *A, void *x, const void *b, void *r, bool force, hipStream_t s, bool *ran);
+constexpr int64_t GS_CORRECTION_MIN_ROWS = 16384;
 int sym_fill_sentinels(void *p, int64_t n);
 int sweep_error(pamg_matrix_s *A, bool *error);
 inline size_t tsize(int dtype) { return dtype == PAMG_F64 ? 8 : 4; }
diff --git a/pyamg_amd/csrc/pamg_lane.hip b/pyamg_amd/csrc/pamg_lane.hip
--- a/pyamg_amd/csrc/pamg_lane.hip
+++ b/pyamg_amd/csrc/pamg_lane.hip
@@ -396,7 +396,7 @@
     }
 }
 
-template <int NREG, bool BCOH = false>
+template <int NREG, bool BCOH = false, bool XOZ = false>
 __device__ __forceinline__ void m_gather(const LaneMArgs &a, MCtx<NREG> &C, int idle, const bool xz = false, const bool coh = false)
 {
 #pragma unroll
@@ -410,7 +410,8 @@
     const int row = C.rid < 0 ? 0 : (C.rid & LANE_MASK);
     if constexpr (BCOH) C.bv = __hip_atomic_load(a.b + row, __ATOMIC_RELAXED, __HIP_MEMORY_SCOPE_AGENT);
     else C.bv = a.b[row];
-    C.xo = coh ? __hip_atomic_load(a.xold + row, __ATOMIC_RELAXED, __HIP_MEMORY_SCOPE_AGENT) : a.xold[row];
+    if constexpr (XOZ) C.xo = 0.0;
+    else C.xo = coh ? __hip_atomic_load(a.xold + row, __ATOMIC_RELAXED, __HIP_MEMORY_SCOPE_AGENT) : a.xold[row];
 #pragma unroll
     for (int k = 0; k < NREG; ++k) {
         const int col = C.c[k] & LANEM_MASK;
@@ -496,7 +497,7 @@
     return val;
 }
 
-template <int RPW, int MODE, int NREG, int PH = 0, bool WST = false>
+template <int RPW, int MODE, int NREG, int PH = 0, bool WST = false, bool ACC = false>
 __device__ __forceinline__ void m_publish(const LaneMArgs &a, const MCtx<NREG> &C, double val)
 {
     if (((threadIdx.x & 63) & (64 / RPW - 1)) == 0 && C.rid >= 0) {
@@ -504,7 +505,10 @@
         if constexpr (MODE == 1) __hip_atomic_store(a.xs + row, val, __ATOMIC_RELAXED, __HIP_MEMORY_SCOPE_WORKGROUP);
         else __hip_atomic_store(a.xs + row, val, __ATOMIC_RELAXED, __HIP_MEMORY_SCOPE_AGENT);
         if constexpr (PH != 1) {
-            if (!(C.rid & LANE_NODIAG)) a.y[row] = val;
+            if (!(C.rid & LANE_NODIAG)) {
+                if constexpr (ACC) a.y[row] = a.y[row] + val;
+                else a.y[row] = val;
+            }
         }
         if constexpr (WST) {
             if (!(C.rid & LANE_NODIAG)) __hip_atomic_store(a.w + row, C.num, __ATOMIC_RELAXED, __HIP_MEMORY_SCOPE_AGENT);
@@ -516,7 +520,7 @@
 
 __device__ __forceinline__ int4 c_rec(const int4 *rp, int g, int gend) { return rp[(size_t)(g < gend ? g : gend - 1)]; }
 
-template <int PH, bool WST = false, bool BCOH = false>
+template <int PH, bool WST = false, bool BCOH = false, bool ACC = false>
 __device__ __forceinline__ void c_group(const LaneMArgs &a, double *lds, const int4 &q, int g, int lane, int idle, const bool xz, const bool coh)
 {
     using T = double;
@@ -560,7 +564,8 @@
     T bv;
     if constexpr (BCOH) bv = __hip_atomic_load(a.b + row, __ATOMIC_RELAXED, __HIP_MEMORY_SCOPE_AGENT);
     else bv = a.b[row];
-    const T xo = coh ? __hip_atomic_load(a.xold + row, __ATOMIC_RELAXED, __HIP_MEMORY_SCOPE_AGENT) : a.xold[row];
+    T xo = T(0);
+    if constexpr (!(ACC && PH == 1)) xo = coh ? __hip_atomic_load(a.xold + row, __ATOMIC_RELAXED, __HIP_MEMORY_SCOPE_AGENT) : a.xold[row];
     unsigned pend = 0;
 #pragma unroll
     for (int k = 0; k < LANEC_K; ++k)
@@ -627,7 +632,10 @@
     if (tail && rid >= 0) {
         __hip_atomic_store(a.xs + row, val, __ATOMIC_RELAXED, __HIP_MEMORY_SCOPE_AGENT);
         if constexpr (PH != 1) {
-            if (upd) a.y[row] = val;
+            if (upd) {
+                if constexpr (ACC) a.y[row] = a.y[row] + val;
+                else a.y[row] = val;
+            }
         }
         if constexpr (WST) {
             if (upd) __hip_atomic_store(a.w + row, num, __ATOMIC_RELAXED, __HIP_MEMORY_SCOPE_AGENT);
@@ -652,7 +660,7 @@
         int4 q = c_rec(rp, g, gend);
         for (; g < gend; g += W) {
             const int4 nq = c_rec(rp, g + W, gend);
-            c_group<0, Z != 0>(a, c_lds + wib * LANEC_UMAX, q, g, lane, idle, false, false);
+            c_group<0, Z == 1, false, Z == 2>(a, c_lds + wib * LANEC_UMAX, q, g, lane, idle, false, false);
             q = nq;
         }
     } else {
@@ -675,7 +683,7 @@
                 long long t2 = 0;
                 unsigned sp = 0;
                 const double val = m_finish<RPW, NREG>(a, X, idle, &t2, &sp);
-                m_publish<RPW, MODE, NREG, 0, Z != 0>(a, X, val);
+                m_publish<RPW, MODE, NREG, 0, Z == 1, Z == 2>(a, X, val);
                 if (lane == 0) {
                     long long *o = a.prof + (size_t)g * 4;
                     o[0] = t0 | ((long long)(sp > 4095u ? 4095u : sp) << 52);
@@ -685,7 +693,7 @@
                 m_slots<RPW, NREG>(a, X, q0, q1, g, lane);
                 m_gather<NREG>(a, X, idle);
                 const double val = m_finish<RPW, NREG>(a, X, idle);
-                m_publish<RPW, MODE, NREG, 0, Z != 0>(a, X, val);
+                m_publish<RPW, MODE, NREG, 0, Z == 1, Z == 2>(a, X, val);
             }
             q0 = n0; q1 = n1;
         }
@@ -715,7 +723,7 @@
             m_slots<RPW, NREG>(a, X, q0, q1, g, lane);
             m_gather<NREG>(a, X, idle);
             const double val = m_finish<RPW, NREG>(a, X, idle);
-            m_publish<RPW, MODE, NREG, 0, Z != 0>(a, X, val);
+            m_publish<RPW, MODE, NREG, 0, Z == 1, Z == 2>(a, X, val);
             if (g2 >= gend) break;
             g = g2; q0 = n0; q1 = n1;
             g2 = (int)__builtin_amdgcn_readfirstlane(tk3);
@@ -759,7 +767,7 @@
         int4 q = c_rec(rp, g, gend);
         for (; g < gend; g += W) {
             const int4 nq = c_rec(rp, g + W, gend);
-            c_group<PH, Z && PH == 1, Z && PH == 2>(a, c_lds + wib * LANEC_UMAX, q, g, lane, idle, xz, PH == 2);
+            c_group<PH, Z && PH == 1, Z && PH == 2, Z == 2>(a, c_lds + wib * LANEC_UMAX, q, g, lane, idle, xz, PH == 2);
             m_wipe<MODE>(wipe, g, gend, wq, wr, wblk, lane);
             ++done;
             q = nq;
@@ -776,9 +784,9 @@
             int4 n0, n1;
             m_rec(rp, g + W, gend, n0, n1);
             m_slots<RPW, NREG>(a, X, q0, q1, g, lane);
-            m_gather<NREG, Z && PH == 2>(a, X, idle, xz, PH == 2);
+            m_gather<NREG, Z && PH == 2, Z == 2 && PH == 1>(a, X, idle, xz, PH == 2);
             const double val = m_finish<RPW, NREG>(a, X, idle, nullptr, nullptr, xz);
-            m_publish<RPW, MODE, NREG, PH, Z && PH == 1>(a, X, val);
+            m_publish<RPW, MODE, NREG, PH, Z && PH == 1, Z == 2 && PH == 2>(a, X, val);
             m_wipe<MODE>(wipe, g, gend, wq, wr, wblk, lane);
             ++done;
             q0 = n0; q1 = n1;
@@ -798,9 +806,9 @@
             unsigned tk3 = 0;
             if (g2 < gend && lane == 0) tk3 = __hip_atomic_fetch_add(ticket, 1u, __ATOMIC_RELAXED, __HIP_MEMORY_SCOPE_AGENT);
             m_slots<RPW, NREG>(a, X, q0, q1, g, lane);
-            m_gather<NREG, Z && PH == 2>(a, X, idle, xz, PH == 2);
+            m_gather<NREG, Z && PH == 2, Z == 2 && PH == 1>(a, X, idle, xz, PH == 2);
             const double val = m_finish<RPW, NREG>(a, X, idle, nullptr, nullptr, xz);
-            m_publish<RPW, MODE, NREG, PH, Z && PH == 1>(a, X, val);
+            m_publish<RPW, MODE, NREG, PH, Z && PH == 1, Z == 2 && PH == 2>(a, X, val);
             m_wipe<MODE>(wipe, g, gend, wq, wr, wblk, lane);
             ++done;
             if (g2 >= gend) break;
@@ -1253,7 +1261,7 @@
     a.sidx = t->d_sidx; a.crid = t->d_crid; a.crd = t->d_crd; a.crows = t->cluster;
 }
 
-static int lanem_launch_plan(pamg_matrix_s *A, GsSchedule *g, LaneMSched *t, void *x, const void *b, double *w, hipStream_t s)
+static int lanem_launch_plan(pamg_matrix_s *A, GsSchedule *g, LaneMSched *t, void *x, const void *b, double *w, hipStream_t s, bool acc = false)
 {
     if (!t || !g->d_xold) return PAMG_E_STATE;
     const int64_t n = A->nrows;
@@ -1271,7 +1279,8 @@
     }
     a.prof = (A->gs_prof && !t->cluster) ? t->d_prof : nullptr;
     const int fgrid = (int)std::min<int64_t>(4096, (n + BLK - 1) / BLK);
-    hipLaunchKernelGGL(lanem_prepare_kernel, dim3(fgrid), dim3(BLK), 0, s, (const double *)x, (double *)g->d_xold, (double *)g->d_xs, n);
+    if (acc) hipLaunchKernelGGL((lane_fill_sentinel_kernel<double>), dim3(fgrid), dim3(BLK), 0, s, (double *)g->d_xs, n);
+    else hipLaunchKernelGGL(lanem_prepare_kernel, dim3(fgrid), dim3(BLK), 0, s, (const double *)x, (double *)g->d_xold, (double *)g->d_xs, n);
     PAMG_HIP(hipGetLastError());
     const bool xcd = !t->cluster && (A->gran_xcd == 1 || (A->gran_xcd == 0 && lane_one_xcd(A, g) && A->nrows <= 8192));
     static const int nreg_env = [] { const char *e = getenv("PAMG_LANEM_NREG"); return e ? atoi(e) : 0; }();
@@ -1285,6 +1294,11 @@
           : t->rpw == 2 ? (xcd ? (const void *)gs_lanem_kernel<1, 2, 4, 1> : (const void *)gs_lanem_kernel<0, 2, 4, 1>)
           : all_regs    ? (xcd ? (const void *)gs_lanem_kernel<1, 1, 8, 1> : (const void *)gs_lanem_kernel<0, 1, 8, 1>)
                         : (xcd ? (const void *)gs_lanem_kernel<1, 1, 2, 1> : (const void *)gs_lanem_kernel<0, 1, 2, 1>);
+    if (acc)
+        k = t->cluster  ? (const void *)gs_lanem_kernel<0, 0, 8, 2>
+          : t->rpw == 2 ? (xcd ? (const void *)gs_lanem_kernel<1, 2, 4, 2> : (const void *)gs_lanem_kernel<0, 2, 4, 2>)
+          : all_regs    ? (xcd ? (const void *)gs_lanem_kernel<1, 1, 8, 2> : (const void *)gs_lanem_kernel<0, 1, 8, 2>)
+                        : (xcd ? (const void *)gs_lanem_kernel<1, 1, 2, 2> : (const void *)gs_lanem_kernel<0, 1, 2, 2>);
     static thread_local int cus = 0;
     if (!cus) cus = device_cus_lane();
     if (!(t->cap > 0 && t->cap_kernel == k)) {
@@ -1315,11 +1329,18 @@
 
 int lanem_launch(pamg_matrix_s *A, GsSchedule *g, void *x, const void *b, hipStream_t s) { return lanem_launch_plan(A, g, g->lanem, x, b, nullptr, s); }
 
-int lanem_zero_pair_launch(pamg_matrix_s *A, GsSchedule *gf, GsSchedule *gb, void *x, const void *b, hipStream_t s)
+int lanem_zero_pair_launch(pamg_matrix_s *A, GsSchedule *gf, GsSchedule *gb, void *x, const void *b, bool acc, hipStream_t s)
 {
     if (!zero_plans_ready(A, gf, gb)) return PAMG_E_UNSUPPORTED;
-    PAMG_TRY(lanem_launch_plan(A, gf, A->zplan[0], x, b, (double *)A->d_zw, s));
-    PAMG_TRY(lanem_launch_plan(A, gb, A->zplan[1], x, A->d_zw, nullptr, s));
+    if (acc) {
+        if (!gb->d_xold) return PAMG_E_STATE;
+        PAMG_HIP(hipMemsetAsync(gb->d_xold, 0, (size_t)A->nrows * sizeof(double), s));
+        PAMG_TRY(lanem_launch_plan(A, gf, A->zplan[0], gb->d_xold, b, (double *)A->d_zw, s));
+        PAMG_TRY(lanem_launch_plan(A, gb, A->zplan[1], x, A->d_zw, nullptr, s, true));
+    } else {
+        PAMG_TRY(lanem_launch_plan(A, gf, A->zplan[0], x, b, (double *)A->d_zw, s));
+        PAMG_TRY(lanem_launch_plan(A, gb, A->zplan[1], x, A->d_zw, nullptr, s));
+    }
     A->zero_plan_launches++;
     return PAMG_OK;
 }
@@ -1334,10 +1355,12 @@
     return PAMG_OK;
 }
 
-int lanem_sym_launch(pamg_matrix_s *A, GsSchedule *gf, GsSchedule *gb, void *x, const void *b, bool x_zero, hipStream_t s)
+int lanem_sym_launch(pamg_matrix_s *A, GsSchedule *gf, GsSchedule *gb, void *x, const void *b, bool x_zero, hipStream_t s, bool acc)
 {
     LaneMSched *tf = gf->lanem, *tb = gb->lanem;
     if (!tf || !tb || !A->d_sym_hf[0] || !A->d_sym_hf[1] || !A->d_sym_hb || !A->d_sym_sync) return PAMG_E_STATE;
+    if (acc && !zero_plans_ready(A, gf, gb)) return PAMG_E_UNSUPPORTED;
+    if (acc) x_zero = true;
     const bool zero = x_zero && zero_plans_ready(A, gf, gb);
     if (zero) { tf = A->zplan[0]; tb = A->zplan[1]; }
     const int64_t n = A->nrows;
@@ -1378,10 +1401,15 @@
           : tf->rpw == 2 ? (xcd ? (const void *)gs_lanem_sym_kernel<1, 2, 4, 1> : (const void *)gs_lanem_sym_kernel<0, 2, 4, 1>)
           : all_regs     ? (xcd ? (const void *)gs_lanem_sym_kernel<1, 1, 8, 1> : (const void *)gs_lanem_sym_kernel<0, 1, 8, 1>)
                          : (xcd ? (const void *)gs_lanem_sym_kernel<1, 1, 2, 1> : (const void *)gs_lanem_sym_kernel<0, 1, 2, 1>);
+    if (acc)
+        k = tf->cluster  ? (const void *)gs_lanem_sym_kernel<0, 0, 8, 2>
+          : tf->rpw == 2 ? (xcd ? (const void *)gs_lanem_sym_kernel<1, 2, 4, 2> : (const void *)gs_lanem_sym_kernel<0, 2, 4, 2>)
+          : all_regs     ? (xcd ? (const void *)gs_lanem_sym_kernel<1, 1, 8, 2> : (const void *)gs_lanem_sym_kernel<0, 1, 8, 2>)
+                         : (xcd ? (const void *)gs_lanem_sym_kernel<1, 1, 2, 2> : (const void *)gs_lanem_sym_kernel<0, 1, 2, 2>);
     static thread_local int cus = 0;
     if (!cus) cus = device_cus_lane();
-    int &kcap = zero ? A->zsym_cap : A->sym_cap;
-    const void *&kcap_kernel = zero ? A->zsym_cap_kernel : A->sym_cap_kernel;
+    int &kcap = acc ? A->csym_cap : zero ? A->zsym_cap : A->sym_cap;
+    const void *&kcap_kernel = acc ? A->csym_cap_kernel : zero ? A->zsym_cap_kernel : A->sym_cap_kernel;
     if (!(kcap > 0 && kcap_kernel == k)) {
         int nb = 0;
         if (hipOccupancyMaxActiveBlocksPerMultiprocessor(&nb, k, BLK, 0) != hipSuccess) nb = 2;
diff --git a/pyamg_amd/csrc/pamg_matrix.hip b/pyamg_amd/csrc/pamg_matrix.hip
--- a/pyamg_amd/csrc/pamg_matrix.hip
+++ b/pyamg_amd/csrc/pamg_matrix.hip
@@ -1404,10 +1404,41 @@
         PAMG_TRY(ensure_zero_parts(A, true));
         if (!zero_plans_ready(A, gf, gb)) { A->zero_plans = 1; return PAMG_OK; }
     }
-    const int st = lanem_zero_pair_launch(A, gf, gb, x, b, s);
+    const int st = lanem_zero_pair_launch(A, gf, gb, x, b, false, s);
     if (st == PAMG_E_UNSUPPORTED) return PAMG_OK;
     if (st == PAMG_OK) *ran = true;
     return st;
+}
+
+int gs_sweep_correction(pamg_matrix_s *A, void *x, const void *b, void *r, bool force, hipStream_t s, bool *ran)
+{
+    *ran = false;
+    if (!r || A->zero_plans == 1) return PAMG_OK;
+    if (!force && (A->gs_correction == 1 || (A->gs_correction == 0 && A->nrows < GS_CORRECTION_MIN_ROWS))) return PAMG_OK;
+    if (!A->zplan[0] || !A->zplan[1] || !A->d_zw) {
+        if (!force || A->zero_plans != 2 || A->zplan[0] || A->zplan[1]) return PAMG_OK;
+        hipStreamCaptureStatus cs = hipStreamCaptureStatusNone;
+        PAMG_HIP(hipStreamIsCapturing(s, &cs));
+        if (cs != hipStreamCaptureStatusNone) return PAMG_OK;
+        PAMG_TRY(ensure_zero_parts(A, true));
+    }
+    GsSchedule *gf = nullptr, *gb = nullptr;
+    if (!zero_form_of(A, &gf, &gb) || !zero_plans_ready(A, gf, gb)) return PAMG_OK;
+    GsSchedule *sf = nullptr, *sb = nullptr;
+    bool fused = sym_form_of(A, &sf, &sb) == 1;
+    if (fused && !A->d_sym_hf[0]) {
+        hipStreamCaptureStatus cs = hipStreamCaptureStatusNone;
+        PAMG_HIP(hipStreamIsCapturing(s, &cs));
+        if (cs == hipStreamCaptureStatusNone) PAMG_TRY(ensure_sym_parts(A));
+        fused = A->d_sym_hf[0] != nullptr;
+    }
+    PAMG_TRY(stream_launch(A, EPI_RESID, x, b, r, 0.0, 0.0, nullptr, s));
+    int st = fused ? lanem_sym_launch(A, gf, gb, x, r, true, s, true) : PAMG_E_UNSUPPORTED;
+    if (st == PAMG_E_UNSUPPORTED) st = lanem_zero_pair_launch(A, gf, gb, x, r, true, s);
+    if (st != PAMG_OK) return st;
+    A->correction_launches++;
+    *ran = true;
+    return PAMG_OK;
 }
 
 int ensure_schedule(pamg_matrix_s *A, int row_start, int row_stop, int row_step, bool block_gs)
@@ -1975,6 +2006,7 @@
         case 37: if (value < 0 || value > 1) return PAMG_E_ARG; A->sym_fused = value; return PAMG_OK;
         case 39: if (value < 0 || value > 2) return PAMG_E_ARG; A->zero_plans = value; if (value == 1) matrix_drop_zero_plans(A); return PAMG_OK;
         case 40: if (value != 0 && (value < 2 || value > 16)) return PAMG_E_ARG; A->zero_merge = value; matrix_drop_zero_plans(A); return PAMG_OK;
+        case 41: if (value < 0 || value > 2) return PAMG_E_ARG; A->gs_correction = value; return PAMG_OK;
         case 30:
             if (value < 0 || value > 2) return PAMG_E_ARG;
             A->line_scan = value;
@@ -2169,13 +2201,14 @@
     return pamg::lanem_info(A->gs[which], info, growth);
 }
 
-int pamg_matrix_sym_info(pamg_matrix_t A, int64_t info[8])
+int pamg_matrix_sym_info(pamg_matrix_t A, int64_t info[9])
 {
     if (!A || !info) return PAMG_E_ARG;
-    for (int k = 0; k < 8; ++k) info[k] = 0;
+    for (int k = 0; k < 9; ++k) info[k] = 0;
     info[0] = A->sym_launches; info[1] = A->sym_zero_launches; info[2] = A->sym_form; info[3] = A->sym_general_grid ? A->sym_general_grid : A->sym_grid; info[4] = A->sym_fused;
     info[5] = -1; info[6] = -1;
     info[7] = A->zero_plan_launches;
+    info[8] = A->correction_launches;
     if (!A->d_sym_hf[0]) return PAMG_OK;
     PAMG_HIP(hipDeviceSynchronize());
     unsigned w[8] = {0, 0, 0, 0, 0, 0, 0, 0};
diff --git a/pyamg_amd/csrc/pamg_solver.hip b/pyamg_amd/csrc/pamg_solver.hip
--- a/pyamg_amd/csrc/pamg_solver.hip
+++ b/pyamg_amd/csrc/pamg_solver.hip
@@ -78,7 +78,7 @@
     return PAMG_OK;
 }
 
-int gs_apply(pamg_matrix_s *A, void *x, const void *b, int sweep, double omega, int its, hipStream_t s, bool x_zero = false)
+int gs_apply(pamg_matrix_s *A, void *x, const void *b, int sweep, double omega, int its, hipStream_t s, bool x_zero = false, void *r = nullptr)
 {
     if (!square_ok(A)) return PAMG_E_ARG;
     if (A->nrows == 0) return PAMG_OK;
@@ -93,6 +93,8 @@
     if (sweep == PAMG_SYMMETRIC) {
         for (int it = 0; it < its; ++it) {
             bool ran = false;
+            if (r && !(x_zero && it == 0)) PAMG_TRY(gs_sweep_correction(A, x, b, r, false, s, &ran));
+            if (ran) continue;
             PAMG_TRY(gs_sweep_symmetric(A, x, b, x_zero && it == 0, s, &ran));
             if (ran) continue;
             if (x_zero && it == 0) PAMG_TRY(gs_sweep_zero_pair(A, x, b, s, &ran));
@@ -189,8 +191,8 @@
     switch (sm.kind) {
         case PAMG_SMOOTH_NONE: return PAMG_OK;
         case PAMG_SMOOTH_JACOBI: return jacobi_pp(L.A, &L.x, &L.xalt, L.b, sm.omega, sm.iterations, s);
-        case PAMG_SMOOTH_GS: return gs_apply(L.A, L.x, L.b, sm.sweep, 1.0, sm.iterations, s, x_zero);
-        case PAMG_SMOOTH_SOR: return gs_apply(L.A, L.x, L.b, sm.sweep, sm.omega, sm.iterations, s, x_zero);
+        case PAMG_SMOOTH_GS: return gs_apply(L.A, L.x, L.b, sm.sweep, 1.0, sm.iterations, s, x_zero, L.r);
+        case PAMG_SMOOTH_SOR: return gs_apply(L.A, L.x, L.b, sm.sweep, sm.omega, sm.iterations, s, x_zero, L.r);
         case PAMG_SMOOTH_POLY:
             return poly_apply(L.A, L.x, L.b, L.work, sm.coeffs.data(), (int)sm.coeffs.size(),
                               sm.iterations, x_zero ? 1 : 0, s);
@@ -1172,6 +1174,18 @@
     return gs_apply(A, x, b, sweep, omega, iterations, (hipStream_t)s, x_is_zero != 0);
 }
 
+int pamg_matrix_gauss_seidel_correction(pamg_matrix_t A, void *x, const void *b, void *r, int iterations, pamg_stream_t s)
+{
+    if (!A || !x || !b || !r || iterations < 0) return PAMG_E_ARG;
+    if (!square_ok(A)) return PAMG_E_ARG;
+    for (int it = 0; it < iterations; ++it) {
+        bool ran = false;
+        PAMG_TRY(gs_sweep_correction(A, x, b, r, true, (hipStream_t)s, &ran));
+        if (!ran) return PAMG_E_UNSUPPORTED;
+    }
+    return PAMG_OK;
+}
+
 int pamg_matrix_polynomial(pamg_matrix_t A, void *x, const void *b, void *work, const double *coeffs,
                            int ncoeffs, int iterations, int x_is_zero, pamg_stream_t s)
 {
diff --git a/pyamg_amd/multilevel.py b/pyamg_amd/multilevel.py
--- a/pyamg_amd/multilevel.py
+++ b/pyamg_amd/multilevel.py
@@ -126,9 +126,9 @@
         return out
 
     def sym_info(self):
-        a = (C.c_int64 * 8)()
+        a = (C.c_int64 * 9)()
         capi.check(capi.lib().pamg_matrix_sym_info(self.handle, a), "pamg_matrix_sym_info")
-        d = dict(zip(("launches", "zero_launches", "form", "launch_grid", "enabled", "handoff_not_sentinel", "counters_not_zero", "zero_plan_launches"), list(a)))
+        d = dict(zip(("launches", "zero_launches", "form", "launch_grid", "enabled", "handoff_not_sentinel", "counters_not_zero", "zero_plan_launches", "correction_launches"), list(a)))
         d["form"] = {0: "none", 1: "merged", 2: "line", 3: "merged_one_xcd"}[d["form"]]
         return d
 
@@ -153,11 +153,11 @@
 
     def tune(self, lds_entries=None, nnz_per_lane=None, max_rows=None, flow_cap=None, gs_mode=None, gran_cap=None, gran_xcd=None, stream_flags=None, gs_prof=None,
              tile_G=None, tile_W=None, tile_cap=None, tile_default=None, tile_D=None, tile_Q=None, tile_part=None, idx16=None, gs_cap=None, val8=None, rowgather=None, rowpat=None,
-             gs_order=None, lane_L=None, lane_G=None, lane_wide=None, lane_flags=None, line_scan=None, rowmask_kz=None, rowmask_flags=None, lane_merge=None, lanem_ahead=None, lanem_rpw=None, lds_pad=None, sym_fused=None, lanem_cluster=None, zero_plans=None, zero_merge=None):
+             gs_order=None, lane_L=None, lane_G=None, lane_wide=None, lane_flags=None, line_scan=None, rowmask_kz=None, rowmask_flags=None, lane_merge=None, lanem_ahead=None, lanem_rpw=None, lds_pad=None, sym_fused=None, lanem_cluster=None, zero_plans=None, zero_merge=None, gs_correction=None):
         lib = capi.lib()
         for key, v in ((0, lds_entries), (1, nnz_per_lane), (2, max_rows), (3, flow_cap), (5, gs_mode), (6, gran_cap), (7, gran_xcd), (8, stream_flags), (11, gs_prof),
                        (12, tile_G), (13, tile_W), (14, tile_cap), (15, tile_default), (16, tile_D), (17, tile_Q), (18, tile_part), (19, idx16), (20, gs_cap), (21, val8), (22, rowgather), (23, rowpat),
-                       (24, gs_order), (25, lane_L), (26, lane_G), (27, lane_wide), (28, lane_flags), (30, line_scan), (31, rowmask_kz), (32, rowmask_flags), (33, lane_merge), (34, lanem_ahead), (35, lanem_rpw), (36, lds_pad), (37, sym_fused), (38, lanem_cluster), (39, zero_plans), (40, zero_merge)):
+                       (24, gs_order), (25, lane_L), (26, lane_G), (27, lane_wide), (28, lane_flags), (30, line_scan), (31, rowmask_kz), (32, rowmask_flags), (33, lane_merge), (34, lanem_ahead), (35, lanem_rpw), (36, lds_pad), (37, sym_fused), (38, lanem_cluster), (39, zero_plans), (40, zero_merge), (41, gs_correction)):
             if v is not None:
                 capi.check(lib.pamg_matrix_tune(self.handle, key, int(v)), "pamg_matrix_tune")
 
@@ -184,6 +184,9 @@
         capi.check(capi.lib().pamg_matrix_gauss_seidel(self.handle, x.ptr, b.ptr, capi.SWEEP[sweep],
                                                        float(omega), int(iterations), stream),
                    "pamg_matrix_gauss_seidel")
+
+    def gauss_seidel_correction(self, x, b, r, iterations=1, stream=None):
+        capi.check(capi.lib().pamg_matrix_gauss_seidel_correction(self.handle, x.ptr, b.ptr, r.ptr, int(iterations), stream), "pamg_matrix_gauss_seidel_correction")
 
     def gauss_seidel_x0(self, x, b, sweep="symmetric", omega=1.0, iterations=1, x_is_zero=False, stream=None):
         capi.check(capi.lib().pamg_matrix_gauss_seidel_x0(self.handle, x.ptr, b.ptr, capi.SWEEP[sweep], float(omega), int(iterations),
```

Measured after the change: 96.44 cycles/s, median of 6. 1.06x the previous value.
